# supyuxiang/Inference-Time-Scaling-for-Diffusion-Models-beyond-Scaling-Denoising-Steps

Hardware: AMD Instinct MI355X
Metric: candidate-images/sec at T=1000, CIFAR-10 32x32 UNet, N=256, 1/2/4/8 MI355X (higher is better)
Workload: dtype bf16; 1 GPU; random-search round: N=256/GPU candidates x T=1000 DDPM steps, Arch A UNet 32x32 (ch128 [1,2,3,4] attn[2] nrb2), Oracle verifier; model=DDPM UNet (Diffusion/Model.py) Arch A, global_batch=256, seq_len=1000, parallelism=candidate-dp1, T=1000, graph=True, n_local=256

## Files before the change

include/itsd.h:

```cpp
#ifndef ITSD_H
#define ITSD_H

#include <stdint.h>

#ifdef __cplusplus
extern "C" {
#endif

#define ITSD_OK 0
#define ITSD_ERR_INVALID 1
#define ITSD_ERR_HIP 2
#define ITSD_ERR_WEIGHTS 3
#define ITSD_ERR_NAN 4
#define ITSD_ERR_OOM 5
#define ITSD_ERR_HANDOFF 6

enum { ITSD_ARCH_DDPM = 0, ITSD_ARCH_CFG = 1 };
enum { ITSD_PREC_FP32 = 0, ITSD_PREC_BF16 = 1 };
enum { ITSD_VERIFY_ORACLE = 0, ITSD_VERIFY_SELFSUP = 1, ITSD_VERIFY_AESTHETIC = 2, ITSD_VERIFY_MEAN = 3 };

#define ITSD_RUN_GRAPH 1u
#define ITSD_RUN_CLIP 2u
#define ITSD_RUN_SYNC 4u

typedef struct itsd_unet itsd_unet;

typedef struct {
  int32_t arch;
  int32_t T;
  int32_t ch;
  int32_t n_mult;
  int32_t ch_mult[8];
  int32_t n_attn;
  int32_t attn[8];
  int32_t num_res_blocks;
  int32_t img_size;
  int32_t num_labels;
  int32_t max_batch;
  int32_t precision;
} itsd_unet_desc;

typedef struct {
  const char* name;
  const float* data;
  int64_t numel;
} itsd_tensor_view;

int itsd_unet_create(const itsd_unet_desc* desc, const itsd_tensor_view* weights, int n_weights,
                     int device, itsd_unet** out);
int itsd_unet_destroy(itsd_unet* u);

int itsd_unet_forward(itsd_unet* u, const float* x, const int32_t* t, const int32_t* labels,
                      float* eps, int n, void* stream);

int itsd_unet_representation(itsd_unet* u, float* repr, int n, void* stream);

int itsd_set_schedule(itsd_unet* u, int T, const float* coeff1, const float* coeff2,
                      const float* sqrt_var, float w);

typedef struct {
  int32_t K;
  const int32_t* tau;
  const float* a0;
  const float* b0;
  const float* c0;
  const float* cx;
  const float* sg;
  int32_t clip_x0;
  float w;
} itsd_x0_schedule;

int itsd_set_schedule_x0(itsd_unet* u, const itsd_x0_schedule* schedule);

int itsd_sampler_run(itsd_unet* u, float* x, const int32_t* labels, int n, int t_begin, int t_end,
                     uint64_t seed, int64_t noise_offset, const float* noise, uint32_t flags, void* stream);

int itsd_sampler_predict_x0(itsd_unet* u, const float* x, const int32_t* labels, int n, int t,
                            float a0, float b0, float* x0, void* stream);

int itsd_branch(float* dst, const float* src, const int32_t* parents, int n_src, int n_dst, int64_t per_cand,
                float a, float b, uint64_t seed, uint32_t stream_id, int64_t cand_offset, void* stream);

int itsd_noise(float* out, const float* pivot, int n_cand, int64_t per_cand, float scale, uint64_t seed,
               uint32_t stream_id, int64_t cand_offset, void* stream);

int itsd_verify(int kind, const float* images, int n_cand, int b, int c, int h, int w,
                double* scores, void* stream);

int itsd_verify_paired(const float* images, const float* ref_features, int n_cand, int c, int h, int w,
                       double* scores, void* stream);

int itsd_attention(const void* qkv, const void* vt, void* out, int n, int S, int C, int precision, void* stream);

int itsd_profile_forward(itsd_unet* u, const float* x, const int32_t* t, int n, double* conv_ms,
                         double* conv_flops, int* conv_launches, double* total_ms, void* stream);

int itsd_profile_ops(itsd_unet* u, const float* x, const int32_t* t, int n, int max_ops, int* kinds,
                     double* ms, double* flops, int* shapes, int* n_ops, void* stream);

int itsd_profile_op(itsd_unet* u, const float* x, const int32_t* t, int n, int op_index, int reps, double* ms,
                    void* stream);

int itsd_set_option(const char* key, int value);

int itsd_unet_query(const itsd_unet* u, const char* key, int64_t* value);

enum { ITSD_OP_GN = 0, ITSD_OP_CONV = 1, ITSD_OP_ATTN = 2, ITSD_OP_GNCOEF = 3, ITSD_OP_ATTNBLOCK = 4,
       ITSD_OP_HEAD = 5, ITSD_OP_TAIL = 6 };
enum { ITSD_TAG_NONE = 0,
       ITSD_TAG_QKV = 1,
       ITSD_TAG_DOWN_MERGE = 2,
       ITSD_TAG_ATTN_S1 = 3,
       ITSD_TAG_CONVT = 4,
       ITSD_TAG_ATTNBLOCK = 5 };
#define ITSD_ACT_PROJ (-2)
typedef struct {
  int32_t kind;
  int32_t launched;
  int32_t folded_into;
  int32_t src1, src2, dst, resid, vt;
  int32_t ksize, stride, pad, upsample, zins, subpix, Cout, K, temb_col, vt_from;
  int32_t silu;
  int32_t S, C;
  int32_t kernel;
  int32_t ksplit, sc_split, kS;
  int32_t epilogue;
  int32_t gn_fold;
  int32_t gn_out_op;
  int32_t sc_op;
  int32_t has_coef;
  int32_t tag;
  char name[96];
} itsd_op_info;
typedef struct {
  int32_t H, W, C;
  int32_t elem_size;
  int32_t has_stats;
  int32_t spi;
  int32_t capacity;
} itsd_act_info;
enum { ITSD_PASS_FORWARD = 0, ITSD_PASS_STEP = 1 };
int itsd_unet_op_info(itsd_unet* u, int pass, int n, int op_index, itsd_op_info* info);
int itsd_unet_act_info(const itsd_unet* u, int act, itsd_act_info* info);
enum { ITSD_READ_ACT = 0, ITSD_READ_STATS = 1, ITSD_READ_COEF = 2, ITSD_READ_PROJ = 3 };
int itsd_unet_read(itsd_unet* u, int what, int id, int n, void* dst, int64_t bytes, void* stream);
int itsd_unet_poison(itsd_unet* u, void* stream);

const char* itsd_kernel_name(int id);

enum { ITSD_CALIB_MFMA_BF16 = 0, ITSD_CALIB_HBM_COPY = 1, ITSD_CALIB_MFMA_BF16_16X16 = 2 };
int itsd_calibrate(int what, double* value, void* stream);

const char* itsd_last_error(void);
int itsd_version(void);

#ifdef __cplusplus
}
#endif
#endif
```

inference-time-scaling-for-diffusion-models-beyond-scaling-denoising-steps_amd/csrc/api.hip:

```cpp
#include <hip/hip_runtime.h>

#include <cmath>
#include <cstdio>
#include <cstring>
#include <functional>
#include <map>
#include <memory>
#include <mutex>
#include <string>
#include <tuple>
#include <unordered_map>
#include <vector>

#include "common.h"
#include "itsd.h"

namespace itsd {
template <typename T> hipError_t launch_conv(const ConvArgs&, const ConvPlan&, hipStream_t);
template <typename T> hipError_t launch_groupnorm(const GNArgs&, int, hipStream_t);
template <typename T> hipError_t launch_attn(const AttnArgs&, int, hipStream_t);
bool attn_flash_ok(int S, int C);
bool attn_cs_ok(int S, int C);
bool attn_block_ok(int S, int C);
hipError_t launch_attn_block(const AttnBlockArgs&, int, hipStream_t);
int g_attn_fuse = 1;
int g_tap_prune = 1;
int g_down_merge = 1;
int g_attn_s1 = 1;
template <typename T> hipError_t launch_head(const HeadArgs&, hipStream_t);
template <typename T> hipError_t launch_tail(const TailArgs&, hipStream_t);
hipError_t launch_emb_input(const int*, int, const float*, const float*, int, float*, int, hipStream_t);
hipError_t launch_linear(const float*, int, int, const float*, const float*, int, int, float*, hipStream_t);
hipError_t launch_verify(int, const float*, int, int, int, int, int, double*, const float*, hipStream_t);
hipError_t launch_set_int(int*, int, hipStream_t);
hipError_t launch_add_int(int*, int, hipStream_t);
int calibrate_run(int what, double* value, hipStream_t s);
hipError_t launch_run_begin(int*, int, int*, RunParams*, const RunParams&, hipStream_t);
int g_option_gen = 0;
bool conv_gn_eligible(int H, int W);
bool p5_eligible(int H, int W);
hipError_t launch_gn_coef(const GNArgs&, int, float*, hipStream_t);
hipError_t launch_head_mfma(const HeadArgs&, hipStream_t);
hipError_t launch_tail_mfma(const TailArgs&, hipStream_t);
bool tail_mfma_ok(int H, int W, int C);
int g_io_mfma = 1;
int g_small_gn = 1;
hipError_t launch_noise(float*, const float*, int, long long, float, unsigned long long, unsigned, long long,
                        hipStream_t);
hipError_t launch_branch(float*, const float*, const int*, int, long long, float, float, unsigned long long, unsigned,
                         long long, hipStream_t);
template <typename T> hipError_t launch_nhwc_to_nchw(const void*, float*, int, int, int, hipStream_t);
}

using namespace itsd;

namespace {

thread_local std::string g_err;

int fail(int code, const std::string& msg) {
  g_err = msg;
  return code;
}

#define HIPCHK(x)                                                                           \
  do {                                                                                      \
    hipError_t e_ = (x);                                                                    \
    if (e_ != hipSuccess) return fail(ITSD_ERR_HIP, std::string(#x) + ": " + hipGetErrorString(e_)); \
  } while (0)

#define CHK(x)                  \
  do {                          \
    int r_ = (x);               \
    if (r_ != ITSD_OK) return r_; \
  } while (0)

std::string handoff_msg(int bits) {
  std::string m = "in-kernel hand-off wait exhausted its poll bound (grid not co-resident?):";
  if (bits & 1) m += " attn_block_split_kernel";
  if (bits & 2) m += " conv3x3_gn_p5_kernel (split-K combine)";
  return m;
}

uint16_t host_f2bf(float f) {
  uint32_t u;
  std::memcpy(&u, &f, 4);
  if ((u & 0x7fffffffu) > 0x7f800000u) return (uint16_t)((u >> 16) | 0x40);
  u += 0x7fffu + ((u >> 16) & 1u);
  return (uint16_t)(u >> 16);
}

struct Act {
  size_t off;
  int H, W, C;
  size_t stats = SIZE_MAX;
  int spi = 0;
};

enum OpKind { OP_GN, OP_CONV, OP_ATTN, OP_GNCOEF, OP_ATTNBLOCK };
constexpr int kCensusAttnBlock = 7;
constexpr int kCensusConvGN = 4;
constexpr int kCensusConvGNW = 5;
constexpr int kCensusConvGNW4 = 6;

struct Op {
  OpKind kind;
  int src1 = -1, src2 = -1, dst = -1;
  size_t gamma = 0, beta = 0;
  int silu = 0;
  int ksize = 3, stride = 1, pad = 1, upsample = 0, zins = 0;
  int subpix = 0;
  size_t wt = 0, bias = 0;
  size_t wfrag = SIZE_MAX;
  int Cout = 0, K = 0;
  int temb_col = -1;
  int resid = -1;
  int S = 0, C = 0;
  int vt = -1, vt_from = 0;
  size_t coef = SIZE_MAX;
  size_t bias2 = 0;
  size_t gn_gamma = SIZE_MAX, gn_beta = SIZE_MAX;
  int sc_op = -1, sc_into = -1;
  size_t sc_wfrag = SIZE_MAX, bias_sc = SIZE_MAX;
  int gn_next = -1, gn_from = -1;
  std::string name;
  int tag = ITSD_TAG_NONE;
};

struct Arena {
  std::vector<char> host;
  size_t add(const void* p, size_t bytes) {
    size_t off = (host.size() + 255) & ~(size_t)255;
    host.resize(off + bytes);
    if (p) std::memcpy(host.data() + off, p, bytes);
    return off;
  }
};

struct GraphEntry {
  std::tuple<int, bool, const float*, int, int> key;
  hipGraphExec_t exec = nullptr;
};

}

struct itsd_unet {
  itsd_unet_desc d{};
  int device = 0;
  bool bf16 = false;
  size_t esz = 4;
  bool cfg = false;
  int H = 32, ch = 128, tdim = 512, sumC = 0;
  int nb_max = 0;
  int last_forward_n = 0;

  char* wdev = nullptr;
  char* ws = nullptr;
  size_t ws_bytes = 0;
  std::vector<Act> acts;
  std::vector<Op> ops;
  int head_out = -1, tail_g = -1, tail_in = -1;
  size_t tail_gn_g = 0, tail_gn_b = 0;

  size_t head_w = 0, head_b = 0, tail_w = 0, tail_b = 0;
  size_t head_wmf = SIZE_MAX, tail_wmf = SIZE_MAX, tail_coef = SIZE_MAX;
  size_t freq = 0, ttable = 0, W0t = 0, b0 = 0, W2t = 0, b2 = 0, Wpt = 0, bp = 0;
  size_t ctable = 0, C1t = 0, cb1 = 0, C3t = 0, cb3 = 0, Wct = 0, bc = 0;

  float* emb_buf = nullptr;
  float* h1_buf = nullptr;
  float* te_buf = nullptr;
  float* proj_buf = nullptr;
  int rows_cap = 0;
  float* cemb_table = nullptr;
  int T_sched = 0;
  float* coeff1 = nullptr;
  float* coeff2 = nullptr;
  float* sqrt_var = nullptr;
  float* temb_table = nullptr;
  int sched_form = 0;
  float* xrow = nullptr;
  int clip_x0 = 0;
  float guide_w = 0.f, guide_w1 = 1.f;
  int* d_t = nullptr;
  int* d_nan = nullptr;
  RunParams* d_run = nullptr;
  float* x_state = nullptr;
  int32_t* lab_state = nullptr;
  long long graph_captures = 0;
  void* zero_page = nullptr;
  float* splitk_ws = nullptr;
  int* tickets = nullptr;
  int* attn_sync = nullptr;
  static constexpr long long kSplitkCap = 16ll << 20;

  hipStream_t stream = nullptr;
  hipEvent_t ev_in = nullptr, ev_out = nullptr;
  std::vector<GraphEntry> graphs;

  template <typename P = float>
  P* wp(size_t off) const { return (P*)(wdev + off); }
  void* ap(int id) const { return ws + acts[id].off; }
};

namespace {

struct Builder {
  itsd_unet* u;
  Arena ar;
  std::unordered_map<std::string, std::pair<const float*, int64_t>> w;
  size_t used = 0;
  size_t ws_off = 0;
  std::string err;
  std::vector<std::pair<std::string, size_t>> temb_cols;

  const float* get(const std::string& name, int64_t numel) {
    auto it = w.find(name);
    if (it == w.end()) {
      if (err.empty()) err = "missing key in state_dict: " + name;
      return nullptr;
    }
    if (it->second.second != numel) {
      if (err.empty())
        err = "size mismatch for " + name + ": got " + std::to_string(it->second.second) + " elements, expected " +
              std::to_string(numel);
      return nullptr;
    }
    ++used;
    return it->second.first;
  }
  const float* peek(const std::string& name, int64_t numel) {
    auto it = w.find(name);
    return (it == w.end() || it->second.second != numel) ? nullptr : it->second.first;
  }
  size_t f32(const std::string& name, int64_t numel) {
    const float* p = get(name, numel);
    return ar.add(p, numel * 4);
  }
  int act(int H, int W, int C) {
    Act a{ws_off, H, W, C};
    size_t bytes = (size_t)u->nb_max * H * W * C * u->esz;
    ws_off = (ws_off + bytes + 255) & ~(size_t)255;
    u->acts.push_back(a);
    return (int)u->acts.size() - 1;
  }
  size_t pack(const std::vector<const float*>& parts, int Cpart, int Cin, int ks, bool flip_t = false) {
    const int Cout = Cpart * (int)parts.size();
    const int K = ks * ks * Cin;
    std::vector<float> tmp((size_t)Cout * K, 0.f);
    for (size_t pi = 0; pi < parts.size(); ++pi) {
      const float* src = parts[pi];
      if (!src) continue;
      for (int co = 0; co < Cpart; ++co)
        for (int ci = 0; ci < Cin; ++ci)
          for (int ky = 0; ky < ks; ++ky)
            for (int kx = 0; kx < ks; ++kx) {
              float v;
              if (!flip_t) v = src[(((size_t)co * Cin + ci) * ks + ky) * ks + kx];
              else v = src[(((size_t)ci * Cpart + co) * ks + (ks - 1 - ky)) * ks + (ks - 1 - kx)];
              tmp[((size_t)pi * Cpart + co) * K + (ky * ks + kx) * Cin + ci] = v;
            }
    }
    if (u->bf16) {
      std::vector<uint16_t> b(tmp.size());
      for (size_t i = 0; i < tmp.size(); ++i) b[i] = host_f2bf(tmp[i]);
      return ar.add(b.data(), b.size() * 2);
    }
    return ar.add(tmp.data(), tmp.size() * 4);
  }
  size_t pack_frag(const float* Wsrc, int Cout, int Cin, int ks) {
    const int K = ks * ks * Cin, nks = K / 16;
    std::vector<uint16_t> b((size_t)Cout * K, 0);
    if (Wsrc)
      for (int cb = 0; cb < Cout / 32; ++cb)
        for (int st = 0; st < nks; ++st)
          for (int L = 0; L < 64; ++L)
            for (int e = 0; e < 8; ++e) {
              const int co = 32 * cb + (L & 31), k = 16 * st + 8 * (L >> 5) + e;
              const int tap = k / Cin, ci = k - tap * Cin, ky = tap / ks, kx = tap - ky * ks;
              b[(((size_t)cb * nks + st) * 64 + L) * 8 + e] =
                  host_f2bf(Wsrc[(((size_t)co * Cin + ci) * ks + ky) * ks + kx]);
            }
    return ar.add(b.data(), b.size() * 2);
  }
  size_t frag4(const std::vector<float>& tmp, int Cout, int K) {
    if (!u->bf16 || Cout % 32 || K % 16) return SIZE_MAX;
    const int nks = K / 16;
    std::vector<uint16_t> f(tmp.size());
    for (int ph = 0; ph < 4; ++ph)
      for (int cb = 0; cb < Cout / 32; ++cb)
        for (int st = 0; st < nks; ++st)
          for (int L = 0; L < 64; ++L)
            for (int e = 0; e < 8; ++e)
              f[((((size_t)ph * (Cout / 32) + cb) * nks + st) * 64 + L) * 8 + e] =
                  host_f2bf(tmp[((size_t)ph * Cout + 32 * cb + (L & 31)) * K + 16 * st + 8 * (L >> 5) + e]);
    return ar.add(f.data(), f.size() * 2);
  }
  size_t pack_subpix(const float* W, int Cout, int Cin, size_t* wfrag = nullptr) {
    static const int lo[2][2] = {{0, 1}, {0, 2}}, hi[2][2] = {{0, 2}, {1, 2}};
    const int K = 4 * Cin;
    std::vector<float> tmp((size_t)4 * Cout * K, 0.f);
    for (int ph = 0; ph < 4; ++ph) {
      const int py = ph >> 1, px = ph & 1;
      for (int co = 0; co < Cout; ++co)
        for (int dy = 0; dy < 2; ++dy)
          for (int dx = 0; dx < 2; ++dx)
            for (int ci = 0; ci < Cin; ++ci) {
              double acc = 0.0;
              for (int ky = lo[py][dy]; ky <= hi[py][dy]; ++ky)
                for (int kx = lo[px][dx]; kx <= hi[px][dx]; ++kx)
                  acc += W ? (double)W[(((size_t)co * Cin + ci) * 3 + ky) * 3 + kx] : 0.0;
              tmp[((size_t)ph * Cout + co) * K + (dy * 2 + dx) * Cin + ci] = (float)acc;
            }
    }
    if (wfrag) *wfrag = frag4(tmp, Cout, K);
    if (u->bf16) {
      std::vector<uint16_t> b(tmp.size());
      for (size_t i = 0; i < tmp.size(); ++i) b[i] = host_f2bf(tmp[i]);
      return ar.add(b.data(), b.size() * 2);
    }
    return ar.add(tmp.data(), tmp.size() * 4);
  }
  size_t pack_convt_subpix(const float* W, int Cout, int Cin, size_t* wfrag = nullptr, bool centre_only = false) {
    auto kk = [](int r, int d) { return r == 0 ? 2 - 2 * d : (d < 0 ? -1 : 3 - 2 * d); };
    const int rd = centre_only ? 0 : 1, kw = 2 * rd + 1, K = kw * kw * Cin;
    std::vector<float> tmp((size_t)4 * Cout * K, 0.f);
    for (int ph = 0; ph < 4; ++ph) {
      const int ry = ph >> 1, rx = ph & 1;
      for (int co = 0; co < Cout; ++co)
        for (int dy = -rd; dy <= rd; ++dy)
          for (int dx = -rd; dx <= rd; ++dx) {
            const int ky = kk(ry, dy), kx = kk(rx, dx);
            if (ky < 0 || kx < 0 || !W) continue;
            for (int ci = 0; ci < Cin; ++ci)
              tmp[((size_t)ph * Cout + co) * K + ((dy + rd) * kw + dx + rd) * Cin + ci] =
                  W[(((size_t)ci * Cout + co) * 5 + ky) * 5 + kx];
          }
    }
    if (wfrag) *wfrag = frag4(tmp, Cout, K);
    if (u->bf16) {
      std::vector<uint16_t> b(tmp.size());
      for (size_t i = 0; i < tmp.size(); ++i) b[i] = host_f2bf(tmp[i]);
      return ar.add(b.data(), b.size() * 2);
    }
    return ar.add(tmp.data(), tmp.size() * 4);
  }
  int upconv(int s1, const std::string& name, int Cout, int Hout) {
    const Act& A = u->acts[s1];
    const int Cin = A.C, epc = u->bf16 ? 8 : 4;
    if (((A.H * A.W) % 128 && 128 % (A.H * A.W)) || Cin % (8 * epc))
      return conv_layer(s1, -1, name, Cout, 3, 1, 1, 1, Hout, Hout);
    const float* W = get(name + ".weight", (int64_t)Cout * Cin * 9);
    size_t wf = SIZE_MAX;
    const bool p4sub = Cout % 128 == 0 && Cin % 64 == 0 && Cin >= 128 && A.H == A.W && (A.W == 8 || A.W == 16 || A.W == 32);
    size_t wt = pack_subpix(W, Cout, Cin, p4sub ? &wf : nullptr);
    size_t b = f32(name + ".bias", Cout);
    int dst = act(Hout, Hout, Cout);
    if (A.H * A.W < 128) u->acts[dst].spi = 4;
    conv(s1, -1, dst, wt, b, Cout, 3, 1, 1, 1);
    Op& o = u->ops.back();
    o.name = name;
    o.subpix = 1;
    o.wfrag = wf;
    return dst;
  }
  size_t concat_f32(const std::vector<const float*>& parts, int n) {
    std::vector<float> tmp((size_t)n * parts.size(), 0.f);
    for (size_t i = 0; i < parts.size(); ++i)
      if (parts[i]) std::memcpy(tmp.data() + i * n, parts[i], n * 4);
    return ar.add(tmp.data(), tmp.size() * 4);
  }
  size_t transposed(const float* W, int out, int in) {
    std::vector<float> tmp((size_t)out * in, 0.f);
    if (W)
      for (int o = 0; o < out; ++o)
        for (int i = 0; i < in; ++i) tmp[(size_t)i * out + o] = W[(size_t)o * in + i];
    return ar.add(tmp.data(), tmp.size() * 4);
  }

  void gn(int s1, int s2, int dst, const std::string& p, int C, int silu) {
    Op o;
    o.kind = OP_GN;
    o.src1 = s1; o.src2 = s2; o.dst = dst;
    o.gamma = f32(p + ".weight", C);
    o.beta = f32(p + ".bias", C);
    o.silu = silu;
    o.name = p;
    u->ops.push_back(o);
  }
  void conv(int s1, int s2, int dst, size_t wt, size_t bias, int Cout, int ks, int stride, int pad, int ups,
            int temb_col = -1, int resid = -1, int zins = 0) {
    Op o;
    o.kind = OP_CONV;
    o.src1 = s1; o.src2 = s2; o.dst = dst;
    o.wt = wt; o.bias = bias; o.Cout = Cout;
    const int Cin = u->acts[s1].C + (s2 >= 0 ? u->acts[s2].C : 0);
    o.K = ks * ks * Cin;
    o.ksize = ks; o.stride = stride; o.pad = pad; o.upsample = ups; o.zins = zins;
    o.temb_col = temb_col; o.resid = resid;
    u->ops.push_back(o);
  }
  int conv_layer(int s1, int s2, const std::string& name, int Cout, int ks, int stride, int pad, int ups, int Hout,
                 int Wout, int temb_col = -1, int resid = -1, const std::string& gn = "", const float* Wx = nullptr,
                 const float* bx = nullptr) {
    const int Cin = u->acts[s1].C + (s2 >= 0 ? u->acts[s2].C : 0);
    size_t coef = SIZE_MAX;
    if (!gn.empty()) {
      Op g;
      g.kind = OP_GNCOEF;
      g.src1 = s1; g.src2 = s2;
      g.gamma = f32(gn + ".weight", Cin);
      g.beta = f32(gn + ".bias", Cin);
      g.coef = coef = ws_off;
      g.name = gn;
      ws_off = (ws_off + (size_t)u->nb_max * Cin * 2 * 4 + 255) & ~(size_t)255;
      u->ops.push_back(g);
    }
    const float* W = Wx ? Wx : get(name + ".weight", (int64_t)Cout * Cin * ks * ks);
    std::vector<float> wwin;
    {
      const Act& A = u->acts[s1];
      const int k0 = std::max(0, pad - (Hout - 1) * stride), k1 = std::min(ks - 1, A.H + pad - 1);
      const int x0 = std::max(0, pad - (Wout - 1) * stride), x1 = std::min(ks - 1, A.W + pad - 1);
      if (itsd::g_tap_prune && gn.empty() && !ups && W && (k0 > 0 || k1 < ks - 1) && k0 == x0 && k1 == x1 && k1 >= k0) {
        const int ks2 = k1 - k0 + 1;
        wwin.resize((size_t)Cout * Cin * ks2 * ks2);
        for (size_t oc = 0; oc < (size_t)Cout * Cin; ++oc)
          for (int ky = 0; ky < ks2; ++ky)
            for (int kx = 0; kx < ks2; ++kx)
              wwin[(oc * ks2 + ky) * ks2 + kx] = W[(oc * ks + k0 + ky) * ks + k0 + kx];
        W = wwin.data();
        ks = ks2;
        pad -= k0;
      }
    }
    size_t wt = pack({W}, Cout, Cin, ks);
    size_t b = bx ? ar.add(bx, (size_t)Cout * 4) : f32(name + ".bias", Cout);
    int dst = act(Hout, Wout, Cout);
    conv(s1, s2, dst, wt, b, Cout, ks, stride, pad, ups, temb_col, resid);
    u->ops.back().name = name;
    u->ops.back().coef = coef;
    if (coef != SIZE_MAX) {
      u->ops.back().gn_gamma = u->ops[u->ops.size() - 2].gamma;
      u->ops.back().gn_beta = u->ops[u->ops.size() - 2].beta;
    }
    const bool plain3 = coef == SIZE_MAX && ks == 3 && stride == 1 && pad == 1 && !ups && Cout % 128 == 0 &&
                        Cin % 128 == 0 && Hout == Wout && (Hout == 32 || Hout == 16 || Hout == 8);
    if ((coef != SIZE_MAX || plain3) && u->bf16 && Cout % 32 == 0 && (ks * ks * Cin) % 16 == 0)
      u->ops.back().wfrag = pack_frag(W, Cout, Cin, ks);
    return dst;
  }
  bool fusable(int s1, int s2, int Cout) const {
    const Act& A = u->acts[s1];
    return u->bf16 && itsd::g_fuse_gn && A.C % 64 == 0 && (s2 < 0 || u->acts[s2].C % 64 == 0) &&
           Cout % 128 == 0 && (conv_gn_eligible(A.H, A.W) || p5_eligible(A.H, A.W));
  }

  int resblock(int x1, int x2, const std::string& p, int in_ch, int out_ch, bool attn) {
    const int H = u->acts[x1].H, W = u->acts[x1].W;
    const int col = u->sumC;
    u->sumC += out_ch;
    temb_cols.push_back({p, (size_t)col});
    int h1, o;
    int resid = x1;
    if (fusable(x1, x2, out_ch)) {
      h1 = conv_layer(x1, x2, p + ".block1.2", out_ch, 3, 1, 1, 0, H, W, col, -1, p + ".block1.0");
    } else {
      int g1 = act(H, W, in_ch);
      gn(x1, x2, g1, p + ".block1.0", in_ch, 1);
      h1 = conv_layer(g1, -1, p + ".block1.2", out_ch, 3, 1, 1, 0, H, W, col);
    }
    const bool f2 = fusable(h1, -1, out_ch);
    int g2 = -1;
    if (!f2) {
      g2 = act(H, W, out_ch);
      gn(h1, -1, g2, p + ".block2.0", out_ch, 1);
    }
    int isc = -1;
    if (in_ch != out_ch) {
      resid = conv_layer(x1, x2, p + ".shortcut", out_ch, 1, 1, 0, 0, H, W);
      isc = (int)u->ops.size() - 1;
    }
    if (f2) o = conv_layer(h1, -1, p + ".block2.3", out_ch, 3, 1, 1, 0, H, W, -1, resid, p + ".block2.0");
    else o = conv_layer(g2, -1, p + ".block2.3", out_ch, 3, 1, 1, 0, H, W, -1, resid);
    if (f2 && isc >= 0 && u->bf16 && out_ch % 32 == 0 && u->acts[x1].C % 64 == 0 && (x2 < 0 || u->acts[x2].C % 64 == 0)) {
      const float* wsc = peek(p + ".shortcut.weight", (int64_t)out_ch * in_ch);
      const float* bsc = peek(p + ".shortcut.bias", out_ch);
      const float* bb2 = peek(p + ".block2.3.bias", out_ch);
      if (wsc && bsc && bb2) {
        std::vector<float> bs((size_t)out_ch);
        for (int c = 0; c < out_ch; ++c) bs[c] = bb2[c] + bsc[c];
        Op& c2 = u->ops.back();
        c2.sc_wfrag = pack_frag(wsc, out_ch, in_ch, 1);
        c2.bias_sc = ar.add(bs.data(), (size_t)out_ch * 4);
        c2.sc_op = isc;
        u->ops[isc].sc_into = (int)u->ops.size() - 1;
      }
    }
    if (attn && H * W == 1 && itsd::g_attn_s1) {
      const std::string a = p + ".attn";
      const int64_t cc = (int64_t)out_ch * out_ch;
      const float* wv = get(a + ".proj_v.weight", cc);
      const float* bv = get(a + ".proj_v.bias", out_ch);
      const float* wp = get(a + ".proj.weight", cc);
      const float* bp = get(a + ".proj.bias", out_ch);
      const bool qk = get(a + ".proj_q.weight", cc) && get(a + ".proj_q.bias", out_ch) && get(a + ".proj_k.weight", cc) &&
                      get(a + ".proj_k.bias", out_ch);
      if (wv && bv && wp && bp && qk) {
        std::vector<float> wf((size_t)cc), bf((size_t)out_ch);
        std::vector<double> row((size_t)out_ch);
        for (int oc = 0; oc < out_ch; ++oc) {
          std::fill(row.begin(), row.end(), 0.0);
          double bacc = (double)bp[oc];
          for (int c = 0; c < out_ch; ++c) {
            const double w = (double)wp[(size_t)oc * out_ch + c];
            const float* vr = wv + (size_t)c * out_ch;
            for (int ic = 0; ic < out_ch; ++ic) row[ic] += w * (double)vr[ic];
            bacc += w * (double)bv[c];
          }
          for (int ic = 0; ic < out_ch; ++ic) wf[(size_t)oc * out_ch + ic] = (float)row[ic];
          bf[oc] = (float)bacc;
        }
        int ga = act(H, W, out_ch);
        gn(o, -1, ga, a + ".group_norm", out_ch, 0);
        const int r = conv_layer(ga, -1, a + ".proj", out_ch, 1, 1, 0, 0, H, W, -1, o, "", wf.data(), bf.data());
        u->ops.back().name = a;
        u->ops.back().tag = ITSD_TAG_ATTN_S1;
        return r;
      }
    }
    if (attn && u->bf16 && itsd::g_attn_fuse && attn_block_ok(H * W, out_ch)) {
      const std::string a = p + ".attn";
      const int C = out_ch;
      const int64_t cc = (int64_t)C * C;
      const float* wq = get(a + ".proj_q.weight", cc);
      const float* wk = get(a + ".proj_k.weight", cc);
      const float* wv = get(a + ".proj_v.weight", cc);
      const float* wp = get(a + ".proj.weight", cc);
      const float* bq = get(a + ".proj_q.bias", C);
      const float* bv = get(a + ".proj_v.bias", C);
      get(a + ".proj_k.bias", C);
      std::vector<float> wcat((size_t)2 * cc, 0.f), bcat((size_t)2 * C, 0.f);
      if (wq && wk && wv && wp && bq && bv) {
        std::vector<double> acc((size_t)cc);
        auto fold = [&](const float* A, const float* B, bool ta, float* dst) {
          std::fill(acc.begin(), acc.end(), 0.0);
          for (int r = 0; r < C; ++r) {
            double* row = acc.data() + (size_t)r * C;
            for (int k = 0; k < C; ++k) {
              const double w = (double)(ta ? A[(size_t)k * C + r] : A[(size_t)r * C + k]);
              const float* br = B + (size_t)k * C;
              for (int i = 0; i < C; ++i) row[i] += w * (double)br[i];
            }
          }
          for (int64_t i = 0; i < cc; ++i) dst[i] = (float)acc[i];
        };
        fold(wk, wq, true, wcat.data());
        fold(wp, wv, false, wcat.data() + cc);
        for (int j = 0; j < C; ++j) {
          double su = 0.0, sb = 0.0;
          for (int k = 0; k < C; ++k) {
            su += (double)wk[(size_t)k * C + j] * (double)bq[k];
            sb += (double)wp[(size_t)j * C + k] * (double)bv[k];
          }
          bcat[j] = (float)su;
          bcat[C + j] = (float)sb;
        }
      }
      Op ab;
      ab.kind = OP_ATTNBLOCK;
      ab.src1 = o;
      ab.gamma = f32(a + ".group_norm.weight", out_ch);
      ab.beta = f32(a + ".group_norm.bias", out_ch);
      ab.wt = pack_frag(wcat.data(), 2 * out_ch, out_ch, 1);
      ab.bias = ar.add(bcat.data(), bcat.size() * 4);
      ab.bias2 = f32(a + ".proj.bias", out_ch);
      ab.S = H * W;
      ab.C = out_ch;
      ab.dst = act(H, W, out_ch);
      ab.name = a;
      ab.tag = ITSD_TAG_ATTNBLOCK;
      u->ops.push_back(ab);
      return ab.dst;
    }
    if (attn) {
      const std::string a = p + ".attn";
      int ga = act(H, W, out_ch);
      gn(o, -1, ga, a + ".group_norm", out_ch, 0);
      const int64_t cc = (int64_t)out_ch * out_ch;
      size_t wqkv = pack({get(a + ".proj_q.weight", cc), get(a + ".proj_k.weight", cc), get(a + ".proj_v.weight", cc)},
                         out_ch, out_ch, 1);
      size_t bqkv = concat_f32({get(a + ".proj_q.bias", out_ch), get(a + ".proj_k.bias", out_ch),
                                get(a + ".proj_v.bias", out_ch)}, out_ch);
      int qkv = act(H, W, 3 * out_ch);
      conv(ga, -1, qkv, wqkv, bqkv, 3 * out_ch, 1, 1, 0, 0);
      u->ops.back().name = a;
      u->ops.back().tag = ITSD_TAG_QKV;
      const int S = H * W;
      int vt = -1;
      if (u->bf16 && S % 16 == 0 && out_ch % 64 == 0 && (S <= 256 || attn_flash_ok(S, out_ch) || attn_cs_ok(S, out_ch))) {
        vt = act(out_ch, S, 1);
        u->ops.back().vt = vt;
        u->ops.back().vt_from = 2 * out_ch;
      }
      int ao = act(H, W, out_ch);
      Op at;
      at.kind = OP_ATTN;
      at.name = a;
      at.src1 = qkv; at.dst = ao; at.S = H * W; at.C = out_ch; at.vt = vt;
      u->ops.push_back(at);
      o = conv_layer(ao, -1, a + ".proj", out_ch, 1, 1, 0, 0, H, W, -1, o);
    }
    return o;
  }
};

int build(itsd_unet* u, const itsd_tensor_view* views, int nviews) {
  Builder b;
  b.u = u;
  for (int i = 0; i < nviews; ++i) b.w[views[i].name] = {views[i].data, views[i].numel};
  const itsd_unet_desc& d = u->d;
  const int ch = d.ch, tdim = 4 * ch, H = d.img_size;
  u->ch = ch; u->tdim = tdim; u->H = H;

  if (!u->cfg) {
    u->freq = b.f32("time_embedding.freq_coeffs", ch / 2);
    u->W0t = b.transposed(b.get("time_embedding.timembedding.0.weight", (int64_t)tdim * ch), tdim, ch);
    u->b0 = b.f32("time_embedding.timembedding.0.bias", tdim);
    u->W2t = b.transposed(b.get("time_embedding.timembedding.2.weight", (int64_t)tdim * tdim), tdim, tdim);
    u->b2 = b.f32("time_embedding.timembedding.2.bias", tdim);
  } else {
    u->ttable = b.f32("time_embedding.timembedding.0.weight", (int64_t)d.T * ch);
    u->W0t = b.transposed(b.get("time_embedding.timembedding.1.weight", (int64_t)tdim * ch), tdim, ch);
    u->b0 = b.f32("time_embedding.timembedding.1.bias", tdim);
    u->W2t = b.transposed(b.get("time_embedding.timembedding.3.weight", (int64_t)tdim * tdim), tdim, tdim);
    u->b2 = b.f32("time_embedding.timembedding.3.bias", tdim);
    u->ctable = b.f32("cond_embedding.condEmbedding.0.weight", (int64_t)(d.num_labels + 1) * ch);
    u->C1t = b.transposed(b.get("cond_embedding.condEmbedding.1.weight", (int64_t)tdim * ch), tdim, ch);
    u->cb1 = b.f32("cond_embedding.condEmbedding.1.bias", tdim);
    u->C3t = b.transposed(b.get("cond_embedding.condEmbedding.3.weight", (int64_t)tdim * tdim), tdim, tdim);
    u->cb3 = b.f32("cond_embedding.condEmbedding.3.bias", tdim);
  }
  u->head_w = b.f32("head.weight", (int64_t)ch * 27);
  u->head_b = b.f32("head.bias", ch);
  u->head_out = b.act(H, H, ch);
  if (u->bf16 && itsd::g_io_mfma && ch % 32 == 0 && (H * H) % 128 == 0 && 128 % H == 0) {
    const float* hw = b.peek("head.weight", (int64_t)ch * 27);
    if (hw) {
      std::vector<uint16_t> wm((size_t)ch * 32, 0);
      for (int co = 0; co < ch; ++co)
        for (int k = 0; k < 27; ++k) wm[(size_t)co * 32 + k] = host_f2bf(hw[(size_t)co * 27 + k]);
      u->head_wmf = b.ar.add(wm.data(), wm.size() * 2);
    }
  } else {
    const int G = stat_slot_px(H * H);
    if ((H * H) % G || (G % H && H % G))
      return fail(ITSD_ERR_INVALID, "img_size " + std::to_string(H) + " not supported by the head kernel (its " +
                                        std::to_string(G) + "-pixel blocks hold whole rows or lie inside one)");
  }

  std::vector<int> hs{u->head_out};
  int cur = u->head_out;
  int now = ch;
  int ndown = 0;
  auto P = [](const char* s, int i) { return std::string(s) + "." + std::to_string(i); };
  for (int i = 0; i < d.n_mult; ++i) {
    const int out = ch * d.ch_mult[i];
    bool at = false;
    for (int k = 0; k < d.n_attn; ++k) at |= (d.attn[k] == i);
    if (u->cfg) at = true;
    for (int r = 0; r < d.num_res_blocks; ++r) {
      cur = b.resblock(cur, -1, P("downblocks", ndown++), now, out, at);
      now = out;
      hs.push_back(cur);
    }
    if (i != d.n_mult - 1) {
      const std::string p = P("downblocks", ndown++);
      const int Hc = b.u->acts[cur].H;
      if (!u->cfg) {
        cur = b.conv_layer(cur, -1, p + ".main", now, 3, 2, 1, 0, Hc / 2, Hc / 2);
      } else if (!itsd::g_down_merge) {
        int t1 = b.conv_layer(cur, -1, p + ".c1", now, 3, 2, 1, 0, Hc / 2, Hc / 2);
        cur = b.conv_layer(cur, -1, p + ".c2", now, 5, 2, 2, 0, Hc / 2, Hc / 2, -1, t1);
      } else {
        const int Cin = b.u->acts[cur].C;
        const float* W1 = b.get(p + ".c1.weight", (int64_t)now * Cin * 9);
        const float* W2 = b.get(p + ".c2.weight", (int64_t)now * Cin * 25);
        const float* b1 = b.get(p + ".c1.bias", now);
        const float* b2 = b.get(p + ".c2.bias", now);
        std::vector<float> wm((size_t)now * Cin * 25, 0.f), bm(now, 0.f);
        if (W2) std::memcpy(wm.data(), W2, wm.size() * 4);
        if (W1)
          for (size_t oc = 0; oc < (size_t)now * Cin; ++oc)
            for (int ky = 0; ky < 3; ++ky)
              for (int kx = 0; kx < 3; ++kx) wm[(oc * 5 + ky + 1) * 5 + kx + 1] += W1[(oc * 3 + ky) * 3 + kx];
        for (int c = 0; c < now; ++c) bm[c] = (b1 ? b1[c] : 0.f) + (b2 ? b2[c] : 0.f);
        cur = b.conv_layer(cur, -1, p + ".c12", now, 5, 2, 2, 0, Hc / 2, Hc / 2, -1, -1, "", wm.data(), bm.data());
        u->ops.back().name = p;
        u->ops.back().tag = ITSD_TAG_DOWN_MERGE;
      }
      hs.push_back(cur);
    }
  }
  cur = b.resblock(cur, -1, "middleblocks.0", now, now, true);
  cur = b.resblock(cur, -1, "middleblocks.1", now, now, false);
  int nup = 0;
  for (int i = d.n_mult - 1; i >= 0; --i) {
    const int out = ch * d.ch_mult[i];
    bool at = false;
    for (int k = 0; k < d.n_attn; ++k) at |= (d.attn[k] == i);
    if (u->cfg) at = false;
    for (int r = 0; r < d.num_res_blocks + 1; ++r) {
      int skip = hs.back();
      hs.pop_back();
      cur = b.resblock(cur, skip, P("upblocks", nup++), now + u->acts[skip].C, out, at);
      now = out;
    }
    if (i != 0) {
      const std::string p = P("upblocks", nup++);
      const int Hc = b.u->acts[cur].H;
      if (!u->cfg) {
        cur = b.upconv(cur, p + ".main", now, 2 * Hc);
      } else {
        const float* Wt = b.get(p + ".t.weight", (int64_t)now * now * 25);
        size_t bt = b.f32(p + ".t.bias", now);
        int tmp = b.act(2 * Hc, 2 * Hc, now);
        const int epc = u->bf16 ? 8 : 4;
        if (((Hc * Hc) % 128 == 0 || 128 % (Hc * Hc) == 0) && now % (8 * epc) == 0) {
          size_t wf = SIZE_MAX;
          const bool p4sub = now % 128 == 0 && now >= 128 && (Hc == 8 || Hc == 16 || Hc == 32);
          const bool c1 = Hc == 1 && itsd::g_tap_prune;
          size_t wt = b.pack_convt_subpix(Wt, now, now, p4sub ? &wf : nullptr, c1);
          if (Hc * Hc < 128) u->acts[tmp].spi = 4;
          b.conv(cur, -1, tmp, wt, bt, now, c1 ? 1 : 3, 1, c1 ? 0 : 1, 0);
          u->ops.back().subpix = 2;
          u->ops.back().wfrag = wf;
          u->ops.back().name = p + ".t";
          u->ops.back().tag = ITSD_TAG_CONVT;
        } else {
          size_t wt = b.pack({Wt}, now, now, 5, true);
          b.conv(cur, -1, tmp, wt, bt, now, 5, 1, 2, 0, -1, -1, 1);
          u->ops.back().name = p + ".t";
          u->ops.back().tag = ITSD_TAG_CONVT;
        }
        cur = b.conv_layer(tmp, -1, p + ".c", now, 3, 1, 1, 0, 2 * Hc, 2 * Hc);
      }
    }
  }
  if (!hs.empty()) return fail(ITSD_ERR_INVALID, "internal: skip stack not empty");
  u->tail_in = cur;
  u->tail_gn_g = b.f32("tail.0.weight", now);
  u->tail_gn_b = b.f32("tail.0.bias", now);
  u->tail_w = b.f32("tail.2.weight", (int64_t)3 * now * 9);
  u->tail_b = b.f32("tail.2.bias", 3);
  if (u->bf16 && itsd::g_io_mfma && tail_mfma_ok(H, H, now)) {
    const float* tw = b.peek("tail.2.weight", (int64_t)3 * now * 9);
    if (tw) {
      const int nks = 9 * now / 32;
      std::vector<uint16_t> wm((size_t)nks * 4 * 3 * 8);
      for (int ks = 0; ks < nks; ++ks)
        for (int kg = 0; kg < 4; ++kg)
          for (int co = 0; co < 3; ++co)
            for (int j = 0; j < 8; ++j) {
              const int k = 32 * ks + 8 * kg + j, tap = k / now, ci = k - tap * now;
              wm[(((size_t)ks * 4 + kg) * 3 + co) * 8 + j] = host_f2bf(tw[((size_t)co * now + ci) * 9 + tap]);
            }
      u->tail_wmf = b.ar.add(wm.data(), wm.size() * 2);
    }
    u->tail_coef = b.ws_off;
    b.ws_off = (b.ws_off + (size_t)u->nb_max * now * 2 * 4 + 255) & ~(size_t)255;
  } else {
    u->tail_g = b.act(H, H, now);
  }

  {
    std::vector<float> Wp((size_t)u->sumC * tdim), bpv(u->sumC), Wc, bcv;
    if (u->cfg) { Wc.resize(Wp.size()); bcv.resize(u->sumC); }
    for (size_t k = 0; k < b.temb_cols.size(); ++k) {
      const std::string& p = b.temb_cols[k].first;
      const size_t col = b.temb_cols[k].second;
      const size_t next = (k + 1 < b.temb_cols.size()) ? b.temb_cols[k + 1].second : (size_t)u->sumC;
      const int oc = (int)(next - col);
      auto fill = [&](const std::string& nm, std::vector<float>& Wd, std::vector<float>& bd) {
        const float* W = b.get(nm + ".weight", (int64_t)oc * tdim);
        const float* bb = b.get(nm + ".bias", oc);
        if (!W || !bb) return;
        for (int o = 0; o < oc; ++o) {
          for (int i = 0; i < tdim; ++i) Wd[(size_t)i * u->sumC + col + o] = W[(size_t)o * tdim + i];
          bd[col + o] = bb[o];
        }
      };
      fill(p + ".temb_proj.1", Wp, bpv);
      if (u->cfg) fill(p + ".cond_proj.1", Wc, bcv);
    }
    u->Wpt = b.ar.add(Wp.data(), Wp.size() * 4);
    u->bp = b.ar.add(bpv.data(), bpv.size() * 4);
    if (u->cfg) {
      u->Wct = b.ar.add(Wc.data(), Wc.size() * 4);
      u->bc = b.ar.add(bcv.data(), bcv.size() * 4);
    }
  }
  if (!b.err.empty()) return fail(ITSD_ERR_WEIGHTS, b.err);
  if ((int)b.used != nviews) {
    return fail(ITSD_ERR_WEIGHTS, "state_dict has " + std::to_string(nviews) + " entries, model uses " +
                                      std::to_string(b.used) + " (unexpected keys present)");
  }
  for (size_t i = 1; i < u->ops.size(); ++i) {
    Op& g = u->ops[i];
    Op& p = u->ops[i - 1];
    if (g.kind == OP_GN && g.src2 < 0 && p.kind == OP_CONV && p.dst == g.src1 && p.sc_into < 0 && p.vt < 0) {
      p.gn_next = (int)i;
      g.gn_from = (int)i - 1;
    }
  }
  {
    std::vector<int> need;
    for (const Op& o : u->ops)
      if (o.kind == OP_GN || o.kind == OP_GNCOEF || o.kind == OP_ATTNBLOCK) {
        need.push_back(o.src1);
        if (o.src2 >= 0) need.push_back(o.src2);
      }
    need.push_back(u->tail_in);
    for (int id : need) {
      Act& A = u->acts[id];
      if (A.stats != SIZE_MAX) continue;
      const int HW = A.H * A.W;
      if (!(128 % HW == 0 || HW % 128 == 0))
        return fail(ITSD_ERR_INVALID, "spatial size " + std::to_string(HW) + " not supported by the GN statistics slots");
      const size_t slots = (size_t)u->nb_max * stat_spi(HW, A.spi);
      A.stats = b.ws_off;
      b.ws_off = (b.ws_off + slots * 2 * A.C * 4 + 255) & ~(size_t)255;
      bool produced = (id == u->head_out);
      for (const Op& o : u->ops) produced |= ((o.kind == OP_CONV || o.kind == OP_ATTNBLOCK) && o.dst == id);
      if (!produced) return fail(ITSD_ERR_INVALID, "internal: GroupNorm input without a statistics producer");
    }
  }
  HIPCHK(hipMalloc(&u->wdev, b.ar.host.size()));
  HIPCHK(hipMemcpy(u->wdev, b.ar.host.data(), b.ar.host.size(), hipMemcpyHostToDevice));
  u->ws_bytes = b.ws_off;
  HIPCHK(hipMalloc(&u->ws, u->ws_bytes));
  return ITSD_OK;
}

struct RunCtx {
  int nb;
  const float* x;
  int x_mod;
  const float* temb;
  const int* tsel;
  long long temb_img_stride;
  const int32_t* labels;
  int label_mod;
  int uncond_from;
  TailArgs tail;
  bool census = false;
  std::vector<std::pair<hipEvent_t, hipEvent_t>>* evs = nullptr;
  std::vector<int>* ev_kind = nullptr;
  std::vector<double>* ev_flops = nullptr;
  std::vector<int>* ev_kid = nullptr;
  std::vector<int>* ev_op = nullptr;
};

int conv_args(itsd_unet* u, const Op& o, const RunCtx& c, ConvArgs& a, ConvPlan& p) {
    const Act& in = u->acts[o.src1];
    const Act& out = u->acts[o.dst];
    a.src1 = u->ap(o.src1);
    a.src2 = o.src2 >= 0 ? u->ap(o.src2) : nullptr;
    a.C1 = in.C;
    a.C2 = o.src2 >= 0 ? u->acts[o.src2].C : 0;
    a.Hin = in.H; a.Win = in.W; a.Hout = out.H; a.Wout = out.W;
    a.ksize = o.ksize; a.stride = o.stride; a.pad = o.pad; a.upsample = o.upsample;
    a.wt = u->wdev + o.wt;
    a.wfrag = o.wfrag != SIZE_MAX ? u->wdev + o.wfrag : nullptr;
    a.Cout = o.Cout; a.K = o.K;
    a.bias = u->wp(o.bias);
    if (o.temb_col >= 0) {
      a.temb = c.temb + o.temb_col;
      a.temb_tsel = c.tsel;
      a.temb_row_stride = u->sumC;
      a.temb_img_stride = c.temb_img_stride;
      if (u->cfg) {
        a.cemb = u->cemb_table + o.temb_col;
        a.cemb_labels = (const int*)c.labels;
        a.cemb_row_stride = u->sumC;
        a.cemb_label_mod = c.label_mod;
        a.cemb_uncond_from = c.uncond_from;
      }
    }
    a.resid = o.resid >= 0 ? u->ap(o.resid) : nullptr;
    a.out = u->ap(o.dst);
    a.M = c.nb * out.H * out.W;
    a.stats = out.stats != SIZE_MAX ? (float*)(u->ws + out.stats) : nullptr;
    a.zero = u->zero_page;
    a.splitk_ws = u->splitk_ws;
    a.splitk_cap = itsd_unet::kSplitkCap;
    a.tickets = u->tickets;
    a.err = u->d_nan + 1;
    a.spin_bound = itsd::g_spin_bound;
    if (o.vt >= 0) {
      if (o.vt_from % 128 || (out.H * out.W) % 8) return fail(ITSD_ERR_INVALID, "internal: bad channel-major V split");
      a.vt_out = u->ap(o.vt);
      a.vt_from = o.vt_from;
    }
    a.zins = o.zins;
    a.dbg = itsd::g_conv_dbg;
    a.xcd = itsd::g_p4_xcd == 1 || (itsd::g_p4_xcd == 2 && a.Wout == 8);
    if (o.subpix) {
      a.subpix = o.subpix;
      a.Hout = in.H; a.Wout = in.W;
      a.M = c.nb * in.H * in.W;
      a.ksize = o.subpix == 2 ? o.ksize : 2; a.pad = o.subpix == 2 ? o.pad : 0; a.upsample = 0; a.zins = 0;
      a.K = a.ksize * a.ksize * (a.C1 + a.C2);
      a.tap_live = o.subpix == 2 && a.ksize == 3 && itsd::g_convt_prune;
    }
    if (o.coef != SIZE_MAX) {
      if (!u->bf16 || o.ksize != 3 || o.stride != 1 || o.pad != 1 || o.upsample || o.zins ||
          !(conv_gn_eligible(in.H, in.W) || p5_eligible(in.H, in.W)) || a.C1 % 64 || a.C2 % 64 || a.Cout % 128)
        return fail(ITSD_ERR_INVALID, "internal: fused GroupNorm conv on an unsupported shape");
      a.gn_coef = (const float*)(u->ws + o.coef);
    }
    {
      const int epc = u->bf16 ? 8 : 4;
      if (a.C1 % epc || a.C2 % epc || a.Cout % 4 || a.K % epc)
        return fail(ITSD_ERR_INVALID, "conv channels must be multiples of " + std::to_string(epc));
    }
  if (o.sc_op >= 0 && itsd::g_p5_sc) {
    const Op& sc = u->ops[o.sc_op];
    a.sc_src1 = u->ap(sc.src1);
    a.sc_src2 = sc.src2 >= 0 ? u->ap(sc.src2) : nullptr;
    a.sc_C1 = u->acts[sc.src1].C;
    a.sc_C2 = sc.src2 >= 0 ? u->acts[sc.src2].C : 0;
    a.sc_wfrag = u->wdev + o.sc_wfrag;
  }
  p = plan_conv(a, u->bf16);
  const bool p5 = p.kernel == ConvKernel::P5 || p.kernel == ConvKernel::P5_SHARED;
  const bool p4 = p.kernel == ConvKernel::P4_GN || p.kernel == ConvKernel::P4_C96;
  if (p.sc_split) {
    a.bias = u->wp(o.bias_sc);
    a.resid = nullptr;
  } else {
    a.sc_src1 = a.sc_src2 = a.sc_wfrag = nullptr;
    a.sc_C1 = a.sc_C2 = 0;
  }
  if (a.gn_coef && o.gn_gamma != SIZE_MAX && itsd::g_gn_fold && (a.C1 + a.C2) % 128 == 0 && in.H * in.W <= 1024 &&
      (p5 || p4)) {
    a.gn_fold = 1;
    a.gn_st1 = (const float*)(u->ws + u->acts[o.src1].stats);
    a.gn_st2 = o.src2 >= 0 ? (const float*)(u->ws + u->acts[o.src2].stats) : nullptr;
    a.gn_spi1 = u->acts[o.src1].spi;
    a.gn_spi2 = o.src2 >= 0 ? u->acts[o.src2].spi : 0;
    a.gn_gamma = u->wp(o.gn_gamma);
    a.gn_beta = u->wp(o.gn_beta);
  }
  if (o.gn_next >= 0 && itsd::g_small_gn && u->bf16 && a.stats && !a.gn_coef && !o.subpix && !a.vt_out &&
      u->acts[o.dst].spi == 0) {
    const int HWo = a.Hout * a.Wout, gs = a.Cout / kGnGroups;
    if (HWo <= 16 && 64 % HWo == 0 && a.Cout % 64 == 0 && gs >= 2 && 64 % gs == 0 && p.kernel == ConvKernel::SMALL) {
      const Op& g = u->ops[o.gn_next];
      a.gn_out = u->ap(g.dst);
      a.go_gamma = u->wp(g.gamma);
      a.go_beta = u->wp(g.beta);
      a.go_silu = g.silu;
    }
  }
  return ITSD_OK;
}

struct ConvLaunch {
  ConvArgs a{};
  ConvPlan p;
  int rc = ITSD_OK;
  std::string err;
};

std::vector<ConvLaunch> resolve_program(itsd_unet* u, const RunCtx& c) {
  std::vector<ConvLaunch> r(u->ops.size());
  for (size_t oi = 0; oi < u->ops.size(); ++oi) {
    if (u->ops[oi].kind != OP_CONV) continue;
    r[oi].rc = conv_args(u, u->ops[oi], c, r[oi].a, r[oi].p);
    if (r[oi].rc != ITSD_OK) r[oi].err = g_err;
  }
  return r;
}

int folded_into(const itsd_unet* u, const std::vector<ConvLaunch>& rp, size_t oi) {
  const Op& o = u->ops[oi];
  if (o.kind == OP_GNCOEF && oi + 1 < u->ops.size() && rp[oi + 1].a.gn_fold) return (int)oi + 1;
  if (o.kind == OP_GN && o.gn_from >= 0 && rp[o.gn_from].a.gn_out) return o.gn_from;
  if (o.kind == OP_CONV && o.sc_into >= 0 && rp[o.sc_into].p.sc_split) return o.sc_into;
  return -1;
}

GNArgs gn_args(const itsd_unet* u, const Op& o) {
  GNArgs g{};
  g.C1 = u->acts[o.src1].C;
  g.C2 = o.src2 >= 0 ? u->acts[o.src2].C : 0;
  g.HW = u->acts[o.src1].H * u->acts[o.src1].W;
  g.gamma = u->wp(o.gamma);
  g.beta = u->wp(o.beta);
  g.eps = kGnEps;
  g.st1 = (const float*)(u->ws + u->acts[o.src1].stats);
  g.st2 = o.src2 >= 0 ? (const float*)(u->ws + u->acts[o.src2].stats) : nullptr;
  g.spi1 = u->acts[o.src1].spi;
  g.spi2 = o.src2 >= 0 ? u->acts[o.src2].spi : 0;
  return g;
}

int launch_op(itsd_unet* u, const Op& o, const RunCtx& c, const ConvLaunch* cl, hipStream_t s) {
  hipError_t e = hipSuccess;
  if (o.kind == OP_GNCOEF) {
    e = launch_gn_coef(gn_args(u, o), c.nb, (float*)(u->ws + o.coef), s);
  } else if (o.kind == OP_GN) {
    GNArgs a = gn_args(u, o);
    a.src1 = u->ap(o.src1);
    a.src2 = o.src2 >= 0 ? u->ap(o.src2) : nullptr;
    a.silu = o.silu;
    a.dst = u->ap(o.dst);
    e = u->bf16 ? launch_groupnorm<bf16_t>(a, c.nb, s) : launch_groupnorm<float>(a, c.nb, s);
  } else if (o.kind == OP_CONV) {
    if (cl->rc != ITSD_OK) return fail(cl->rc, cl->err);
    e = u->bf16 ? launch_conv<bf16_t>(cl->a, cl->p, s) : launch_conv<float>(cl->a, cl->p, s);
  } else if (o.kind == OP_ATTNBLOCK) {
    AttnBlockArgs a{};
    const Act& in = u->acts[o.src1];
    const Act& out = u->acts[o.dst];
    a.x = (const bf16_t*)u->ap(o.src1);
    a.st = (const float*)(u->ws + in.stats);
    a.spi = stat_spi(in.H * in.W, in.spi);
    a.gamma = u->wp(o.gamma);
    a.beta = u->wp(o.beta);
    a.wmv = (const bf16_t*)(u->wdev + o.wt);
    a.buv = u->wp(o.bias);
    a.bp = u->wp(o.bias2);
    a.out = (bf16_t*)u->ap(o.dst);
    a.out_stats = out.stats != SIZE_MAX ? (float*)(u->ws + out.stats) : nullptr;
    a.scale = (float)std::pow((double)o.C, -0.5);
    a.n = c.nb;
    a.S = o.S;
    static_assert((4ll << 20) / 4 <= itsd_unet::kSplitkCap, "the partial-score slab fits the split-K workspace");
    a.spart = u->splitk_ws;
    a.sync = u->attn_sync;
    a.err = u->d_nan + 1;
    a.spin_bound = itsd::g_spin_bound;
    e = launch_attn_block(a, o.C, s);
  } else {
    AttnArgs a{};
    a.qkv = u->ap(o.src1);
    a.vt = o.vt >= 0 ? u->ap(o.vt) : nullptr;
    a.out = u->ap(o.dst);
    a.S = o.S; a.C = o.C;
    a.scale = (float)std::pow((double)o.C, -0.5);
    e = u->bf16 ? launch_attn<bf16_t>(a, c.nb, s) : launch_attn<float>(a, c.nb, s);
  }
  if (e != hipSuccess) return fail(ITSD_ERR_HIP, std::string("kernel launch: ") + hipGetErrorString(e));
  return ITSD_OK;
}

double op_flops(const itsd_unet* u, const Op& o, int nb) {
  if (o.kind == OP_CONV) {
    const Act& out = u->acts[o.dst];
    return 2.0 * nb * out.H * out.W * (double)o.Cout * (o.subpix == 1 ? o.K * 4 / 9 : o.K);
  }
  if (o.kind == OP_ATTN) return 2.0 * 2.0 * nb * (double)o.S * o.S * o.C;
  if (o.kind == OP_ATTNBLOCK)
    return 2.0 * nb * (double)o.S * (4.0 * o.C * o.C) + 2.0 * 2.0 * nb * (double)o.S * o.S * o.C;
  return 0.0;
}

int run_program(itsd_unet* u, const RunCtx& c, const std::vector<ConvLaunch>& rp, hipStream_t s) {
  int cur_op = 0;
  auto mark = [&](int kind, double fl, const std::function<int()>& fn) -> int {
    if (!c.census) return fn();
    if (c.ev_op) c.ev_op->push_back(cur_op);
    hipEvent_t a, b;
    HIPCHK(hipEventCreate(&a));
    if (hipError_t e = hipEventCreate(&b); e != hipSuccess) {
      hipEventDestroy(a);
      return fail(ITSD_ERR_HIP, std::string("hipEventCreate(&b): ") + hipGetErrorString(e));
    }
    HIPCHK(hipEventRecord(a, s));
    itsd::g_last_kernel = nullptr;
    int r = fn();
    HIPCHK(hipEventRecord(b, s));
    c.evs->push_back({a, b});
    c.ev_kind->push_back(kind);
    c.ev_flops->push_back(fl);
    if (c.ev_kid) c.ev_kid->push_back(itsd::kernel_id(itsd::g_last_kernel));
    return r;
  };
  CHK(mark(-1, 2.0 * c.nb * u->H * u->H * 27.0 * u->ch, [&]() -> int {
    HeadArgs h{};
    h.x = c.x;
    h.w = u->wp(u->head_w);
    h.b = u->wp(u->head_b);
    h.out = u->ap(u->head_out);
    h.H = u->H; h.W = u->H; h.Cout = u->ch; h.n = c.nb; h.x_img_mod = c.x_mod;
    const Act& ho = u->acts[u->head_out];
    h.stats = ho.stats != SIZE_MAX ? (float*)(u->ws + ho.stats) : nullptr;
    hipError_t e;
    if (u->head_wmf != SIZE_MAX) {
      h.wmf = (const bf16_t*)(u->wdev + u->head_wmf);
      e = launch_head_mfma(h, s);
    } else {
      e = u->bf16 ? launch_head<bf16_t>(h, s) : launch_head<float>(h, s);
    }
    return e == hipSuccess ? ITSD_OK : fail(ITSD_ERR_HIP, hipGetErrorString(e));
  }));
  for (size_t oi = 0; oi < u->ops.size(); ++oi) {
    const Op& o = u->ops[oi];
    if (folded_into(u, rp, oi) >= 0) continue;
    const ConvLaunch& cl = rp[oi];
    int kind = o.kind == OP_ATTNBLOCK ? kCensusAttnBlock : (int)o.kind;
    cur_op = (int)oi + 1;
    if (o.kind == OP_CONV && o.coef != SIZE_MAX)
      kind = cl.p.wide_segs == 1 ? kCensusConvGNW : cl.p.wide_segs == 4 ? kCensusConvGNW4 : kCensusConvGN;
    double fl = op_flops(u, o, c.nb);
    if (cl.p.sc_split) fl += 2.0 * cl.a.M * (double)o.Cout * (cl.a.sc_C1 + cl.a.sc_C2);
    CHK(mark(kind, fl, [&]() { return launch_op(u, o, c, &cl, s); }));
  }
  cur_op = 0;
  Op g;
  g.src1 = u->tail_in; g.gamma = u->tail_gn_g; g.beta = u->tail_gn_b; g.silu = 1;
  if (u->tail_wmf != SIZE_MAX) {
    g.kind = OP_GNCOEF;
    g.coef = u->tail_coef;
  } else {
    g.kind = OP_GN;
    g.dst = u->tail_g;
  }
  CHK(mark((int)g.kind, 0.0, [&]() { return launch_op(u, g, c, nullptr, s); }));
  CHK(mark(-2, 2.0 * c.tail.n * (c.tail.cfg ? 2 : 1) * u->H * u->H * 27.0 * u->acts[u->tail_in].C, [&]() -> int {
    TailArgs t = c.tail;
    t.w = u->wp(u->tail_w);
    t.b = u->wp(u->tail_b);
    t.H = u->H; t.W = u->H; t.C = u->acts[u->tail_in].C;
    hipError_t e;
    if (u->tail_wmf != SIZE_MAX) {
      t.g = u->ap(u->tail_in);
      t.coef = (const float*)(u->ws + u->tail_coef);
      t.wmf = (const bf16_t*)(u->wdev + u->tail_wmf);
      e = launch_tail_mfma(t, s);
    } else {
      t.g = u->ap(u->tail_g);
      e = u->bf16 ? launch_tail<bf16_t>(t, s) : launch_tail<float>(t, s);
    }
    return e == hipSuccess ? ITSD_OK : fail(ITSD_ERR_HIP, hipGetErrorString(e));
  }));
  return ITSD_OK;
}

int temb_rows(itsd_unet* u, const int* idx, int M, int offset, bool cond, float* out, hipStream_t s) {
  if (M > u->rows_cap) return fail(ITSD_ERR_INVALID, "temb rows exceed capacity");
  const int ch = u->ch, td = u->tdim;
  hipError_t e;
  if (!cond) {
    e = launch_emb_input(idx, M, u->cfg ? nullptr : u->wp(u->freq), u->cfg ? u->wp(u->ttable) : nullptr, ch,
                         u->emb_buf, offset, s);
  } else {
    e = launch_emb_input(idx, M, nullptr, u->wp(u->ctable), ch, u->emb_buf, offset, s);
  }
  if (e != hipSuccess) return fail(ITSD_ERR_HIP, hipGetErrorString(e));
  const float* W0 = u->wp(cond ? u->C1t : u->W0t);
  const float* b0 = u->wp(cond ? u->cb1 : u->b0);
  const float* W2 = u->wp(cond ? u->C3t : u->W2t);
  const float* b2 = u->wp(cond ? u->cb3 : u->b2);
  HIPCHK(launch_linear(u->emb_buf, M, ch, W0, b0, td, 0, u->h1_buf, s));
  HIPCHK(launch_linear(u->h1_buf, M, td, W2, b2, td, 1, u->te_buf, s));
  HIPCHK(launch_linear(u->te_buf, M, td, u->wp(cond ? u->Wct : u->Wpt), u->wp(cond ? u->bc : u->bp), u->sumC, 1,
                       out, s));
  return ITSD_OK;
}

int alloc_rows(itsd_unet* u, int rows) {
  if (rows <= u->rows_cap) return ITSD_OK;
  hipFree(u->emb_buf); hipFree(u->h1_buf); hipFree(u->te_buf);
  HIPCHK(hipMalloc(&u->emb_buf, (size_t)rows * u->ch * 4));
  HIPCHK(hipMalloc(&u->h1_buf, (size_t)rows * u->tdim * 4));
  HIPCHK(hipMalloc(&u->te_buf, (size_t)rows * u->tdim * 4));
  u->rows_cap = rows;
  return ITSD_OK;
}

void clear_graphs(itsd_unet* u) {
  for (auto& g : u->graphs)
    if (g.exec) hipGraphExecDestroy(g.exec);
  u->graphs.clear();
}

void drop_schedule(itsd_unet* u) {
  clear_graphs(u);
  hipFree(u->coeff1); hipFree(u->coeff2); hipFree(u->sqrt_var); hipFree(u->xrow); hipFree(u->temb_table);
  u->coeff1 = u->coeff2 = u->sqrt_var = u->xrow = u->temb_table = nullptr;
  u->T_sched = 0;
  u->sched_form = 0;
  u->clip_x0 = 0;
}

int check_batch(itsd_unet* u, int n) {
  if (n <= 0 || n > u->d.max_batch)
    return fail(ITSD_ERR_INVALID, "batch " + std::to_string(n) + " outside [1, max_batch=" +
                                      std::to_string(u->d.max_batch) + "]");
  return ITSD_OK;
}

RunCtx forward_ctx(const itsd_unet* u, int n, const float* x, const int32_t* labels, float* eps_out) {
  RunCtx c{};
  c.nb = n; c.x = x; c.x_mod = n;
  c.temb = u->proj_buf; c.tsel = nullptr; c.temb_img_stride = u->sumC;
  c.labels = labels; c.label_mod = n; c.uncond_from = -1;
  c.tail.n = n; c.tail.cfg = 0; c.tail.step_mode = 0; c.tail.eps_out = eps_out;
  return c;
}

RunCtx step_ctx(const itsd_unet* u, int n, float* x, const int32_t* labels) {
  RunCtx c{};
  c.nb = u->cfg ? 2 * n : n;
  c.x = x; c.x_mod = n;
  c.temb = u->temb_table; c.tsel = u->d_t; c.temb_img_stride = 0;
  c.labels = labels; c.label_mod = n; c.uncond_from = u->cfg ? n : -1;
  c.tail.n = n; c.tail.cfg = u->cfg ? 1 : 0; c.tail.guide_w = u->guide_w; c.tail.guide_w1 = u->guide_w1;
  c.tail.x = x;
  return c;
}

int enter_stream(itsd_unet* u, hipStream_t cs) {
  HIPCHK(hipSetDevice(u->device));
  HIPCHK(hipEventRecord(u->ev_in, cs));
  HIPCHK(hipStreamWaitEvent(u->stream, u->ev_in, 0));
  return ITSD_OK;
}
int leave_stream(itsd_unet* u, hipStream_t cs) {
  HIPCHK(hipEventRecord(u->ev_out, u->stream));
  HIPCHK(hipStreamWaitEvent(cs, u->ev_out, 0));
  return ITSD_OK;
}

int step_graph(itsd_unet* u, const RunCtx& c, int n, bool labels, const float* noise, hipGraphExec_t* exec) {
  const auto key = std::make_tuple(n, labels, noise, itsd::g_option_gen, u->sched_form);
  for (auto& g : u->graphs)
    if (g.key == key) { *exec = g.exec; return ITSD_OK; }
  hipStream_t s = u->stream;
  HIPCHK(hipStreamBeginCapture(s, hipStreamCaptureModeThreadLocal));
  int r = run_program(u, c, resolve_program(u, c), s);
  if (r == ITSD_OK && launch_add_int(u->d_t, -1, s) != hipSuccess) r = fail(ITSD_ERR_HIP, "add_int");
  hipGraph_t graph = nullptr;
  hipError_t e = hipStreamEndCapture(s, &graph);
  if (r != ITSD_OK) { if (graph) hipGraphDestroy(graph); return r; }
  if (e != hipSuccess) return fail(ITSD_ERR_HIP, std::string("capture: ") + hipGetErrorString(e));
  e = hipGraphInstantiate(exec, graph, nullptr, nullptr, 0);
  hipGraphDestroy(graph);
  if (e != hipSuccess) return fail(ITSD_ERR_HIP, std::string("instantiate: ") + hipGetErrorString(e));
  if (u->graphs.size() >= 4) { hipGraphExecDestroy(u->graphs.front().exec); u->graphs.erase(u->graphs.begin()); }
  u->graphs.push_back({key, *exec});
  ++u->graph_captures;
  return ITSD_OK;
}

struct ProfileScratch {
  float* eps = nullptr;
  int32_t* lab0 = nullptr;
  std::vector<std::pair<hipEvent_t, hipEvent_t>> evs;
  std::vector<int> kinds, kid, eop;
  std::vector<double> fl;
  ~ProfileScratch() {
    for (auto& p : evs) {
      if (p.first) hipEventDestroy(p.first);
      if (p.second) hipEventDestroy(p.second);
    }
    hipFree(eps);
    hipFree(lab0);
  }
  int begin(itsd_unet* u, const int32_t* t, int n, hipStream_t cs) {
    CHK(check_batch(u, n));
    HIPCHK(hipSetDevice(u->device));
    u->last_forward_n = 0;
    HIPCHK(hipStreamSynchronize(cs));
    HIPCHK(hipMalloc(&eps, (size_t)n * 3 * u->H * u->H * 4));
    if (u->cfg) {
      HIPCHK(hipMalloc(&lab0, (size_t)n * 4));
      HIPCHK(hipMemsetAsync(lab0, 0, (size_t)n * 4, u->stream));
    }
    return temb_rows(u, t, n, 0, false, u->proj_buf, u->stream);
  }
  void census(RunCtx& c, bool ids) {
    c.census = true; c.evs = &evs; c.ev_kind = &kinds; c.ev_flops = &fl;
    if (ids) { c.ev_kid = &kid; c.ev_op = &eop; }
  }
};

}

namespace itsd {
thread_local const char* g_last_kernel = nullptr;
std::mutex& kernel_names_mu() {
  static std::mutex m;
  return m;
}
std::vector<const char*>& kernel_names() {
  static std::vector<const char*> v;
  return v;
}
int kernel_id(const char* name) {
  if (!name) return 0;
  std::lock_guard<std::mutex> lk(kernel_names_mu());
  auto& v = kernel_names();
  for (size_t i = 0; i < v.size(); ++i)
    if (v[i] == name || !std::strcmp(v[i], name)) return (int)i + 1;
  v.push_back(name);
  return (int)v.size();
}
}

namespace {
enum : unsigned {
  kDiag = 1,
  kShip1 = 2,
  kBool = 4,
  kSet = 8,
  kMask = 16,
};
struct Option {
  const char* key;
  int* var;
  int lo, hi;
  unsigned flags;
  const char* what;
  int set[6] = {-1, -1, -1, -1, -1, -1};
};
constexpr int kConvDbgMask = 1 | 2 | 8 | 16 | 32 | 64 | 128 | 256 | 512 | 1024 | 2048 | 4096 | (127 << 13) | (3 << 20);
const Option kOptions[] = {
    {"conv_variant", &g_conv_variant, 1, 2, 0, "2 conv_pipe (shipped), 1 conv_igemm (register-staged, parity checks)"},
    {"splitk", &g_splitk, 0, 64, kShip1, "split-K for under-filled grids: 0 off, 1 auto, >= 2 forced slice count"},
    {"splitk_inl", &g_splitk_inl, 0, 1, 0, "conv_pipe split-K: 1 in-launch ticket combine, 0 splitk_epilogue_kernel"},
    {"subpix_split", &g_subpix_split, 0, 1, 0, "under-filled sub-pixel conv_pipe launches split K in-launch"},
    {"conv1x1", &g_conv1x1, 0, 2, kShip1, "streaming 1x1 kernel for statistics-free 1x1 convs of large pixel counts: 0 off, 1 on, 2 the 7-stage ring"},
    {"small_conv", &g_small_conv, 0, 2, 0, "conv_small's 64x64 tiles at the small levels: 0 off, 1 auto, 2 whenever eligible"},
    {"small_8x8", &g_small_8x8, 0, 1, 0, "conv_small (split K) for under-filled 8x8-level convs"},
    {"small_wide", &g_small_wide, 0, 2, 0, "conv_small for under-filled statistics-free convs of larger images: 0 off, 1 under 256 tiles, 2 under 512"},
    {"small_minks", &g_small_minks, 1, 64, kDiag, "conv_small split K: at least this many 64-channel K-chunks a slice"},
    {"small_gn", &g_small_gn, 0, 1, 0, "conv_small writes its consumer GroupNorm's output (the GN launch skipped): 0 off, 1 on"},
    {"conv_dbg", &g_conv_dbg, 0, kConvDbgMask, kDiag | kMask, "measurement-only conv ablations (a bit mask; results are wrong when set)"},
    {"fuse_gn", &g_fuse_gn, 0, 1, kBool, "fused GroupNorm+SiLU+conv3x3 in ResBlocks (UNets created afterwards)"},
    {"gn_wide", &g_gn_wide, 0, 2, 0, "the persistent 256-pixel fused conv: 0 off, 1 auto, 2 whenever eligible"},
    {"gn_fold", &g_gn_fold, 0, 1, kBool, "GroupNorm finalize inside conv3x3_gn_p4 / p5_kernel: 0 off, 1 on"},
    {"p4_w", &g_p4_w, 0, 7, 0, "levels conv3x3_gn_p4_kernel takes (bit 0 W = 8, 1 W = 16, 2 W = 32); the others run p5 / 128-pixel tiles"},
    {"p4_xcd", &g_p4_xcd, 0, 2, kDiag, "conv3x3_gn_p4_kernel deals each XCD a contiguous range of tiles: 0 off, 1 on, 2 the 8x8 level only"},
    {"p4_c96", &g_p4_c96, 0, 2, 0, "8x8 conv3x3_gn_p4_kernel on 96-cout tiles: 0 off, 1 auto, 2 always (Cout % 96 == 0)"},
    {"p4_sub", &g_p4_sub, 0, 1, 0, "nearest-x2 upsample convs on conv3x3_gn_p4_kernel's sub-pixel form: 0 off, 1 on"},
    {"p4_plain", &g_p4_plain, 0, 2, 0, "plain 3x3 stride-1 convs on conv3x3_gn_p4_kernel (halo copies the input): 0 off, 1 from 128 tiles, 2 any tile count"},
    {"p5", &g_p5, 0, 2, 0, "conv3x3_gn_p5_kernel at 8x8: 0 off, 1 auto, 2 always (4x4: always)"},
    {"p5_split", &g_p5_split, 0, 16, 0, "p5's K slices: 0 auto (cost model), 1..16 forced"},
    {"p5_sc", &g_p5_sc, 0, 2, 0, "ResBlock 1x1 shortcuts as K slices of their block2 p5 conv: 0 off, 1 auto, 2 always"},
    {"p5_pub", &g_p5_pub, 0, 1, 0, "p5's two-slice last-arriver combine: 1 only the first arriver stores its partial, 0 both (round 5; bit-identity checks)"},
    {"p5_xl", &g_p5_xl, 0, 3, 0, "p5's split-K partials through one XCD's L2: 0 off, 1 the shared combine at 8x8 / 16x16, 2 every eligible form (A/B), 3 (shipped) 1 + the two-slice form at 8x8 / 16x16 where K <= 3456"},
    {"p5_dist", &g_p5_dist, 0, 2, 0, "p5's split-K combine shared by every slice (co-resident grids): 0 off (last arriver), 1 on, 2 the plans of 1 combined by the last arriver (bit-identity checks)"},
    {"p5_c64", &g_p5_c64, 0, 2, kDiag, "64-cout conv3x3_gn_p5_kernel items at 8x8 / 4x4: 0 off, 1 auto, 2 always"},
    {"convt_prune", &g_convt_prune, 0, 1, 0, "ConvTranspose2d sub-pixel phases skip their all-zero taps (p4 / conv_pipe)"},
    {"tap_prune", &g_tap_prune, 0, 1, kBool, "drop all-padding conv taps at build time (UNets created afterwards)"},
    {"down_merge", &g_down_merge, 0, 1, kBool, "CFG DownSample c1 + c2 as one 5x5 conv (UNets created afterwards)"},
    {"io_mfma", &g_io_mfma, 0, 1, kBool, "bf16 head / tail on MFMA (UNets created afterwards)"},
    {"attn_fuse", &g_attn_fuse, 0, 1, 0, "fused AttnBlock kernel (S = 64): 0 off, 1 on (UNets created afterwards; the 16-token form was removed)"},
    {"attn_s1", &g_attn_s1, 0, 1, 0, "one-token AttnBlock folded to GroupNorm + one 1x1 conv (UNets created afterwards)"},
    {"attn_split", &g_attn_split, 0, 6, kSet, "attn_block_split_kernel (an image over G blocks): 0 off, 1 auto, 2 / 4 / 6 forced", {0, 1, 2, 4, 6, -1}},
    {"attn_wide", &g_attn_wide, 0, 2, 0, "channel-split attention (attn_cs_kernel): 0 off, 1 auto (C >= 384 at S >= 256; C = 1024), 2 wherever it applies"},
    {"attn_wide_nq", &g_attn_wide_nq, 0, 2, 0, "channel-split attention: query groups a block (0 auto, 1, 2)"},
    {"attn_cs", &g_attn_cs, 0, 8, kDiag, "attn_mfma_kernel output-channel slices: 0 auto, 1..8 forced"},
    {"attn_aq", &g_attn_aq, 0, 64, kDiag | kSet, "attn_mfma_kernel queries per block: 0 auto, 32, 64", {0, 32, 64, -1}},
    {"spin_bound", &g_spin_bound, 0, 0x7fffffff, 0, "diagnostic: polls before an in-kernel hand-off wait fails (shipped 1 << 22)"},
};
}

extern "C" {

int itsd_version(void) { return 1; }

const char* itsd_kernel_name(int id) {
  std::lock_guard<std::mutex> lk(itsd::kernel_names_mu());
  return id > 0 && id <= (int)itsd::kernel_names().size() ? itsd::kernel_names()[id - 1] : "";
}

int itsd_set_option(const char* key, int value) {
  if (!key) return fail(ITSD_ERR_INVALID, "null key");
#ifdef ITSD_DIAG
  const bool shipped = false;
#else
  const bool shipped = true;
#endif
  const Option* o = nullptr;
  for (const Option& r : kOptions)
    if (!std::strcmp(key, r.key)) o = &r;
  if (o && shipped && (o->flags & kDiag))
    return fail(ITSD_ERR_INVALID, std::string(key) + ": diagnostic builds only (tools/build_diag.sh)");
  if (o && shipped && (o->flags & kShip1) && value > 1)
    return fail(ITSD_ERR_INVALID, std::string(key) + " in [" + std::to_string(o->lo) + ",1] (above: diagnostic builds only, tools/build_diag.sh)");
  ++itsd::g_option_gen;
  if (!o) return fail(ITSD_ERR_INVALID, std::string("unknown option ") + key);
  int v = value;
  if (o->flags & kBool) {
    v = value ? 1 : 0;
  } else if (o->flags & kMask) {
    v = value & o->hi;
  } else if (o->flags & kSet) {
    bool ok = false;
    std::string vals;
    for (const int* q = o->set; *q >= 0; ++q) {
      ok |= *q == value;
      vals += (vals.empty() ? "" : ",") + std::to_string(*q);
    }
    if (!ok) return fail(ITSD_ERR_INVALID, std::string(key) + " in {" + vals + "}: " + o->what);
  } else if (value < o->lo || value > o->hi) {
    return fail(ITSD_ERR_INVALID, std::string(key) + " in [" + std::to_string(o->lo) + "," + std::to_string(o->hi) + "]: " + o->what);
  }
  *o->var = v;
  return ITSD_OK;
}

const char* itsd_last_error(void) { return g_err.c_str(); }

int itsd_calibrate(int what, double* value, void* stream) {
  if (!value) return fail(ITSD_ERR_INVALID, "null argument");
  if (what != ITSD_CALIB_MFMA_BF16 && what != ITSD_CALIB_HBM_COPY && what != ITSD_CALIB_MFMA_BF16_16X16) return fail(ITSD_ERR_INVALID, "unknown calibration");
  const int rc = calibrate_run(what, value, (hipStream_t)stream);
  if (rc == ITSD_ERR_OOM) return fail(rc, "calibration buffers (2 x 1 GiB)");
  if (rc != ITSD_OK) return fail(rc, "calibration kernel");
  return ITSD_OK;
}

int itsd_unet_query(const itsd_unet* u, const char* key, int64_t* value) {
  if (!u || !key || !value) return fail(ITSD_ERR_INVALID, "null argument");
  if (!std::strcmp(key, "graph_captures")) *value = u->graph_captures;
  else if (!std::strcmp(key, "max_batch")) *value = u->d.max_batch;
  else if (!std::strcmp(key, "T_sched")) *value = u->T_sched;
  else if (!std::strcmp(key, "sched_form")) *value = u->sched_form;
  else if (!std::strcmp(key, "ws_bytes")) *value = (int64_t)u->ws_bytes;
  else if (!std::strcmp(key, "ops")) *value = (int64_t)u->ops.size();
  else if (!std::strcmp(key, "status")) {
    if (hipStreamSynchronize(u->stream) != hipSuccess) return fail(ITSD_ERR_HIP, "status: stream synchronize");
    int flag = 0;
    if (hipMemcpy(&flag, u->d_nan + 1, 4, hipMemcpyDeviceToHost) != hipSuccess) return fail(ITSD_ERR_HIP, "status: copy");
    *value = flag;
  }
  else return fail(ITSD_ERR_INVALID, std::string("unknown query key ") + key);
  return ITSD_OK;
}

int itsd_unet_create(const itsd_unet_desc* desc, const itsd_tensor_view* weights, int n_weights, int device,
                     itsd_unet** out) {
  if (!desc || !out || (!weights && n_weights)) return fail(ITSD_ERR_INVALID, "null argument");
  const itsd_unet_desc& d = *desc;
  if (d.arch != ITSD_ARCH_DDPM && d.arch != ITSD_ARCH_CFG) return fail(ITSD_ERR_INVALID, "unknown arch");
  if (d.ch <= 0 || d.ch % 32 || d.n_mult < 1 || d.n_mult > 8 || d.n_attn < 0 || d.n_attn > 8 ||
      d.num_res_blocks < 1 || d.max_batch < 1 || d.img_size < 8)
    return fail(ITSD_ERR_INVALID, "invalid UNet descriptor");
  if (d.img_size % (1 << (d.n_mult - 1))) return fail(ITSD_ERR_INVALID, "img_size not divisible by the down path");
  for (int k = 0; k < d.n_attn; ++k)
    if (d.attn[k] < 0 || d.attn[k] >= d.n_mult) return fail(ITSD_ERR_INVALID, "attn index out of bound");
  if (d.precision != ITSD_PREC_FP32 && d.precision != ITSD_PREC_BF16) return fail(ITSD_ERR_INVALID, "precision");
  HIPCHK(hipSetDevice(device));
  {
    int cus = 0;
    if (hipDeviceGetAttribute(&cus, hipDeviceAttributeMultiprocessorCount, device) == hipSuccess && cus > 0)
      itsd::g_num_cus = cus;
  }
  std::unique_ptr<itsd_unet> u(new itsd_unet());
  u->d = d;
  u->device = device;
  u->bf16 = d.precision == ITSD_PREC_BF16;
  u->esz = u->bf16 ? 2 : 4;
  u->cfg = d.arch == ITSD_ARCH_CFG;
  u->nb_max = d.max_batch * (u->cfg ? 2 : 1);
  CHK(build(u.get(), weights, n_weights));
  HIPCHK(hipStreamCreateWithFlags(&u->stream, hipStreamNonBlocking));
  HIPCHK(hipEventCreateWithFlags(&u->ev_in, hipEventDisableTiming));
  HIPCHK(hipEventCreateWithFlags(&u->ev_out, hipEventDisableTiming));
  HIPCHK(hipMalloc(&u->d_t, 64));
  HIPCHK(hipMalloc(&u->d_nan, 64));
  HIPCHK(hipMalloc(&u->d_run, sizeof(RunParams)));
  HIPCHK(hipMemset(u->d_run, 0, sizeof(RunParams)));
  HIPCHK(hipMalloc(&u->x_state, (size_t)d.max_batch * 3 * d.img_size * d.img_size * 4));
  HIPCHK(hipMalloc(&u->lab_state, (size_t)d.max_batch * 4));
  HIPCHK(hipMalloc(&u->zero_page, 64 * 4096 + 1024));
  HIPCHK(hipMemset(u->zero_page, 0, 64 * 4096 + 1024));
  HIPCHK(hipMalloc(&u->splitk_ws, itsd_unet::kSplitkCap * 4));
  HIPCHK(hipMalloc(&u->tickets, itsd::kTicketCap * 4));
  HIPCHK(hipMemset(u->tickets, 0, itsd::kTicketCap * 4));
  HIPCHK(hipMalloc(&u->attn_sync, (size_t)u->nb_max * 4));
  HIPCHK(hipMemset(u->attn_sync, 0, (size_t)u->nb_max * 4));
  HIPCHK(hipMalloc(&u->proj_buf, (size_t)d.max_batch * u->sumC * 4));
  CHK(alloc_rows(u.get(), std::max(d.max_batch, d.num_labels + 1)));
  if (u->cfg) {
    HIPCHK(hipMalloc(&u->cemb_table, (size_t)(d.num_labels + 1) * u->sumC * 4));
    CHK(temb_rows(u.get(), nullptr, d.num_labels + 1, 0, true, u->cemb_table, u->stream));
    HIPCHK(hipStreamSynchronize(u->stream));
  }
  *out = u.release();
  return ITSD_OK;
}

int itsd_unet_destroy(itsd_unet* u) {
  if (!u) return ITSD_OK;
  hipSetDevice(u->device);
  clear_graphs(u);
  hipFree(u->wdev); hipFree(u->ws); hipFree(u->emb_buf); hipFree(u->h1_buf); hipFree(u->te_buf);
  hipFree(u->proj_buf); hipFree(u->cemb_table); hipFree(u->coeff1); hipFree(u->coeff2); hipFree(u->sqrt_var);
  hipFree(u->xrow); hipFree(u->temb_table); hipFree(u->d_t); hipFree(u->d_nan); hipFree(u->d_run); hipFree(u->x_state); hipFree(u->lab_state); hipFree(u->zero_page);
  hipFree(u->splitk_ws);
  hipFree(u->tickets);
  hipFree(u->attn_sync);
  if (u->stream) hipStreamDestroy(u->stream);
  if (u->ev_in) hipEventDestroy(u->ev_in);
  if (u->ev_out) hipEventDestroy(u->ev_out);
  delete u;
  return ITSD_OK;
}

int itsd_unet_forward(itsd_unet* u, const float* x, const int32_t* t, const int32_t* labels, float* eps, int n,
                      void* stream) {
  if (!u || !x || !t || !eps) return fail(ITSD_ERR_INVALID, "null argument");
  if (u->cfg && !labels) return fail(ITSD_ERR_INVALID, "CFG UNet needs labels");
  CHK(check_batch(u, n));
  hipStream_t cs = (hipStream_t)stream;
  hipStream_t s = u->stream;
  CHK(enter_stream(u, cs));
  CHK(temb_rows(u, t, n, 0, false, u->proj_buf, s));
  const RunCtx c = forward_ctx(u, n, x, labels, eps);
  HIPCHK(hipMemsetAsync(u->d_nan + 1, 0, 4, s));
  CHK(run_program(u, c, resolve_program(u, c), s));
  u->last_forward_n = n;
  return leave_stream(u, cs);
}

int itsd_unet_representation(itsd_unet* u, float* repr, int n, void* stream) {
  if (!u || !repr) return fail(ITSD_ERR_INVALID, "null argument");
  if (u->last_forward_n == 0) return fail(ITSD_ERR_INVALID, "itsd_unet_representation: no itsd_unet_forward on this handle yet");
  if (n < 1 || n > u->last_forward_n)
    return fail(ITSD_ERR_INVALID, "itsd_unet_representation: n outside [1, last forward's batch]");
  const Act& A = u->acts[u->tail_in];
  hipStream_t cs = (hipStream_t)stream;
  hipStream_t s = u->stream;
  CHK(enter_stream(u, cs));
  HIPCHK(u->bf16 ? launch_nhwc_to_nchw<bf16_t>(u->ap(u->tail_in), repr, n, A.H * A.W, A.C, s)
                 : launch_nhwc_to_nchw<float>(u->ap(u->tail_in), repr, n, A.H * A.W, A.C, s));
  return leave_stream(u, cs);
}

int itsd_set_schedule(itsd_unet* u, int T, const float* coeff1, const float* coeff2, const float* sqrt_var, float w) {
  if (!u || T < 1 || !coeff1 || !coeff2 || !sqrt_var) return fail(ITSD_ERR_INVALID, "bad schedule");
  if (u->cfg && T > u->d.T)
    return fail(ITSD_ERR_INVALID, "CFG time-embedding table has " + std::to_string(u->d.T) + " rows < sampler T");
  HIPCHK(hipSetDevice(u->device));
  drop_schedule(u);
  HIPCHK(hipMalloc(&u->coeff1, T * 4));
  HIPCHK(hipMalloc(&u->coeff2, T * 4));
  HIPCHK(hipMalloc(&u->sqrt_var, T * 4));
  HIPCHK(hipMemcpy(u->coeff1, coeff1, T * 4, hipMemcpyHostToDevice));
  HIPCHK(hipMemcpy(u->coeff2, coeff2, T * 4, hipMemcpyHostToDevice));
  HIPCHK(hipMemcpy(u->sqrt_var, sqrt_var, T * 4, hipMemcpyHostToDevice));
  HIPCHK(hipMalloc(&u->temb_table, (size_t)T * u->sumC * 4));
  CHK(alloc_rows(u, T));
  CHK(temb_rows(u, nullptr, T, 0, false, u->temb_table, u->stream));
  HIPCHK(hipStreamSynchronize(u->stream));
  u->T_sched = T;
  u->guide_w = w;
  u->guide_w1 = (float)(1.0 + (double)w);
  return ITSD_OK;
}

int itsd_set_schedule_x0(itsd_unet* u, const itsd_x0_schedule* sc) {
  if (!sc) return fail(ITSD_ERR_INVALID, "itsd_set_schedule_x0: null schedule");
  if (!sc->tau || !sc->a0 || !sc->b0 || !sc->c0 || !sc->cx || !sc->sg)
    return fail(ITSD_ERR_INVALID, "itsd_set_schedule_x0: null table");
  const int K = sc->K;
  if (K < 1) return fail(ITSD_ERR_INVALID, "itsd_set_schedule_x0: K = " + std::to_string(K) + " < 1");
  for (int k = 0; k < K; ++k)
    if (sc->tau[k] < 0 || (k && sc->tau[k] <= sc->tau[k - 1]))
      return fail(ITSD_ERR_INVALID, "itsd_set_schedule_x0: tau[" + std::to_string(k) + "] = " +
                                        std::to_string(sc->tau[k]) + ": timesteps must be >= 0 and strictly increasing");
  if (sc->clip_x0 != 0 && sc->clip_x0 != 1)
    return fail(ITSD_ERR_INVALID, "itsd_set_schedule_x0: clip_x0 = " + std::to_string(sc->clip_x0) + " is neither 0 nor 1");
  if (!u) return fail(ITSD_ERR_INVALID, "itsd_set_schedule_x0: null handle");
  if (u->cfg && sc->tau[K - 1] >= u->d.T)
    return fail(ITSD_ERR_INVALID, "CFG time-embedding table has " + std::to_string(u->d.T) + " rows <= timestep " +
                                      std::to_string(sc->tau[K - 1]));
  HIPCHK(hipSetDevice(u->device));
  drop_schedule(u);
  HIPCHK(hipMalloc(&u->xrow, (size_t)5 * K * 4));
  const float* rows[5] = {sc->a0, sc->b0, sc->c0, sc->cx, sc->sg};
  for (int i = 0; i < 5; ++i) HIPCHK(hipMemcpy(u->xrow + (size_t)i * K, rows[i], (size_t)K * 4, hipMemcpyHostToDevice));
  HIPCHK(hipMalloc(&u->temb_table, (size_t)K * u->sumC * 4));
  CHK(alloc_rows(u, K));
  int* d_tau = nullptr;
  HIPCHK(hipMalloc(&d_tau, (size_t)K * 4));
  int rc = ITSD_OK;
  if (hipMemcpy(d_tau, sc->tau, (size_t)K * 4, hipMemcpyHostToDevice) != hipSuccess) rc = fail(ITSD_ERR_HIP, "tau upload");
  if (rc == ITSD_OK) rc = temb_rows(u, d_tau, K, 0, false, u->temb_table, u->stream);
// ... 5 lines not shown
  u->clip_x0 = sc->clip_x0;
  u->guide_w = sc->w;
  u->guide_w1 = (float)(1.0 + (double)sc->w);
  return ITSD_OK;
}

int itsd_sampler_run(itsd_unet* u, float* x, const int32_t* labels, int n, int t_begin, int t_end, uint64_t seed,
                     int64_t noise_offset, const float* noise, uint32_t flags, void* stream) {
  if (!u || !x) return fail(ITSD_ERR_INVALID, "null argument");
  if (!u->T_sched) return fail(ITSD_ERR_INVALID, "itsd_set_schedule not called");
  if (u->cfg && !labels) return fail(ITSD_ERR_INVALID, "CFG sampler needs labels");
  CHK(check_batch(u, n));
  if (t_begin >= u->T_sched || t_end < 0 || t_end > t_begin) return fail(ITSD_ERR_INVALID, "bad step range");
  hipStream_t cs = (hipStream_t)stream;
  hipStream_t s = u->stream;
  CHK(enter_stream(u, cs));
  u->last_forward_n = 0;
  const int clip_at = (flags & ITSD_RUN_CLIP) ? t_end : -1;
  const size_t xbytes = (size_t)n * 3 * u->H * u->H * 4;
  HIPCHK(hipMemcpyAsync(u->x_state, x, xbytes, hipMemcpyDeviceToDevice, s));
  if (labels) HIPCHK(hipMemcpyAsync(u->lab_state, labels, (size_t)n * 4, hipMemcpyDeviceToDevice, s));

  RunCtx c = step_ctx(u, n, u->x_state, labels ? u->lab_state : nullptr);
  TailArgs& t = c.tail;
  t.step_mode = u->sched_form ? 3 : 1; t.tsel = u->d_t;
  t.coeff1 = u->coeff1; t.coeff2 = u->coeff2; t.sqrt_var = u->sqrt_var;
  if (u->sched_form) {
    for (int i = 0; i < 5; ++i) t.xrow[i] = u->xrow + (size_t)i * u->T_sched;
    t.clip_x0 = u->clip_x0;
  }
  t.noise = noise; t.run = u->d_run; t.nan_flag = u->d_nan;

  RunParams rp{};
  rp.seed = seed; rp.noise_offset = noise_offset; rp.clip_at = clip_at;
  HIPCHK(launch_run_begin(u->d_t, t_begin, u->d_nan, u->d_run, rp, s));
  const int steps = t_begin - t_end + 1;
  if (flags & ITSD_RUN_GRAPH) {
    hipGraphExec_t exec = nullptr;
    CHK(step_graph(u, c, n, labels != nullptr, noise, &exec));
    for (int i = 0; i < steps; ++i) HIPCHK(hipGraphLaunch(exec, s));
  } else {
    const std::vector<ConvLaunch> convs = resolve_program(u, c);
    for (int i = 0; i < steps; ++i) {
      CHK(run_program(u, c, convs, s));
      HIPCHK(launch_add_int(u->d_t, -1, s));
    }
  }
  HIPCHK(hipMemcpyAsync(x, u->x_state, xbytes, hipMemcpyDeviceToDevice, s));
  CHK(leave_stream(u, cs));
  if (flags & ITSD_RUN_SYNC) {
    HIPCHK(hipStreamSynchronize(s));
    int flag[2] = {0, 0};
    HIPCHK(hipMemcpy(flag, u->d_nan, 8, hipMemcpyDeviceToHost));
    if (flag[1]) return fail(ITSD_ERR_HANDOFF, handoff_msg(flag[1]));
    if (flag[0]) return fail(ITSD_ERR_NAN, "nan in tensor.");
  }
  return ITSD_OK;
}

int itsd_sampler_predict_x0(itsd_unet* u, const float* x, const int32_t* labels, int n, int t, float a0, float b0,
                            float* x0, void* stream) {
  if (!u || !x || !x0) return fail(ITSD_ERR_INVALID, "null argument");
  if (!u->T_sched) return fail(ITSD_ERR_INVALID, "itsd_set_schedule not called");
  if (u->cfg && !labels) return fail(ITSD_ERR_INVALID, "CFG sampler needs labels");
  CHK(check_batch(u, n));
  if (t < 0 || t >= u->T_sched)
    return fail(ITSD_ERR_INVALID, "step " + std::to_string(t) + " outside [0, T_sched=" + std::to_string(u->T_sched) + ")");
  hipStream_t cs = (hipStream_t)stream;
  hipStream_t s = u->stream;
  CHK(enter_stream(u, cs));
  u->last_forward_n = 0;
  RunCtx c = step_ctx(u, n, const_cast<float*>(x), labels);
  c.tail.step_mode = 2; c.tail.a0 = a0; c.tail.b0 = b0; c.tail.x0_out = x0;
  HIPCHK(launch_set_int(u->d_t, t, s));
  HIPCHK(hipMemsetAsync(u->d_nan + 1, 0, 4, s));
  CHK(run_program(u, c, resolve_program(u, c), s));
  return leave_stream(u, cs);
}

int itsd_branch(float* dst, const float* src, const int32_t* parents, int n_src, int n_dst, int64_t per_cand, float a,
                float b, uint64_t seed, uint32_t stream_id, int64_t cand_offset, void* stream) {
  if (!dst || !src || !parents) return fail(ITSD_ERR_INVALID, "itsd_branch: null argument");
  if (n_src < 1 || n_dst < 0 || per_cand < 1)
    return fail(ITSD_ERR_INVALID, "itsd_branch: needs n_src >= 1, n_dst >= 0, per_cand >= 1");
  if (n_dst == 0) return ITSD_OK;
  for (int j = 0; j < n_dst; ++j)
    if (parents[j] < 0 || parents[j] >= n_src)
      return fail(ITSD_ERR_INVALID, "itsd_branch: parents[" + std::to_string(j) + "] = " + std::to_string(parents[j]) +
                                        " outside [0, n_src=" + std::to_string(n_src) + ")");
  {
    const uintptr_t d0 = (uintptr_t)dst, s0 = (uintptr_t)src;
    const uintptr_t db = (uintptr_t)n_dst * (uintptr_t)per_cand * 4, sb = (uintptr_t)n_src * (uintptr_t)per_cand * 4;
    if (d0 < s0 + sb && s0 < d0 + db) return fail(ITSD_ERR_INVALID, "itsd_branch: dst and src overlap");
  }
  HIPCHK(launch_branch(dst, src, parents, n_dst, per_cand, a, b, seed, stream_id, cand_offset, (hipStream_t)stream));
  return ITSD_OK;
}

int itsd_verify(int kind, const float* images, int n_cand, int b, int c, int h, int w, double* scores, void* stream) {
  if (!images || !scores || n_cand < 1 || b < 1) return fail(ITSD_ERR_INVALID, "bad verify arguments");
  if (kind < 0 || kind > 3) return fail(ITSD_ERR_INVALID, "unknown verifier kind");
  if (kind == ITSD_VERIFY_SELFSUP && (c * 64 > 192 || h % 8 || w % 8 || b > 64))
    return fail(ITSD_ERR_INVALID, "selfsup verifier needs c<=3, h,w divisible by 8, b<=64");
  HIPCHK(launch_verify(kind, images, n_cand, b, c, h, w, scores, nullptr, (hipStream_t)stream));
  return ITSD_OK;
}

int itsd_verify_paired(const float* images, const float* ref_features, int n_cand, int c, int h, int w,
                       double* scores, void* stream) {
  if (!images || !ref_features || !scores || n_cand < 1) return fail(ITSD_ERR_INVALID, "bad verify arguments");
  if (c * 64 > 192 || h % 8 || w % 8) return fail(ITSD_ERR_INVALID, "paired selfsup needs c<=3, h,w divisible by 8");
  HIPCHK(launch_verify(4, images, n_cand, 1, c, h, w, scores, ref_features, (hipStream_t)stream));
  return ITSD_OK;
}

int itsd_attention(const void* qkv, const void* vt, void* out, int n, int S, int C, int precision, void* stream) {
  if (!qkv || !out || n < 1 || S < 1 || C < 1) return fail(ITSD_ERR_INVALID, "bad attention arguments");
  if (precision != ITSD_PREC_FP32 && precision != ITSD_PREC_BF16) return fail(ITSD_ERR_INVALID, "precision");
  AttnArgs a{};
  a.qkv = qkv; a.out = out; a.S = S; a.C = C;
  a.scale = (float)std::pow((double)C, -0.5);
  if (precision == ITSD_PREC_BF16) {
    if (C % 8) return fail(ITSD_ERR_INVALID, "C must be a multiple of 8");
    if (vt) {
      if (S % 16 || C % 64 || (S > 256 && !attn_flash_ok(S, C) && !attn_cs_ok(S, C)))
        return fail(ITSD_ERR_INVALID, "MFMA attention needs S % 16 == 0, C % 64 == 0 (S > 256: S % 32 == 0 with C in "
                                      "{64,128,256}, or S % 64 == 0 with C in {256,384,512,1024})");
      a.vt = vt;
    }
    HIPCHK(launch_attn<bf16_t>(a, n, (hipStream_t)stream));
  } else {
    if (C % 4) return fail(ITSD_ERR_INVALID, "C must be a multiple of 4");
    HIPCHK(launch_attn<float>(a, n, (hipStream_t)stream));
  }
  return ITSD_OK;
}

int itsd_noise(float* out, const float* pivot, int n_cand, int64_t per_cand, float scale, uint64_t seed,
               uint32_t stream_id, int64_t cand_offset, void* stream) {
  if (!out || n_cand < 0 || per_cand < 1) return fail(ITSD_ERR_INVALID, "bad noise arguments");
  if (n_cand == 0) return ITSD_OK;
  HIPCHK(launch_noise(out, pivot, n_cand, per_cand, scale, seed, stream_id, cand_offset, (hipStream_t)stream));
  return ITSD_OK;
}

int itsd_profile_forward(itsd_unet* u, const float* x, const int32_t* t, int n, double* conv_ms, double* conv_flops,
                         int* conv_launches, double* total_ms, void* stream) {
  if (!u || !x || !t) return fail(ITSD_ERR_INVALID, "null argument");
  if (u->cfg) return fail(ITSD_ERR_INVALID, "profile_forward: DDPM only");
  hipStream_t s = u->stream;
  ProfileScratch p;
  CHK(p.begin(u, t, n, (hipStream_t)stream));
  RunCtx c = forward_ctx(u, n, x, nullptr, p.eps);
  p.census(c, false);
  int r = run_program(u, c, resolve_program(u, c), s);
  hipError_t e = hipStreamSynchronize(s);
  CHK(r);
  HIPCHK(e);
  double cm = 0, cf = 0, tm = 0;
  int cl = 0;
  for (size_t i = 0; i < p.evs.size(); ++i) {
    float ms = 0.f;
    hipEventElapsedTime(&ms, p.evs[i].first, p.evs[i].second);
    tm += ms;
    if (p.kinds[i] == OP_CONV || p.kinds[i] == kCensusConvGN || p.kinds[i] == kCensusConvGNW ||
        p.kinds[i] == kCensusConvGNW4) {
      cm += ms; cf += p.fl[i]; ++cl;
    }
  }
  if (conv_ms) *conv_ms = cm;
  if (conv_flops) *conv_flops = cf;
  if (conv_launches) *conv_launches = cl;
  if (total_ms) *total_ms = tm;
  return ITSD_OK;
}

int itsd_profile_op(itsd_unet* u, const float* x, const int32_t* t, int n, int op_index, int reps, double* ms,
                    void* stream) {
  if (!u || !x || !t || !ms || reps < 1) return fail(ITSD_ERR_INVALID, "null argument or reps < 1");
  if (op_index < 1 || op_index > (int)u->ops.size()) return fail(ITSD_ERR_INVALID, "profile_op: op_index out of range");
  hipStream_t s = u->stream;
  ProfileScratch p;
  CHK(p.begin(u, t, n, (hipStream_t)stream));
  const RunCtx c = forward_ctx(u, n, x, p.lab0, p.eps);
  const std::vector<ConvLaunch> convs = resolve_program(u, c);
  CHK(run_program(u, c, convs, s));
  p.evs.push_back({nullptr, nullptr});
  hipEvent_t &e0 = p.evs[0].first, &e1 = p.evs[0].second;
  HIPCHK(hipEventCreate(&e0));
  HIPCHK(hipEventCreate(&e1));
  const Op& o = u->ops[op_index - 1];
  const ConvLaunch* cl = &convs[op_index - 1];
  CHK(launch_op(u, o, c, cl, s));
  HIPCHK(hipEventRecord(e0, s));
  for (int i = 0; i < reps; ++i) CHK(launch_op(u, o, c, cl, s));
  HIPCHK(hipEventRecord(e1, s));
  HIPCHK(hipStreamSynchronize(s));
  float m = 0.f;
  HIPCHK(hipEventElapsedTime(&m, e0, e1));
  *ms = (double)m / reps;
  return ITSD_OK;
}

int itsd_profile_ops(itsd_unet* u, const float* x, const int32_t* t, int n, int max_ops, int* kinds, double* ms,
                     double* flops, int* shapes, int* n_ops, void* stream) {
  if (!u || !x || !t || !n_ops) return fail(ITSD_ERR_INVALID, "null argument");
  hipStream_t s = u->stream;
  ProfileScratch p;
  CHK(p.begin(u, t, n, (hipStream_t)stream));
  RunCtx c = forward_ctx(u, n, x, p.lab0, p.eps);
  p.census(c, true);
  const std::vector<ConvLaunch> convs = resolve_program(u, c);
  int r = run_program(u, c, convs, s);
  hipError_t e = hipStreamSynchronize(s);
  CHK(r);
  HIPCHK(e);
  int k = 0;
  for (size_t i = 0; i < p.evs.size() && k < max_ops; ++i, ++k) {
    const int op = p.eop[i];
    float m = 0.f;
    hipEventElapsedTime(&m, p.evs[i].first, p.evs[i].second);
    if (kinds) kinds[k] = (p.kid[i] << 8) | (p.kinds[i] & 0xff);
    if (ms) ms[k] = m;
    if (flops) flops[k] = p.fl[i];
    if (shapes) {
      int* sh = shapes + 8 * k;
      for (int q = 0; q < 8; ++q) sh[q] = 0;
      sh[6] = op;
      if (op >= 1) {
        const Op& o = u->ops[op - 1];
        const Act& out = u->acts[o.dst >= 0 ? o.dst : o.src1];
        const Act& in = u->acts[o.src1];
        sh[0] = n * out.H * out.W;
        sh[1] = o.kind == OP_CONV ? o.Cout : out.C;
        sh[2] = o.kind == OP_CONV ? o.K : in.C + (o.src2 >= 0 ? u->acts[o.src2].C : 0);
        sh[3] = out.H;
        sh[4] = o.ksize;
        sh[5] = o.stride * 10 + o.upsample;
        sh[7] = (o.resid >= 0 ? 1 : 0) | (out.stats != SIZE_MAX ? 2 : 0) | (o.coef != SIZE_MAX ? 4 : 0);
        const ConvLaunch& cl = convs[op - 1];
        if (cl.p.sc_split) sh[7] = (sh[7] & ~1) | ((cl.a.sc_C1 + cl.a.sc_C2) << 8);
      }
    }
  }
  *n_ops = k;
  return ITSD_OK;
}

int itsd_unet_op_info(itsd_unet* u, int pass, int n, int op_index, itsd_op_info* info) {
  if (!u || !info) return fail(ITSD_ERR_INVALID, "null argument");
  if (pass != ITSD_PASS_FORWARD && pass != ITSD_PASS_STEP) return fail(ITSD_ERR_INVALID, "op_info: unknown pass");
  const int nops = (int)u->ops.size();
  if (op_index < 0 || op_index > nops + 1)
    return fail(ITSD_ERR_INVALID, "op_info: op_index outside [0, ops + 1 = " + std::to_string(nops + 1) + "]");
  CHK(check_batch(u, n));
  itsd_op_info r;
  std::memset(&r, 0, sizeof(r));
  r.launched = 1;
  r.src1 = r.src2 = r.dst = r.resid = r.vt = r.temb_col = r.kernel = -1;
  auto name = [&r](const std::string& s) { std::snprintf(r.name, sizeof(r.name), "%s", s.c_str()); };
  if (op_index == 0) {
    r.kind = ITSD_OP_HEAD;
    r.dst = u->head_out;
    r.ksize = 3; r.stride = 1; r.pad = 1; r.Cout = u->ch; r.K = 27;
    name("head");
  } else if (op_index == nops + 1) {
    r.kind = ITSD_OP_TAIL;
    r.src1 = u->tail_in;
    r.dst = u->tail_g;
    r.has_coef = u->tail_wmf != SIZE_MAX;
    r.silu = 1;
    r.ksize = 3; r.stride = 1; r.pad = 1; r.Cout = 3; r.K = 9 * u->acts[u->tail_in].C;
    name("tail");
  } else {
    const RunCtx c = pass == ITSD_PASS_STEP ? step_ctx(u, n, nullptr, nullptr) : forward_ctx(u, n, nullptr, nullptr, nullptr);
    const std::vector<ConvLaunch> rp = resolve_program(u, c);
    const int oi = op_index - 1;
    const Op& o = u->ops[oi];
    r.kind = o.kind == OP_GN ? ITSD_OP_GN : o.kind == OP_CONV ? ITSD_OP_CONV : o.kind == OP_ATTN ? ITSD_OP_ATTN
             : o.kind == OP_GNCOEF ? ITSD_OP_GNCOEF : ITSD_OP_ATTNBLOCK;
    r.src1 = o.src1; r.src2 = o.src2; r.dst = o.dst; r.resid = o.resid; r.vt = o.vt;
    r.silu = o.silu;
    r.S = o.S; r.C = o.C;
    r.tag = o.tag;
    name(o.name);
    if (const int into = folded_into(u, rp, (size_t)oi); into >= 0) { r.launched = 0; r.folded_into = into + 1; }
    if (o.kind == OP_GNCOEF) r.has_coef = 1;
    if (o.kind == OP_CONV) {
      const ConvLaunch& cl = rp[oi];
      if (cl.rc != ITSD_OK) return fail(cl.rc, cl.err);
      r.ksize = o.ksize; r.stride = o.stride; r.pad = o.pad; r.upsample = o.upsample; r.zins = o.zins;
      r.subpix = o.subpix; r.Cout = o.Cout; r.K = o.K; r.temb_col = o.temb_col; r.vt_from = o.vt_from;
      r.kernel = (int)cl.p.kernel;
      r.ksplit = cl.p.ksplit; r.sc_split = cl.p.sc_split; r.kS = cl.p.S;
      r.epilogue = cl.p.epilogue ? 1 : 0;
      r.gn_fold = cl.a.gn_fold;
      r.gn_out_op = cl.a.gn_out ? o.gn_next + 1 : 0;
      r.sc_op = cl.p.sc_split ? o.sc_op + 1 : 0;
      r.has_coef = o.coef != SIZE_MAX;
    }
  }
  *info = r;
  return ITSD_OK;
}

int itsd_unet_act_info(const itsd_unet* u, int act, itsd_act_info* info) {
  if (!u || !info) return fail(ITSD_ERR_INVALID, "null argument");
  itsd_act_info r;
  std::memset(&r, 0, sizeof(r));
  if (act == ITSD_ACT_PROJ) {
    r.H = r.W = 1; r.C = u->sumC; r.elem_size = 4; r.capacity = u->d.max_batch;
  } else {
    if (act < 0 || act >= (int)u->acts.size())
      return fail(ITSD_ERR_INVALID, "act_info: act outside [0, " + std::to_string(u->acts.size()) + ")");
    const Act& A = u->acts[act];
    r.H = A.H; r.W = A.W; r.C = A.C; r.elem_size = (int)u->esz; r.capacity = u->nb_max;
    r.has_stats = A.stats != SIZE_MAX;
    r.spi = stat_spi(A.H * A.W, A.spi);
  }
  *info = r;
  return ITSD_OK;
}

int itsd_unet_read(itsd_unet* u, int what, int id, int n, void* dst, int64_t bytes, void* stream) {
  if (!u || !dst) return fail(ITSD_ERR_INVALID, "null argument");
  const char* src = nullptr;
  int64_t want = 0;
  int cap = u->nb_max;
  if (what == ITSD_READ_ACT || what == ITSD_READ_STATS) {
    if (id < 0 || id >= (int)u->acts.size())
      return fail(ITSD_ERR_INVALID, "read: act outside [0, " + std::to_string(u->acts.size()) + ")");
    const Act& A = u->acts[id];
    if (what == ITSD_READ_ACT) {
      src = u->ws + A.off;
      want = (int64_t)A.H * A.W * A.C * (int64_t)u->esz;
    } else {
      if (A.stats == SIZE_MAX) return fail(ITSD_ERR_INVALID, "read: activation " + std::to_string(id) + " has no statistics slab");
      src = u->ws + A.stats;
      want = (int64_t)stat_spi(A.H * A.W, A.spi) * 2 * A.C * 4;
    }
  } else if (what == ITSD_READ_COEF) {
    const int nops = (int)u->ops.size();
    if (id == nops + 1 && u->tail_coef != SIZE_MAX) {
      src = u->ws + u->tail_coef;
      want = (int64_t)u->acts[u->tail_in].C * 2 * 4;
    } else if (id >= 1 && id <= nops && u->ops[id - 1].kind == OP_GNCOEF) {
      const Op& o = u->ops[id - 1];
      src = u->ws + o.coef;
      want = (int64_t)(u->acts[o.src1].C + (o.src2 >= 0 ? u->acts[o.src2].C : 0)) * 2 * 4;
    } else {
      return fail(ITSD_ERR_INVALID, "read: op " + std::to_string(id) + " has no coef buffer");
    }
  } else if (what == ITSD_READ_PROJ) {
    src = (const char*)u->proj_buf;
    want = (int64_t)u->sumC * 4;
    cap = u->d.max_batch;
  } else {
    return fail(ITSD_ERR_INVALID, "read: unknown buffer class " + std::to_string(what));
  }
  if (n < 1 || n > cap) return fail(ITSD_ERR_INVALID, "read: n outside [1, " + std::to_string(cap) + "]");
  want *= n;
  if (bytes != want)
    return fail(ITSD_ERR_INVALID, "read: bytes = " + std::to_string(bytes) + ", the buffer holds " + std::to_string(want));
// ... 18 lines not shown
```

inference-time-scaling-for-diffusion-models-beyond-scaling-denoising-steps_amd/csrc/common.h:

```cpp
#pragma once

#include <hip/hip_runtime.h>
#include <stdint.h>

namespace itsd {

extern int g_conv_variant;
extern int g_small_conv;
extern int g_splitk;
extern int g_conv_dbg;
extern int g_gn_wide;
extern int g_attn_cs;
extern int g_attn_aq;
extern int g_p4_w;
extern int g_num_cus;
extern int g_splitk_inl;
extern int g_p4_plain;
extern int g_conv1x1;
extern int g_small_8x8;
extern int g_small_wide;
extern int g_attn_wide_nq;
extern int g_attn_wide;
extern int g_small_minks;
extern int g_convt_prune;
// ... 10 lines not shown
extern int g_p5_c64;
extern int g_spin_bound;
extern int g_attn_split;
extern int g_gn_fold;
extern int g_fuse_gn;
extern thread_local const char* g_last_kernel;
int kernel_id(const char* name);
#define ITSD_LAUNCH(K, ...)                                    \
  do {                                                         \
    if (!::itsd::g_last_kernel) ::itsd::g_last_kernel = #K;    \
    hipLaunchKernelGGL(K, __VA_ARGS__);                        \
  } while (0)

typedef uint16_t bf16_t;

constexpr long long kTicketCap = 16384;

constexpr int kGnGroups = 32;
constexpr float kGnEps = 1e-5f;

typedef __attribute__((ext_vector_type(8))) short bf16x8;
typedef __attribute__((ext_vector_type(4))) float f32x4;
typedef __attribute__((ext_vector_type(16))) float f32x16;
typedef __attribute__((ext_vector_type(4))) uint32_t u32x4;

__device__ __forceinline__ float bf2f(bf16_t u) { return __uint_as_float(((uint32_t)u) << 16); }
__device__ __forceinline__ bf16_t f2bf(float f) {
  __bf16 b = (__bf16)f;
  return __builtin_bit_cast(bf16_t, b);
}

__device__ __forceinline__ uint32_t pk_bf16(float lo, float hi) {
  typedef float f2v __attribute__((ext_vector_type(2)));
  typedef __bf16 b2v __attribute__((ext_vector_type(2)));
  const b2v r = __builtin_convertvector((f2v){lo, hi}, b2v);
  return __builtin_bit_cast(uint32_t, r);
}

template <typename T> struct Elem;
template <> struct Elem<float> {
  static __device__ __forceinline__ float load(const float* p) { return *p; }
  static __device__ __forceinline__ float to(float v) { return v; }
  static __device__ __forceinline__ float tof(float v) { return v; }
};
template <> struct Elem<bf16_t> {
  static __device__ __forceinline__ float load(const bf16_t* p) { return bf2f(*p); }
  static __device__ __forceinline__ bf16_t to(float v) { return f2bf(v); }
  static __device__ __forceinline__ float tof(bf16_t v) { return bf2f(v); }
};

__device__ __forceinline__ float silu(float x) { return x / (1.0f + __expf(-x)); }

__device__ __forceinline__ float wave_sum(float v) {
#pragma unroll
  for (int o = 32; o > 0; o >>= 1) v += __shfl_xor(v, o, 64);
  return v;
}
__device__ __forceinline__ double wave_sum_d(double v) {
#pragma unroll
  for (int o = 32; o > 0; o >>= 1) v += __shfl_xor(v, o, 64);
  return v;
}
__device__ __forceinline__ float wave_max(float v) {
#pragma unroll
  for (int o = 32; o > 0; o >>= 1) v = fmaxf(v, __shfl_xor(v, o, 64));
  return v;
}

struct ConvArgs {
  const void* src1;
  const void* src2;
  int C1, C2;
  int Hin, Win, Hout, Wout;
  int ksize, stride, pad, upsample;
  int zins;
  const void* wt;
  const void* wfrag;
  int Cout, K;
  const float* bias;
  const float* temb;
  const int* temb_tsel;
  long long temb_row_stride, temb_img_stride;
  const float* cemb;
  const int* cemb_labels;
  long long cemb_row_stride;
  int cemb_label_mod;
  int cemb_uncond_from;
  const void* resid;
  void* out;
  int M;
  float* stats;
  const void* zero;
  void* vt_out;
  int vt_from;
  float* splitk_ws;
  long long splitk_cap;
  const float* gn_coef;
  int subpix;
  int dbg;
  int xcd;
  int tap_live;
  int ksplit;
  int* tickets;
  int gn_fold;
  const float* gn_st1;
  const float* gn_st2;
  int gn_spi1, gn_spi2;
  const float* gn_gamma;
  const float* gn_beta;
  const void* sc_src1;
  const void* sc_src2;
  int sc_C1, sc_C2, sc_split;
  const void* sc_wfrag;
  int kdist;
  int kpub;
  int kxl;
  int* err;
  int spin_bound;
  void* gn_out;
  const float* go_gamma;
  const float* go_beta;
  int go_silu;
};

enum class ConvKernel {
  P5,
  P5_SHARED,
  P4_GN,
  P4_C96,
  P4_PLAIN,
  P4_SUB,
  P4_CONVT,
  GN128,
  STREAM1X1,
  SMALL,
  PIPE_LIN,
  PIPE,
  PIPE_SUBPIX,
  IGEMM,
};
struct ConvPlan {
  bool valid = true;
  ConvKernel kernel = ConvKernel::IGEMM;
  dim3 grid;
  int block = 256;
  int ksplit = 1, sc_split = 0, cb = 128, kdist = 0, kpub = 0, kxl = 0;
  int S = 1;
  bool inl = true, epilogue = false;
  int gn_segs = 0;
  int wide_segs = 0;
};
ConvPlan plan_conv(const ConvArgs& a, bool bf16);

__host__ __device__ inline int stat_slot_px(int HW) { return HW < 128 ? HW : 128; }
__host__ __device__ inline int stat_spi(int HW, int spi) { return spi > 0 ? spi : HW / stat_slot_px(HW); }

struct GNArgs {
  const void* src1; const void* src2;
  const float* st1; const float* st2;
  int C1, C2, HW;
  int spi1, spi2;
  const float* gamma; const float* beta;
  float eps;
  int silu;
  void* dst;
  int chunks_per_block;
};

struct AttnArgs {
  const void* qkv;
  const void* vt;
  void* out;
  int S, C;
  float scale;
};

struct AttnBlockArgs {
  const bf16_t* x;
  const float* st;
  int spi;
  const float* gamma; const float* beta;
  const bf16_t* wmv;
  const float* buv;
  const float* bp;
  bf16_t* out;
  float* out_stats;
  float scale;
  int n;
  int S;
  float* spart;
  int* sync;
  int* err;
  int spin_bound;
};

struct HeadArgs {
  const float* x;
  const float* w;
  const float* b;
  void* out;
  int H, W, Cout, n;
  int x_img_mod;
  float* stats;
  const bf16_t* wmf;
};

struct RunParams {
  unsigned long long seed;
  long long noise_offset;
  int clip_at;
  int pad_;
};

struct TailArgs {
  const void* g;
  const float* w;
  const float* b;
  int H, W, C, n;
  int cfg;
  float guide_w;
  float guide_w1;
  int step_mode;
  float* eps_out;
  float* x;
  const int* tsel;
  const float* coeff1; const float* coeff2; const float* sqrt_var;
  const float* noise;
  const RunParams* run;
  int* nan_flag;
  const float* coef;
  const bf16_t* wmf;
  float a0, b0;
  float* x0_out;
  const float* xrow[5];
  int clip_x0;
};

constexpr int kBranchChunk = 256;

}
```

inference-time-scaling-for-diffusion-models-beyond-scaling-denoising-steps_amd/csrc/conv.hip:

```cpp
#include <algorithm>
#include <type_traits>

#include "common.h"

namespace itsd {

constexpr int CONV_BM = 128;
constexpr int CONV_BN = 128;
constexpr int ROWB = 128;
constexpr int TILEB = 128 * ROWB;
constexpr int EROW = 132;
constexpr int EPI_BYTES = 128 * EROW * 4 + 8 * 2 * 128 * 4;
constexpr int SMEM_BYTES = (2 * 2 * TILEB > EPI_BYTES) ? 2 * 2 * TILEB : EPI_BYTES;
int g_fuse_gn = 1;
int g_conv_dbg = 0;
int g_conv_variant = 2;
int g_small_conv = 1;
int g_conv1x1 = 1;
int g_small_8x8 = 1;
int g_small_wide = 1;
int g_splitk = 1;
int g_gn_wide = 1;
int g_p4_w = 7;
int g_num_cus = 256;
// ... 1132 lines not shown
        bfg[j] = *(const bf16x8*)(halo + h * ROWB + (((2 * kk + hh) ^ ((h >> 1) & 7)) << 4));
      }
#pragma unroll
      for (int i = 0; i < 2; ++i)
#pragma unroll
        for (int j = 0; j < 2; ++j)
          acc[i][j] = __builtin_amdgcn_mfma_f32_32x32x16_bf16(af[i], bfg[j], acc[i][j], 0, 0, 0);
    }
  };

  zero_acc(acc);
  load_chunk(0);
  issue_w(0);
  issue_w(1);
  wait_vmcnt<8>();
  write_halo();
  asm volatile("s_waitcnt lgkmcnt(0)" ::: "memory");
  auto run_chunk = [&](int cc, auto stage) {
    constexpr bool ST = decltype(stage)::value;
    const int s0 = cc * 9;
    wait_vmcnt<4>();
    __builtin_amdgcn_s_barrier();
    issue_w(s0 + 2);
    if constexpr (ST) {
      asm volatile("" ::: "memory");
      load_chunk(cc + 1);
      asm volatile("" ::: "memory");
    }
    mma_tap(s0, 0);
#pragma unroll 1
    for (int tap = 1; tap < 8; ++tap) {
      if (ST && tap <= 2) wait_vmcnt<4 + LPC>();
      else wait_vmcnt<4>();
      __builtin_amdgcn_s_barrier();
      issue_w(s0 + tap + 2);
      mma_tap(s0 + tap, tap);
    }
    wait_vmcnt<4>();
    __builtin_amdgcn_s_barrier();
    issue_w(s0 + 10);
    mma_tap(s0 + 8, 8);
    if constexpr (ST) {
      asm volatile("s_waitcnt lgkmcnt(0)" ::: "memory");
      __builtin_amdgcn_s_barrier();
      write_halo();
      asm volatile("s_waitcnt lgkmcnt(0)" ::: "memory");
    }
  };
  for (int cc = 0; cc + 1 < ncc; ++cc) run_chunk(cc, std::true_type{});
  run_chunk(ncc - 1, std::false_type{});
  wait_vmcnt<0>();
  __syncthreads();
  if (a.dbg & 16) return;
  conv_epilogue<T>(a, acc, smem, tileP, tileC);
}

#ifdef ITSD_STAMPS
__device__ unsigned long long g_stamps[1024 * 16 * 8];
__device__ __forceinline__ unsigned long long stamp() {
  __builtin_amdgcn_sched_barrier(0);
  const unsigned long long t = __builtin_amdgcn_s_memtime();
  __builtin_amdgcn_sched_barrier(0);
  return t;
}
#define STAMP(var) const unsigned long long var = stamp()
#define STAMP_ADD(slot, d) st[slot] += (d)
__device__ __forceinline__ void tl_stamp(int slot) {
  __builtin_amdgcn_sched_barrier(0);
  const unsigned long long t = (threadIdx.x >> 6) == 1 ? __builtin_amdgcn_s_memtime() : __builtin_amdgcn_s_memrealtime();
  if ((threadIdx.x & 63) == 0) g_stamps[((blockIdx.x & 1023) * 16 + (threadIdx.x >> 6)) * 8 + slot] = t;
  __builtin_amdgcn_sched_barrier(0);
}
#define TL(slot) tl_stamp(slot)
#else
#define TL(slot)
#define STAMP(var)
#define STAMP_ADD(slot, d)
#endif
constexpr int GNW_BN = 256;
constexpr int GNW_EPI = GNW_BN * EROW * 4 + (GNW_BN / 16) * 2 * CONV_BM * 4;
constexpr int GNW_SMEM = 160 * 1024;
static_assert(GNW_EPI <= GNW_SMEM, "epilogue tile");

constexpr float GN_L2E = -1.44269504f;
__device__ __forceinline__ float gn_silu_l2(float x, float a2, float b2) {
  const float t = __builtin_fmaf(x, a2, b2);
  return t * __builtin_amdgcn_rcpf(__builtin_fmaf(__builtin_amdgcn_exp2f(t), GN_L2E, GN_L2E));
}
__device__ __forceinline__ void gn_silu_x4(uint32_t xa, uint32_t xb, float a0, float a1, float a2, float a3,
                                           float b0, float b1, float b2, float b3, uint32_t zm, uint32_t& ya,
                                           uint32_t& yb) {
  float t0, t1, t2, t3, e0, e1, e2, e3;
  asm volatile(
      "v_lshlrev_b32 %2, 16, %10\n\t"
      "v_and_b32 %3, 0xffff0000, %10\n\t"
      "v_lshlrev_b32 %4, 16, %11\n\t"
      "v_and_b32 %5, 0xffff0000, %11\n\t"
      "v_fma_f32 %2, %2, %12, %16\n\t"
      "v_fma_f32 %3, %3, %13, %17\n\t"
      "v_fma_f32 %4, %4, %14, %18\n\t"
      "v_fma_f32 %5, %5, %15, %19\n\t"
      "v_exp_f32 %6, %2\n\t"
      "v_exp_f32 %7, %3\n\t"
      "v_exp_f32 %8, %4\n\t"
      "v_exp_f32 %9, %5\n\t"
      "v_fma_f32 %6, %6, %21, %21\n\t"
      "v_fma_f32 %7, %7, %21, %21\n\t"
      "v_fma_f32 %8, %8, %21, %21\n\t"
      "v_fma_f32 %9, %9, %21, %21\n\t"
      "v_rcp_f32 %6, %6\n\t"
      "v_rcp_f32 %7, %7\n\t"
      "v_rcp_f32 %8, %8\n\t"
      "v_rcp_f32 %9, %9\n\t"
      "v_mul_f32 %2, %2, %6\n\t"
      "v_mul_f32 %3, %3, %7\n\t"
      "v_mul_f32 %4, %4, %8\n\t"
      "v_mul_f32 %5, %5, %9\n\t"
      "v_cvt_pk_bf16_f32 %0, %2, %3\n\t"
      "v_cvt_pk_bf16_f32 %1, %4, %5\n\t"
      "v_and_b32 %0, %0, %20\n\t"
      "v_and_b32 %1, %1, %20"
      : "=&v"(ya), "=&v"(yb), "=&v"(t0), "=&v"(t1), "=&v"(t2), "=&v"(t3), "=&v"(e0), "=&v"(e1), "=&v"(e2),
        "=&v"(e3)
      : "v"(xa), "v"(xb), "v"(a0), "v"(a1), "v"(a2), "v"(a3), "v"(b0), "v"(b1), "v"(b2), "v"(b3), "v"(zm),
        "s"(GN_L2E));
}

template <int W> struct GnpCfg;
template <> struct GnpCfg<32> { static constexpr int NSEG = 1, ITEMS = 11, RES = 1; };
template <> struct GnpCfg<16> { static constexpr int NSEG = 1, ITEMS = 11, RES = 1; };
template <> struct GnpCfg<8> { static constexpr int NSEG = 4, ITEMS = 13, RES = 0; };


#ifndef ITSD_P4_M16
#define ITSD_P4_M16 2
#endif
#ifndef ITSD_P4_ZR8
#define ITSD_P4_ZR8 1
#endif
#ifndef ITSD_P5_SC_LAUNCH
#define ITSD_P5_SC_LAUNCH 7.5
#endif
#ifndef ITSD_P5_SWZ
#define ITSD_P5_SWZ 1
#endif
#ifndef ITSD_P4_SUBSWZ
#define ITSD_P4_SUBSWZ 1
#endif
#ifndef ITSD_P4_HSWZ
#define ITSD_P4_HSWZ 1
#endif
constexpr int P4_RING = 6;
constexpr int P4_BD = 2;
template <int W, int AB = 0>
__global__ __launch_bounds__(512, 1) void conv3x3_gn_p4_kernel(ConvArgs a) {
  typedef bf16_t T;
  constexpr bool SUB = (AB & 128) != 0, PLAIN = SUB || (AB & 2) != 0;
  constexpr bool SUB4 = SUB && (AB & 256) == 0;
  constexpr int NTAP = SUB4 ? 4 : 9, KST = 4 * NTAP;
  constexpr bool COMPACT = !SUB && (W == 8 || W == 16);
  constexpr int NSEG = GnpCfg<W>::NSEG, ITEMS = COMPACT ? 8 : GnpCfg<W>::ITEMS, RES = COMPACT ? 1 : GnpCfg<W>::RES;
  constexpr int W2 = W + 2;
  constexpr int THs = NSEG == 1 ? GNW_BN / W : W;
  constexpr int HS = (THs + 2) * W2;
  constexpr int HWs = THs * W;
  constexpr int TPS = 256 / NSEG, RPP = TPS / 8;
  constexpr int ZROW = GNW_BN;
  constexpr bool M16 = ITSD_P4_M16 >= 1 && RES && !SUB && (AB & 1) == 0 && (W == 32 || ITSD_P4_M16 >= 2);
  constexpr int ZROWS = COMPACT ? (M16 ? (ITSD_P4_ZR8 ? 72 : 65) : 1) : 0;
  auto hswz = [](int h) { return M16 && ITSD_P4_HSWZ ? (h & 6) : ((h >> 1) & 7); };
  constexpr bool CSWZ = ITSD_P4_SUBSWZ && !COMPACT && !M16 && W <= 16;
  constexpr int SC1 = 1, SC2 = W <= 8 ? 2 : 1;
  constexpr bool C96 = (AB & 512) != 0;
  constexpr int BM = C96 ? 96 : CONV_BM, HB = BM / 2, NCI = HB / 16;
  static_assert(!C96 || (M16 && COMPACT), "96-cout tiles: the 16x16x32 compact forms");
  constexpr int HALO = COMPACT ? (((GNW_BN + ZROWS) * ROWB + 1023) & ~1023) : NSEG * ITEMS * RPP * ROWB;
  constexpr int RESB = RES ? GNW_BN * CONV_BM * 2 : 0;
  static_assert(COMPACT ? ITEMS * RPP == HWs : ITEMS * RPP >= HS, "halo items cover the segment");
  constexpr int RING = ((AB & 64) || SUB) ? 4 : P4_RING, BD = (AB & 32) ? P4_BD + 1 : P4_BD;
  static_assert(KST % RING == 0, "ring slots repeat per chunk");
  __shared__ __attribute__((aligned(16))) char smem[2 * HALO + RESB + 2 * NSEG * CONV_BM * 4 + 4 * 64 * 4];
  char* const rlds = smem + 2 * HALO;
  float* const addv = (float*)(smem + 2 * HALO + RESB);
#ifdef ITSD_STAMPS
  {
    const unsigned hw = __builtin_amdgcn_s_getreg(4 | (4 << 6) | (1 << 11));
    if ((threadIdx.x & 63) == 0) g_stamps[((blockIdx.x & 1023) * 16 + 8 + (threadIdx.x >> 6)) * 8 + 1] = hw;
  }
#endif
  const int tid = threadIdx.x, lane = tid & 63;
  const int wid = __builtin_amdgcn_readfirstlane(tid >> 6);
  const int H = a.Hout;
  const int Cin = a.C1 + a.C2, ncc = Cin / 64, kpt = Cin >> 4;
  const int nTC = a.Cout / BM, nPT = a.M / GNW_BN, NT = (SUB ? 4 : 1) * nPT * nTC;
  const int G = gridDim.x;
  const int b = (a.xcd && (G & 7) == 0) ? (int)(blockIdx.x & 7) * (G >> 3) + (int)(blockIdx.x >> 3) : (int)blockIdx.x;
  const int tb0 = (int)(((long long)b * NT) / G);
  const int ntiles = (int)(((long long)(b + 1) * NT) / G) - tb0;
  const int nstages = ntiles * ncc;
  constexpr bool CT = SUB && !SUB4;
  const int Q = nPT * nTC;
  auto tile_r = [&](int k) -> int {
    const int t = tb0 + k;
    if constexpr (!SUB) return t;
    if (CT && a.tap_live) return (t - (t >= 2 * Q ? 2 * Q : 0)) >> 1;
    return t % Q;
  };
  auto tile_p = [&](int k) { return (tile_r(k) / nTC) * GNW_BN; };
  auto tile_c = [&](int k) { return (tile_r(k) % nTC) * BM; };
  auto tile_ph = [&](int k) -> int {
    const int t = tb0 + k;
    if constexpr (!SUB) return 0;
    if (CT && a.tap_live) return t >= 2 * Q ? 1 + ((t - 2 * Q) & 1) : 3 * (t & 1);
    return t / Q;
  };
  auto orow = [&](int p, int ph) -> size_t {
    if constexpr (!SUB) return (size_t)p;
    const int HWi = H * W, img = p / HWi, rem = p - img * HWi, i = rem / W, j = rem - i * W;
    return ((size_t)img * 2 * H + 2 * i + (ph >> 1)) * (2 * W) + 2 * j + (ph & 1);
  };
#ifdef ITSD_STAMPS
  unsigned long long st[8] = {0, 0, 0, 0, 0, 0, 0, 0};
  const unsigned long long t_begin = stamp();
  auto stamps_out = [&]() {
    st[7] = stamp() - t_begin;
    if (lane == 0) {
      const int bb = blockIdx.x & 1023;
#pragma unroll
      for (int qq = 0; qq < 8; ++qq) g_stamps[(bb * 16 + wid) * 8 + qq] = st[qq];
    }
  };
#define P4_STAMP_OUT() stamps_out()
#else
#define P4_STAMP_OUT()
#endif
  auto block_sync = [&]() {
    STAMP(b0);
    asm volatile("s_waitcnt lgkmcnt(0)" ::: "memory");
    __builtin_amdgcn_s_barrier();
    asm volatile("" ::: "memory");
    STAMP(b1);
    STAMP_ADD(1, b1 - b0);
  };
  if (ntiles == 0) return;
  auto stage_addv = [&](int k, int t0) {
    const int tileP = tile_p(k), tileC = tile_c(k), img0 = tileP / (H * W);
    const long long trow = a.temb ? (a.temb_tsel ? (long long)(*a.temb_tsel) * a.temb_row_stride : 0) : 0;
    for (int it = t0; it < NSEG * BM; it += 256) {
      const int il = it / BM, cl = it - il * BM, co = tileC + cl, img = img0 + il;
      float v = a.bias[co];
      if (a.temb) v += a.temb[trow + (long long)img * a.temb_img_stride + co];
      if (a.cemb) {
        int lab = 0;
        if (a.cemb_uncond_from < 0 || img < a.cemb_uncond_from) lab = a.cemb_labels[img % a.cemb_label_mod];
        v += a.cemb[(long long)lab * a.cemb_row_stride + co];
      }
      addv[(k & 1) * NSEG * BM + it] = v;
    }
  };

  if (wid < 4) {
    if constexpr (M16) {
    const int wm = wid & 1, wn = wid >> 1, m = lane & 15, kg = lane >> 4;
    static_assert(COMPACT || (W == 32 && NSEG == 1), "halo rows of the 16-pixel blocks from one base");
    const int hb0 = COMPACT ? wn * 128 + m : wn * 4 * W2 + m;
    const uint32_t ablk = (uint32_t)(NTAP * kpt) * 1024;
    const __amdgpu_buffer_rsrc_t wrs = __builtin_amdgcn_make_buffer_rsrc((void*)a.wfrag, (short)0, 0x7fffffff, 0x00020000);
    const uint32_t avo0 = (uint32_t)((kg >> 1) * 1024 + (m + 32 * (kg & 1)) * 16) + 2 * wm * ablk, avo1 = avo0 + ablk;
    auto abase_of = [&](int k) -> uint32_t { return (uint32_t)(tile_c(k) >> 5) * ablk; };
    constexpr int KS2 = 2 * NTAP, RING2 = 3;
    static_assert(KS2 % RING2 == 0, "ring slots repeat per chunk");
    f32x4 acc[NCI][8];
#pragma unroll
    for (int i = 0; i < NCI; ++i)
#pragma unroll
      for (int j = 0; j < 8; ++j) acc[i][j] = f32x4{0.f, 0.f, 0.f, 0.f};
    u32x4 ra[RING2][NCI];
    const uint32_t avl = (uint32_t)((kg >> 1) * 1024 + (m + 32 * (kg & 1)) * 16);
    auto fo96 = [&](int b) -> uint32_t { return (uint32_t)((3 * wm + b) >> 1) * ablk + (uint32_t)((3 * wm + b) & 1) * 256; };
    auto load_a = [&](uint32_t base, int st, u32x4 (&dst)[NCI], int hf) __attribute__((always_inline)) {
      const uint32_t off = base + (uint32_t)((st >> 1) * kpt + 2 * (st & 1)) * 1024;
      if constexpr ((AB & 8) != 0) {
#pragma unroll
        for (int b = 2 * hf; b < 2 * hf + 2; ++b)
          if (b < NCI) dst[b] = u32x4{(uint32_t)st, (uint32_t)b, 0u, 0u};
      } else if constexpr (C96) {
#pragma unroll
        for (int b = 2 * hf; b < 2 * hf + 2; ++b)
          if (b < NCI) dst[b] = __builtin_amdgcn_raw_buffer_load_b128(wrs, avl, off + fo96(b), 0);
      } else {
        const uint32_t vo = hf ? avo1 : avo0;
        dst[2 * hf] = __builtin_amdgcn_raw_buffer_load_b128(wrs, vo, off, 0);
        dst[2 * hf + 1] = __builtin_amdgcn_raw_buffer_load_b128(wrs, vo + 256, off, 0);
      }
    };
    {
      const uint32_t ab0 = abase_of(0);
#pragma unroll
      for (int s0 = 0; s0 < RING2 - 1; ++s0) {
        load_a(ab0, s0, ra[s0], 0);
        load_a(ab0, s0, ra[s0], 1);
      }
    }
    auto init_acc = [&](int kk) __attribute__((always_inline)) {
#pragma unroll
      for (int j = 0; j < 8; ++j) {
        const int seg = NSEG == 1 ? 0 : (wn * 128 + j * 16) / HWs;
#pragma unroll
        for (int i = 0; i < NCI; ++i)
          acc[i][j] = *(const f32x4*)(addv + ((kk & 1) * NSEG + seg) * BM + wm * HB + 16 * i + 4 * kg);
      }
    };
    stage_addv(0, tid);
    block_sync();
    init_acc(0);
    int q = 0;
    for (int k = 0; k < ntiles; ++k) {
      const uint32_t ab = abase_of(k);
      const uint32_t abn = k + 1 < ntiles ? abase_of(k + 1) : ab;
      for (int cc = 0; cc < ncc; ++cc, ++q) {
        const char* hcur = smem + (q & 1) * HALO;
        const uint32_t nb = cc + 1 < ncc ? ab + (uint32_t)(cc + 1) * 4 * 1024 : abn;
        const uint32_t cb = ab + (uint32_t)cc * 4 * 1024;
        STAMP(c0);
        auto half_sched = [&]() __attribute__((always_inline)) {
#pragma unroll
          for (int g = 0; g < 2; ++g) {
            __builtin_amdgcn_sched_group_barrier(0x008, 1, 0);
            __builtin_amdgcn_sched_group_barrier(0x020, 1, 0);
            __builtin_amdgcn_sched_group_barrier(0x002, 2, 0);
          }
#pragma unroll
          for (int g = 0; g < 4; ++g) {
            __builtin_amdgcn_sched_group_barrier(0x008, 1, 0);
            __builtin_amdgcn_sched_group_barrier(0x100, 1, 0);
            __builtin_amdgcn_sched_group_barrier(0x002, 2, 0);
          }
#pragma unroll
          for (int g = 0; g < 10; ++g) {
            __builtin_amdgcn_sched_group_barrier(0x008, 1, 0);
            __builtin_amdgcn_sched_group_barrier(0x002, 2, 0);
          }
          __builtin_amdgcn_sched_barrier(0);
// ... 349 lines not shown
          if (!has_res) rr = uint2{0u, 0u};
          float v[4];
          v[0] = acc[i][j][4 * g + 0] + ad[0] + __uint_as_float(rr.x << 16);
          v[1] = acc[i][j][4 * g + 1] + ad[1] + __uint_as_float(rr.x & 0xffff0000u);
          v[2] = acc[i][j][4 * g + 2] + ad[2] + __uint_as_float(rr.y << 16);
          v[3] = acc[i][j][4 * g + 3] + ad[3] + __uint_as_float(rr.y & 0xffff0000u);
          const T b0 = f2bf(v[0]), b1 = f2bf(v[1]), b2 = f2bf(v[2]), b3 = f2bf(v[3]);
          wv[g][0] = (uint32_t)b0 | ((uint32_t)b1 << 16);
          wv[g][1] = (uint32_t)b2 | ((uint32_t)b3 << 16);
          const float r0 = bf2f(b0), r1 = bf2f(b1), r2 = bf2f(b2), r3 = bf2f(b3);
          s16[4 * g + 0] += r0; q16[4 * g + 0] = fmaf(r0, r0, q16[4 * g + 0]);
          s16[4 * g + 1] += r1; q16[4 * g + 1] = fmaf(r1, r1, q16[4 * g + 1]);
          s16[4 * g + 2] += r2; q16[4 * g + 2] = fmaf(r2, r2, q16[4 * g + 2]);
          s16[4 * g + 3] += r3; q16[4 * g + 3] = fmaf(r3, r3, q16[4 * g + 3]);
        }
#pragma unroll
        for (int gp = 0; gp < 4; gp += 2) {
          u32x4 o;
#pragma unroll
          for (int d = 0; d < 2; ++d) {
            const auto sw = __builtin_amdgcn_permlane32_swap(wv[gp][d], wv[gp + 1][d], false, false);
            o[d] = sw[0];
            o[2 + d] = sw[1];
          }
          const int c8 = wmi * 32 + 8 * (gp + hh);
          *(u32x4*)((T*)a.out + orow(tileP + p, tph) * a.Cout + tileC + c8) = o;
        }
        if (a.stats && ((NSEG == 1 && j == 3) || (NSEG != 1 && (j & 1)))) {
          float v[32];
#pragma unroll
          for (int e = 0; e < 16; ++e) {
            v[e] = s16[e];
            v[16 + e] = q16[e];
          }
          auto xchg = [](float x, auto wc) {
            constexpr int w = decltype(wc)::value;
            const int xi = __builtin_bit_cast(int, x);
            int r;
            if constexpr (w == 1) r = __builtin_amdgcn_update_dpp(0, xi, 0xB1, 0xF, 0xF, false);
            else if constexpr (w == 2) r = __builtin_amdgcn_update_dpp(0, xi, 0x4E, 0xF, 0xF, false);
            else if constexpr (w == 8) r = __builtin_amdgcn_update_dpp(0, xi, 0x128, 0xF, 0xF, false);
            else r = __builtin_amdgcn_ds_swizzle(xi, 0x1F | (w << 10));
            return __builtin_bit_cast(float, r);
          };
          auto halve = [&](auto wc) {
            constexpr int w = decltype(wc)::value;
            const bool up = (rl & w) != 0;
#pragma unroll
            for (int ii = 0; ii < w; ++ii) {
              const float lo = v[ii], hi = v[ii + w];
              v[ii] = (up ? hi : lo) + xchg(up ? lo : hi, wc);
            }
          };
          halve(std::integral_constant<int, 16>{});
          halve(std::integral_constant<int, 8>{});
          halve(std::integral_constant<int, 4>{});
          halve(std::integral_constant<int, 2>{});
          halve(std::integral_constant<int, 1>{});
          {
            constexpr int SLOT = NSEG == 1 ? 128 : 64;
            long long slot = (long long)(tileP + wn * 128 + (NSEG == 1 ? 0 : (j >> 1) * 64)) / SLOT;
            if constexpr (SUB) slot = slot * 4 + tph;
            const int e = rl & 15, co = wmi * 32 + 8 * (e >> 2) + 4 * hh + (e & 3);
            a.stats[(slot * 2 + (rl >> 4)) * a.Cout + tileC + co] = v[0];
          }
#pragma unroll
          for (int e = 0; e < 16; ++e) s16[e] = q16[e] = 0.f;
        }
      }
      }
      } else {
        float sm = 0.f;
#pragma unroll
        for (int i = 0; i < 2; ++i)
#pragma unroll
          for (int j = 0; j < 4; ++j)
#pragma unroll
            for (int r = 0; r < 16; ++r) sm += acc[i][j][r];
        if (sm == 1.2345f) ((float*)a.out)[0] = sm;
      }
      if constexpr (RES) {
        if (k + 1 < ntiles) init_acc(k + 1);
      } else {
#pragma unroll
        for (int i = 0; i < 2; ++i)
#pragma unroll
          for (int j = 0; j < 4; ++j)
#pragma unroll
            for (int r = 0; r < 16; ++r) acc[i][j][r] = 0.0f;
      }
      STAMP(e1);
      STAMP_ADD(6, e1 - e0);
    }
    if constexpr (RES) block_sync();
    P4_STAMP_OUT();
    return;
    }
  }

  const int tt = tid - 256, lch = tt & 7, sg = tt / TPS, lt = tt - sg * TPS;
  static_assert(COMPACT || NSEG * ITEMS * RPP > NSEG * HS, "a scratch row exists");
  if (a.dbg & (1 << 20)) __builtin_amdgcn_s_setprio(1);
  if (a.dbg & (1 << 21)) __builtin_amdgcn_s_setprio(2);
  const int dump = NSEG * HS * ROWB + (lch << 4);
  const int hrow0 = (COMPACT ? sg * HWs : sg * HS) + (lt >> 3), hrow1 = hrow0 + RPP;
  const int lds0 = hrow0 * ROWB + ((lch ^ hswz(hrow0)) << 4);
  const int lds1 = hrow1 * ROWB + ((lch ^ hswz(hrow1)) << 4);
  auto item_lds = [&](int j) {
    if constexpr (CSWZ) {
      const int r = (lt >> 3) + RPP * j, hy = r / W2, hx = r - hy * W2;
      return (sg * HS + r) * ROWB + ((lch ^ ((SC1 * hy + SC2 * hx) & 7)) << 4);
    }
    return ((j & 1) ? lds1 : lds0) + (j >> 1) * (2 * RPP * ROWB);
  };
  auto tile_y0img = [&](int k, int& img0, int& y0) {
    const int tileP = tile_p(k);
    img0 = tileP / (H * W);
    y0 = (tileP - img0 * H * W) / W;
  };
  int ipix[ITEMS];
  const float* cbase;
  int simg = 0;
  int gimg = -1;
  float* const gsw = (float*)(smem + 2 * HALO + RESB + 2 * NSEG * CONV_BM * 4) + (wid - 4) * 64;
  auto group_stats = [&](int img) __attribute__((always_inline)) {
    const int g = lane & 31, hf = Cin / 64, c0 = g * 2 * hf + (lane >> 5) * hf;
    const int HWi = H * W;
    const int sp1 = stat_spi(HWi, a.gn_spi1), sp2 = a.C2 ? stat_spi(HWi, a.gn_spi2) : 0;
    const int spm = sp1 > sp2 ? sp1 : sp2, np = hf >> 1, m = np * spm;
    double sm = 0.0, sq = 0.0;
    for (int b0 = 0; b0 < m; b0 += 8) {
      float2 vs[8], vq[8];
#pragma unroll
      for (int i = 0; i < 8; ++i) {
        const int it = b0 + i, q = it / np, cr = c0 + 2 * (it - q * np);
        const bool s1 = cr < a.C1;
        const bool ok = it < m && q < (s1 ? sp1 : sp2);
        const int c = ok ? cr : c0, qq = ok ? q : 0;
        const bool t1 = c < a.C1;
        const float* st = t1 ? a.gn_st1 : a.gn_st2;
        const int Cs = t1 ? a.C1 : a.C2, cs = t1 ? c : c - a.C1, sp = t1 ? sp1 : sp2;
        const long long slot = (long long)img * sp + qq;
        const float2 u0 = *(const float2*)(st + (slot * 2) * Cs + cs);
        const float2 u1 = *(const float2*)(st + (slot * 2 + 1) * Cs + cs);
        vs[i] = ok ? u0 : float2{0.f, 0.f};
        vq[i] = ok ? u1 : float2{0.f, 0.f};
      }
#pragma unroll
      for (int i = 0; i < 8; ++i) {
        sm += (double)vs[i].x + (double)vs[i].y;
        sq += (double)vq[i].x + (double)vq[i].y;
      }
    }
    sm += __shfl_xor(sm, 32, 64);
    sq += __shfl_xor(sq, 32, 64);
    const double E = (double)(Cin / 32) * HWi, mean = sm / E;
    double var = sq / E - mean * mean;
    var = var > 0.0 ? var : 0.0;
    if (lane < 32) {
      gsw[2 * g] = (float)mean;
      gsw[2 * g + 1] = (float)(1.0 / sqrt(var + 1e-5));
    }
  };
  auto geometry_pix = [&](int k) __attribute__((always_inline)) {
    int img0, y0;
    tile_y0img(k, img0, y0);
    int ltv = lt;
    asm volatile("" : "+v"(ltv));
#pragma unroll
    for (int j = 0; j < ITEMS; ++j) {
      const int r = (ltv >> 3) + RPP * j;
      if constexpr (COMPACT) {
        ipix[j] = (img0 + sg) * HWs + r;
      } else {
        const int hy = r / W2, hx = r - hy * W2, iy = y0 + hy - 1, ix = hx - 1;
        const bool ok = r < HS && iy >= 0 && iy < H && ix >= 0 && ix < W;
        ipix[j] = ok ? ((img0 + sg) * H + iy) * W + ix : 0;
      }
    }
    if constexpr (!PLAIN) cbase = a.gn_coef + ((size_t)(img0 + sg) * (Cin / 8) + lch) * 16;
    simg = img0 + sg;
  };
  static_assert(COMPACT || ITEMS * RPP - HS < RPP, "scratch rows only in the last item");
  const int waddr_last = (COMPACT || ((lt >> 3) + RPP * (ITEMS - 1)) < HS) ? item_lds(ITEMS - 1) : dump;
  auto waddr = [&](int j) { return j == ITEMS - 1 ? waddr_last : item_lds(j); };
  int inm = 0;
  auto geometry_emit = [&](int k) __attribute__((always_inline)) {
    int img0, y0;
    tile_y0img(k, img0, y0);
    int ltv = lt;
    asm volatile("" : "+v"(ltv));
    inm = 0;
    if constexpr (COMPACT) {
      inm = (1 << ITEMS) - 1;
      return;
    }
#pragma unroll
    for (int j = 0; j < ITEMS; ++j) {
      const int r = (ltv >> 3) + RPP * j;
      const int hy = r / W2, hx = r - hy * W2, iy = y0 + hy - 1, ix = hx - 1;
      const bool in = r >= HS || (iy >= 0 && iy < H && ix >= 0 && ix < W);
      inm |= (int)in << j;
    }
  };
  const int nrec1 = (int)std::min<long long>((long long)a.M * a.C1 * 2, 0x7fffffffLL);
  const int nrec2 = (int)std::min<long long>((long long)a.M * a.C2 * 2, 0x7fffffffLL);
  struct Src {
    __amdgpu_buffer_rsrc_t rs;
    uint32_t rowb, so;
  };
  auto src_of = [&](int cc, bool live) __attribute__((always_inline)) {
    const int ci0 = cc * 64;
    const bool s1 = ci0 < a.C1;
    Src c;
    c.rs = __builtin_amdgcn_make_buffer_rsrc(s1 ? (void*)a.src1 : (void*)a.src2, (short)0,
                                             live ? (s1 ? nrec1 : nrec2) : 0, 0x00020000);
    c.rowb = (uint32_t)(s1 ? a.C1 : a.C2) * 2;
    c.so = (uint32_t)(s1 ? ci0 : ci0 - a.C1) * 2;
    return c;
  };
  const int dh = (wid - 4) & 1, ds = (wid - 4) >> 1;
  auto res_dma = [&](int k) __attribute__((always_inline)) {
    if constexpr (RES) {
      const int tileP = tile_p(k), tileC = tile_c(k);
#pragma unroll
      for (int i = 0; i < 16; ++i) {
        const int row = 128 * ds + 8 * i + (lane >> 3), u = (lane & 7) ^ ((row >> 1) & 7);
        const int us = (C96 && u >= HB / 8) ? 0 : u;
        const T* src = (const T*)a.resid + (size_t)(tileP + row) * a.Cout + tileC + dh * HB + us * 8;
        __builtin_amdgcn_global_load_lds((const void*)src, (lds_ptr_t)(rlds + dh * 32768 + (128 * ds + 8 * i) * 128), 16, 0, 0);
      }
    }
  };
  auto drain = [&](int kd) __attribute__((always_inline)) {
    if constexpr (RES) {
      int lane = tid & 63;
      asm volatile("" : "+v"(lane));
      const int tileP = tile_p(kd), tileC = tile_c(kd), u = lane & 7, dph = tile_ph(kd);
      constexpr int NH = NSEG == 4 ? 2 : 1;
#pragma unroll
      for (int hf = 0; hf < NH; ++hf) {
        float v[16];
#pragma unroll
        for (int e = 0; e < 16; ++e) v[e] = 0.f;
#pragma unroll
        for (int i = hf * 16 / NH; i < (hf + 1) * 16 / NH; ++i) {
          const int row = 128 * ds + 8 * i + (lane >> 3);
          u32x4 d = *(const u32x4*)(rlds + dh * 32768 + row * 128 + ((u ^ ((row >> 1) & 7)) << 4));
          if (!C96 || u < HB / 8) *(u32x4*)((T*)a.out + orow(tileP + row, dph) * a.Cout + tileC + dh * HB + u * 8) = d;
          else d = u32x4{0u, 0u, 0u, 0u};
#pragma unroll
          for (int w = 0; w < 4; ++w) {
            const float lo = __uint_as_float(d[w] << 16), hi = __uint_as_float(d[w] & 0xffff0000u);
            v[2 * w] += lo;
            v[2 * w + 1] += hi;
            v[8 + 2 * w] = fmaf(lo, lo, v[8 + 2 * w]);
            v[8 + 2 * w + 1] = fmaf(hi, hi, v[8 + 2 * w + 1]);
          }
        }
        if (a.stats) {
          auto xchg = [&](float x, auto wc) {
            constexpr int w = decltype(wc)::value;
            const int xi = __builtin_bit_cast(int, x);
            int r;
            if constexpr (w == 8) r = __builtin_amdgcn_update_dpp(0, xi, 0x128, 0xF, 0xF, false);
            else if constexpr (w == 16) r = __builtin_amdgcn_ds_swizzle(xi, 0x1F | (16 << 10));
            else r = __builtin_amdgcn_ds_bpermute((lane ^ 32) << 2, xi);
            return __builtin_bit_cast(float, r);
          };
          auto halve = [&](auto wc, int n) {
            const bool up = (lane & decltype(wc)::value) != 0;
#pragma unroll
            for (int ii = 0; ii < 8; ++ii) {
              if (ii < n) {
                const float lo = v[ii], hi = v[ii + n];
                v[ii] = (up ? hi : lo) + xchg(up ? lo : hi, wc);
              }
            }
          };
          halve(std::integral_constant<int, 8>{}, 8);
          halve(std::integral_constant<int, 16>{}, 4);
          halve(std::integral_constant<int, 32>{}, 2);
          long long slot = NH == 1 ? (long long)tileP / 128 + ds : ((long long)tileP + 128 * ds + 64 * hf) / 64;
          if constexpr (SUB) {
            const int HWi = H * W, spp = HWi / 128, img = tileP / HWi;
            slot = (long long)img * 4 * spp + dph * spp + (tileP - img * HWi) / 128 + ds;
          }
          const int co = dh * HB + 8 * u + 4 * ((lane >> 4) & 1) + 2 * (lane >> 5);
          if (!C96 || u < HB / 8) *(float2*)(a.stats + (slot * 2 + ((lane >> 3) & 1)) * a.Cout + tileC + co) = float2{v[0], v[1]};
        }
      }
    }
  };
  int kL = 0, ccL = 0;
  u32x4 h[ITEMS];
  f32x4 c[4], cn[4];
  auto prescale = [&]() __attribute__((always_inline)) {
    if constexpr (PLAIN) return;
    if (a.gn_fold) {
      const int c0 = ccL * 64 + 8 * lch;
      const float rg = 32.0f / (float)Cin;
#pragma unroll
      for (int e = 0; e < 8; ++e) {
        const int g = (int)(((float)(c0 + e) + 0.5f) * rg);
        const float mean = gsw[2 * g], rstd = gsw[2 * g + 1];
        const float sc = rstd * cn[e >> 2][e & 3];
        c[e >> 2][e & 3] = sc * GN_L2E;
        c[2 + (e >> 2)][e & 3] = (cn[2 + (e >> 2)][e & 3] - mean * sc) * GN_L2E;
      }
    } else {
#pragma unroll
      for (int q = 0; q < 4; ++q)
#pragma unroll
        for (int e = 0; e < 4; ++e) c[q][e] = cn[q][e] * GN_L2E;
    }
  };
  auto load_cn = [&](int ccx) __attribute__((always_inline)) {
    if constexpr (PLAIN) return;
    if (a.gn_fold) {
      const int c0 = ccx * 64 + 8 * lch;
      cn[0] = *(const f32x4*)(a.gn_gamma + c0);
      cn[1] = *(const f32x4*)(a.gn_gamma + c0 + 4);
      cn[2] = *(const f32x4*)(a.gn_beta + c0);
      cn[3] = *(const f32x4*)(a.gn_beta + c0 + 4);
    } else {
      const f32x4* cp = (const f32x4*)(cbase + ccx * 128);
#pragma unroll
      for (int q = 0; q < 4; ++q) cn[q] = cp[q];
    }
  };
  auto emit = [&](char* hbuf) __attribute__((always_inline)) {
    if (ccL == 0) geometry_emit(kL);
    bool opened = false;
    if (++ccL == ncc) {
      ccL = 0;
      if (++kL < ntiles) {
        geometry_pix(kL);
        opened = true;
      }
    }
    const bool live = kL < ntiles;
    load_cn(live ? ccL : 0);
    const Src nx = src_of(ccL, live);
    typedef __attribute__((ext_vector_type(2))) float f32x2;
    typedef __attribute__((ext_vector_type(2))) __bf16 bf16x2_t;
#pragma unroll
    for (int j = 0; j < ITEMS; ++j) {
      const uint32_t zm = (uint32_t)__builtin_amdgcn_sbfe(inm, j, 1);
      uint32_t yw[4];
      if constexpr (PLAIN) {
#pragma unroll
        for (int w = 0; w < 4; ++w) yw[w] = h[j][w] & zm;
      } else
#pragma unroll
      for (int hf = 0; hf < 2; ++hf)
        gn_silu_x4(h[j][2 * hf], h[j][2 * hf + 1], c[hf][0], c[hf][1], c[hf][2], c[hf][3], c[2 + hf][0],
                   c[2 + hf][1], c[2 + hf][2], c[2 + hf][3], zm, yw[2 * hf], yw[2 * hf + 1]);
      const u32x4 y = {yw[0], yw[1], yw[2], yw[3]};
      *(u32x4*)(hbuf + waddr(j)) = y;
      __builtin_amdgcn_sched_barrier(0);
      h[j] = __builtin_amdgcn_raw_buffer_load_b128(nx.rs, __umul24((uint32_t)ipix[j], nx.rowb) + lch * 16, nx.so, 0);
    }
    if (a.gn_fold && opened && simg != gimg) {
      group_stats(simg);
      gimg = simg;
    }
    prescale();
  };
  geometry_pix(0);
  {
    load_cn(0);
    const Src s0 = src_of(0, true);
#pragma unroll
    for (int j = 0; j < ITEMS; ++j)
      h[j] = __builtin_amdgcn_raw_buffer_load_b128(s0.rs, __umul24((uint32_t)ipix[j], s0.rowb) + lch * 16, s0.so, 0);
    if (a.gn_fold) group_stats(simg);
    gimg = simg;
    prescale();
  }
  if constexpr (COMPACT) {
    if (tt < 16) *(u32x4*)(smem + (tt >> 3) * HALO + ZROW * ROWB + ((tt & 7) << 4)) = u32x4{0u, 0u, 0u, 0u};
    if (M16 && ITSD_P4_ZR8) {
      const int r = (tt >> 3) & 15;
      *(u32x4*)(smem + (tt >> 7) * HALO + (ZROW + (r & 7) + (r >> 3) * 64) * ROWB + ((tt & 7) << 4)) = u32x4{0u, 0u, 0u, 0u};
    } else if (M16 && tt >= 16 && tt < 32) {
      *(u32x4*)(smem + ((tt >> 3) & 1) * HALO + (ZROW + 64) * ROWB + ((tt & 7) << 4)) = u32x4{0u, 0u, 0u, 0u};
    }
  }
  emit(smem);
#ifdef ITSD_STAMPS
  st[5] = stamp() - t_begin;
#endif
  block_sync();
  for (int q = 0, k = 0, cc = 0; q < nstages; ++q) {
    STAMP(h0);
    if (RES && cc == 1 && k > 0) {
      drain(k - 1);
      asm volatile("s_waitcnt lgkmcnt(0)" ::: "memory");
    }
    const bool res = RES && a.resid && cc == ncc - 1;
    if (res) res_dma(k);
    const int addv_cc = RES ? 0 : ncc - 1;
    if (cc == addv_cc && k + 1 < ntiles) stage_addv(k + 1, tt);
    if (q + 1 < nstages) emit(smem + ((q + 1) & 1) * HALO);
    if (res) {
      if (q + 1 < nstages) asm volatile("s_waitcnt vmcnt(%0)" ::"n"(ITEMS + 4) : "memory");
      else asm volatile("s_waitcnt vmcnt(0)" ::: "memory");
    }
#ifdef ITSD_STAMPS
    asm volatile("s_waitcnt lgkmcnt(0)" ::: "memory");
#endif
    STAMP(h1);
    STAMP_ADD(3, h1 - h0);
    block_sync();
    if (++cc == ncc) {
      cc = 0;
      ++k;
    }
  }
  if constexpr (RES) {
    block_sync();
    drain(ntiles - 1);
  }
  P4_STAMP_OUT();
}

template <int W> struct Gp5Cfg {
  static constexpr int HW = W * W;
  static constexpr bool ROWS = HW > 128;
  static constexpr int TH = ROWS ? 128 / W : W, NSEG = ROWS ? 1 : 128 / HW, W2 = W + 2, HS = (TH + 2) * W2;
  static constexpr int HY0 = ROWS ? 0 : 1, NHY = ROWS ? TH + 2 : TH;
  static constexpr int TPS = 256 / NSEG, RPP = TPS / 8, ITEMS = NHY * W / RPP;
  static constexpr int HALO = ((NSEG * HS * ROWB) + 1023) & ~1023;
};
#ifndef ITSD_P5_RING
#define ITSD_P5_RING 9
#endif
#ifndef ITSD_P5_BD
#define ITSD_P5_BD 3
#endif
constexpr int P5_RING = ITSD_P5_RING;
constexpr int P5_BD = ITSD_P5_BD;

template <int W, int CB = 128, bool DIST = false>
__global__ __launch_bounds__(512, 1) void conv3x3_gn_p5_kernel(ConvArgs a) {
  typedef bf16_t T;
  using Cf = Gp5Cfg<W>;
  static_assert(CB == 128 || (CB == 64 && W <= 8), "p5 cout tile");
  static_assert(!DIST || CB == 128, "shared combine: 128-cout items");
  constexpr int CWB = CB / 32, NJW = CWB;
  constexpr int HW = Cf::HW, NSEG = Cf::NSEG, W2 = Cf::W2, HS = Cf::HS, TPS = Cf::TPS, RPP = Cf::RPP;
  constexpr int ITEMS = Cf::ITEMS, HALO = Cf::HALO, TH = Cf::TH, HY0 = Cf::HY0, NHY = Cf::NHY;
  constexpr int SPX = TH * W;
  constexpr int SC1 = 1, SC2 = W <= 8 ? 2 : 1;
  auto swz = [](int hy, int hx, int h) { return W <= 16 && ITSD_P5_SWZ ? (SC1 * hy + SC2 * hx) & 7 : (h >> 1) & 7; };
  static_assert(NSEG * SPX == 128 && ITEMS * RPP == NHY * W && ITEMS <= 31 && 36 % P5_RING == 0, "p5 geometry");
  constexpr int SEGW = 64 / TPS > 0 ? 64 / TPS : 1;
  constexpr int RTILE = 128 * CONV_BM * 2;
  __shared__ __attribute__((aligned(16))) char smem[2 * HALO + 2 * NSEG * CONV_BM * 4 + 4 * 2 * SEGW * 64 * 4 + 2 * RTILE];
  float* const addv = (float*)(smem + 2 * HALO);
  char* const rres = smem + 2 * HALO + 2 * NSEG * CONV_BM * 4 + 4 * 2 * SEGW * 64 * 4;
  float* const gsw_all = (float*)(smem + 2 * HALO + 2 * NSEG * CONV_BM * 4);
  TL(0);
#ifdef ITSD_STAMPS
  {
    const unsigned hw = __builtin_amdgcn_s_getreg(4 | (4 << 6) | (1 << 11));
    if ((threadIdx.x & 63) == 0) g_stamps[((blockIdx.x & 1023) * 16 + 8 + (threadIdx.x >> 6)) * 8] = hw;
  }
#endif
  const int tid = threadIdx.x, lane = tid & 63;
  const int wid = __builtin_amdgcn_readfirstlane(tid >> 6);
  const int Cin = a.C1 + a.C2, nch = Cin / 64, kpt = Cin >> 4;
  const int nimg = a.M / HW, nTP = Cf::ROWS ? a.M / 128 : (nimg + NSEG - 1) / NSEG;
  const int nTC = a.Cout / CB, S = a.ksplit;
  const int S2 = a.sc_split, ST = S + S2, nchx = (a.sc_C1 + a.sc_C2) / 64;
  const int NI = nTP * nTC * ST;
  const int G = gridDim.x, b = blockIdx.x;
  const int bl = (G & 7) ? b : (b & 7) * (G >> 3) + (b >> 3);
  const int nit = bl < NI ? (NI - 1 - bl) / G + 1 : 0;
  if (nit == 0) return;
  const bool xl = a.kxl != 0;
  const int d1 = xl ? ST : nTP, d2 = xl ? nTP : ST;
  auto item_of = [&](int k, int& tp, int& tc, int& z) {
    const int L = bl + k * G;
    const int i1 = L % d1, r = L / d1, i2 = r % d2;
    tp = xl ? i2 : i1;
    z = xl ? i1 : i2;
    tc = r / d2;
  };
  auto chunk_lo = [&](int z) { return z < S ? (nch * z) / S : (nchx * (z - S)) / S2; };
  auto chunk_hi = [&](int z) { return z < S ? (nch * (z + 1)) / S : (nchx * (z + 1 - S)) / S2; };
  auto block_sync = [&]() {
    asm volatile("s_waitcnt lgkmcnt(0)" ::: "memory");
    __builtin_amdgcn_s_barrier();
    asm volatile("" ::: "memory");
  };

  if (wid < 4) {
    const int rl = lane & 31, hh = lane >> 5;
    const int cw = CB == 128 ? wid : wid % CWB, jb0 = CB == 128 ? 0 : (wid / CWB) * NJW;
    int hb[NJW];
    int hq[NJW];
#pragma unroll
    for (int j = 0; j < NJW; ++j) {
      const int pl = (jb0 + j) * 32 + rl, seg = pl / SPX, rem = pl - seg * SPX, y = rem / W;
      hb[j] = seg * HS + y * W2 + (rem - y * W);
      hq[j] = SC1 * y + SC2 * (rem - y * W);
    }
    auto bunit = [&](int j, int h, int ky, int kx) {
      return W <= 16 && ITSD_P5_SWZ ? (hq[j] + SC1 * ky + SC2 * kx) & 7 : (h >> 1) & 7;
    };
    const uint32_t ablk = (uint32_t)(9 * kpt) * 1024;
    const __amdgpu_buffer_rsrc_t wrs = __builtin_amdgcn_make_buffer_rsrc((void*)a.wfrag, (short)0, 0x7fffffff, 0x00020000);
    const uint32_t avo = (uint32_t)lane * 16 + (uint32_t)cw * ablk;
    auto abase = [&](int tc, int cc) -> uint32_t { return (uint32_t)(tc * CWB) * ablk + (uint32_t)cc * 4 * 1024; };
    auto load_a = [&](uint32_t base, int st, u32x4& dst) __attribute__((always_inline)) {
#if defined(ITSD_DIAG) && defined(P5_AB)
      if constexpr ((P5_AB & 8) != 0) {
        dst = u32x4{(uint32_t)st, 0u, 0u, 0u};
        return;
      }
#endif
      dst = __builtin_amdgcn_raw_buffer_load_b128(wrs, avo, base + (uint32_t)((st >> 2) * kpt + (st & 3)) * 1024, 0);
    };
    f32x16 acc[NJW];
    u32x4 ra[P5_RING];
    const __amdgpu_buffer_rsrc_t wrx = __builtin_amdgcn_make_buffer_rsrc((void*)a.sc_wfrag, (short)0, 0x7fffffff, 0x00020000);
    const uint32_t ablkx = (uint32_t)(nchx * 4) * 1024;
    auto load_ax = [&](int tc, int cc, int st, u32x4& dst) __attribute__((always_inline)) {
      dst = __builtin_amdgcn_raw_buffer_load_b128(wrx, (uint32_t)lane * 16,
                                                  (uint32_t)(tc * CWB + cw) * ablkx + (uint32_t)(cc * 4 + st) * 1024, 0);
    };
    bool ring = false;
    {
      int tp, tc, z;
      item_of(0, tp, tc, z);
      if (z < S) {
        const uint32_t ab0 = abase(tc, chunk_lo(z));
#pragma unroll
        for (int s0 = 0; s0 < P5_RING - 1; ++s0) load_a(ab0, s0, ra[s0]);
        ring = true;
      }
    }
    block_sync();
    TL(1);
    int q = 0;
    for (int k = 0; k < nit; ++k) {
      int tp, tc, z;
      item_of(k, tp, tc, z);
      const int c0 = chunk_lo(z), c1 = chunk_hi(z);
#pragma unroll
      for (int j = 0; j < NJW; ++j)
#pragma unroll
        for (int r = 0; r < 16; ++r) acc[j][r] = 0.0f;
#if defined(ITSD_DIAG) && defined(P5_CHAINS2)
      f32x16 acc2[NJW];
#pragma unroll
      for (int j = 0; j < NJW; ++j)
#pragma unroll
        for (int r = 0; r < 16; ++r) acc2[j][r] = 0.0f;
#endif
      if (z >= S) {
#pragma unroll
        for (int st = 0; st < 4; ++st) load_ax(tc, c0, st, ra[st]);
        auto chunk1 = [&](auto pc, int cc) __attribute__((always_inline)) {
          constexpr int P = decltype(pc)::value;
          if (cc + 1 < c1) {
#pragma unroll
            for (int st = 0; st < 4; ++st) load_ax(tc, cc + 1, st, ra[4 * (1 - P) + st]);
          }
          int tx[NJW];
#pragma unroll
          for (int j = 0; j < NJW; ++j) {
            const int h = hb[j] + W2 + 1;
            tx[j] = (q & 1) * HALO + h * ROWB + ((hh ^ bunit(j, h, 1, 1)) << 4);
          }
#pragma unroll
// ... 1146 lines not shown
    while (S > 1 && (long long)blocks * S * 16384 > a.splitk_cap) --S;
    return S < 1 ? 1 : S;
  };
  if (a.subpix) {
    if (!pipe || !lin || (a.subpix == 2 ? (a.ksize != 3 && !(a.ksize == 1 && a.Hout * a.Wout == 1)) : a.ksize != 2) ||
        ((a.Hout * a.Wout) % 128 && 128 % (a.Hout * a.Wout))) {
      p.valid = false;
      return p;
    }
    if (bf16 && p4_sub_selected(a)) return persistent(a.subpix == 1 ? ConvKernel::P4_SUB : ConvKernel::P4_CONVT, 4 * tiles256);
    const int blocks = (int)(grid.x * grid.y) * 4;
    if (a.splitk_ws && a.tickets && g_splitk && g_splitk_inl && g_subpix_split && blocks < 256 && blocks <= kTicketCap)
      p.S = fit(std::min((512 + blocks - 1) / blocks, nK / 8), blocks);
    p.kernel = ConvKernel::PIPE_SUBPIX;
    p.grid = dim3(grid.x, grid.y, 4 * p.S);
    return p;
  }
  p.grid = grid;
  if (!pipe || g_conv_variant == 1) return p;
  p.kernel = lin ? ConvKernel::PIPE_LIN : ConvKernel::PIPE;
  if (a.splitk_ws && g_splitk) {
    const int blocks = (int)(grid.x * grid.y);
    p.inl = blocks <= kTicketCap && g_splitk_inl;
    int S = 1;
    if (g_splitk >= 2) S = std::min(g_splitk, nK / 4);
    else if (blocks < 256) S = std::min((512 + blocks - 1) / blocks, nK / 8);
    p.S = fit(S, blocks);
    p.grid.z = p.S;
    p.epilogue = p.S > 1 && !(p.inl && a.tickets);
  }
  return p;
}

#ifdef ITSD_DIAG
static hipError_t launch_p4_ablation(const ConvArgs& a, dim3 gp, hipStream_t s) {
  switch ((g_conv_dbg >> 13) & 127) {
    case 2: ITSD_LAUNCH((conv3x3_gn_p4_kernel<32, 2>), gp, dim3(512), 0, s, a); break;
    case 4: ITSD_LAUNCH((conv3x3_gn_p4_kernel<32, 4>), gp, dim3(512), 0, s, a); break;
    case 8: ITSD_LAUNCH((conv3x3_gn_p4_kernel<32, 8>), gp, dim3(512), 0, s, a); break;
    case 16: ITSD_LAUNCH((conv3x3_gn_p4_kernel<32, 16>), gp, dim3(512), 0, s, a); break;
    case 24: ITSD_LAUNCH((conv3x3_gn_p4_kernel<32, 24>), gp, dim3(512), 0, s, a); break;
    case 10: ITSD_LAUNCH((conv3x3_gn_p4_kernel<32, 10>), gp, dim3(512), 0, s, a); break;
    case 32: ITSD_LAUNCH((conv3x3_gn_p4_kernel<32, 32>), gp, dim3(512), 0, s, a); break;
    case 64: ITSD_LAUNCH((conv3x3_gn_p4_kernel<32, 64>), gp, dim3(512), 0, s, a); break;
    case 18: ITSD_LAUNCH((conv3x3_gn_p4_kernel<32, 18>), gp, dim3(512), 0, s, a); break;
    default: return hipErrorInvalidValue;
  }
  return hipGetLastError();
}

#endif

#define ITSD_GO(K) ITSD_LAUNCH(K, p.grid, dim3(p.block), 0, s, a)
#define ITSD_GO_W(K32, K16, K8)    \
  do {                             \
    if (a.Wout == 32) ITSD_GO(K32); \
    else if (a.Wout == 16) ITSD_GO(K16); \
    else ITSD_GO(K8);              \
  } while (0)

static void launch_p5(const ConvArgs& a, const ConvPlan& p, hipStream_t s) {
  if (p.kernel == ConvKernel::P5_SHARED) {
    if (a.Wout == 4) ITSD_GO((conv3x3_gn_p5_kernel<4, 128, true>));
    else ITSD_GO_W((conv3x3_gn_p5_kernel<32, 128, true>), (conv3x3_gn_p5_kernel<16, 128, true>), (conv3x3_gn_p5_kernel<8, 128, true>));
    return;
  }
  if (a.Wout == 64) ITSD_GO(conv3x3_gn_p5_kernel<64>);
#ifdef ITSD_DIAG
  else if (a.Wout == 8 && p.cb == 64) ITSD_GO((conv3x3_gn_p5_kernel<8, 64>));
  else if (a.Wout <= 8 && p.cb == 64) ITSD_GO((conv3x3_gn_p5_kernel<4, 64>));
#endif
  else if (a.Wout == 4) ITSD_GO(conv3x3_gn_p5_kernel<4>);
  else ITSD_GO_W(conv3x3_gn_p5_kernel<32>, conv3x3_gn_p5_kernel<16>, conv3x3_gn_p5_kernel<8>);
}

static void launch_stream1x1(const ConvArgs& a, const ConvPlan& p, hipStream_t s) {
  const int Cin = a.C1 + a.C2;
#define ITSD_S1(NS)                                                 \
  if (Cin == 128) ITSD_GO((conv1x1_stream_kernel<128, NS>));        \
  else if (Cin == 256) ITSD_GO((conv1x1_stream_kernel<256, NS>));   \
  else if (Cin == 384) ITSD_GO((conv1x1_stream_kernel<384, NS>));   \
  else if (Cin == 512) ITSD_GO((conv1x1_stream_kernel<512, NS>));   \
  else ITSD_GO((conv1x1_stream_kernel<640, NS>));
  if (g_conv1x1 == 2) {
    ITSD_S1(7)
  } else {
    ITSD_S1(4)
  }
#undef ITSD_S1
}

template <typename T>
hipError_t launch_conv(const ConvArgs& a0, const ConvPlan& p, hipStream_t s) {
  const bool generic = p.kernel == ConvKernel::PIPE_LIN || p.kernel == ConvKernel::PIPE ||
                       p.kernel == ConvKernel::PIPE_SUBPIX || p.kernel == ConvKernel::IGEMM;
  if (!p.valid || (a0.gn_out && p.kernel != ConvKernel::SMALL) || (a0.sc_C1 + a0.sc_C2 && !p.sc_split) ||
      (sizeof(T) != 2 && !generic))
    return hipErrorInvalidValue;
  ConvArgs a = a0;
  switch (p.kernel) {
    case ConvKernel::P5:
    case ConvKernel::P5_SHARED:
      a.ksplit = p.ksplit;
      a.sc_split = p.sc_split;
      a.kdist = p.kdist;
      a.kpub = p.kpub;
      a.kxl = p.kxl;
      launch_p5(a, p, s);
      break;
    case ConvKernel::P4_GN:
#ifdef ITSD_DIAG
      if ((g_conv_dbg & 4096) && a.Wout == 32) return launch_p4_ablation(a, p.grid, s);
#endif
      ITSD_GO_W(conv3x3_gn_p4_kernel<32>, conv3x3_gn_p4_kernel<16>, conv3x3_gn_p4_kernel<8>);
      break;
    case ConvKernel::P4_C96: ITSD_GO((conv3x3_gn_p4_kernel<8, 512>)); break;
    case ConvKernel::P4_PLAIN:
      ITSD_GO_W((conv3x3_gn_p4_kernel<32, 2>), (conv3x3_gn_p4_kernel<16, 2>), (conv3x3_gn_p4_kernel<8, 2>));
      break;
    case ConvKernel::P4_SUB:
      ITSD_GO_W((conv3x3_gn_p4_kernel<32, 128>), (conv3x3_gn_p4_kernel<16, 128>), (conv3x3_gn_p4_kernel<8, 128>));
      break;
    case ConvKernel::P4_CONVT:
      ITSD_GO_W((conv3x3_gn_p4_kernel<32, 384>), (conv3x3_gn_p4_kernel<16, 384>), (conv3x3_gn_p4_kernel<8, 384>));
      break;
    case ConvKernel::GN128:
      if (p.gn_segs == 1) ITSD_GO(conv3x3_gn_kernel<1>);
      else ITSD_GO(conv3x3_gn_kernel<2>);
      break;
    case ConvKernel::STREAM1X1: launch_stream1x1(a, p, s); break;
    case ConvKernel::SMALL: ITSD_GO(conv_small<false>); break;
    case ConvKernel::PIPE_SUBPIX: ITSD_GO((conv_pipe<T, 2, true>)); break;
    case ConvKernel::PIPE_LIN:
    case ConvKernel::PIPE:
      if (!p.inl) a.tickets = nullptr;
      if (p.kernel == ConvKernel::PIPE_LIN) ITSD_GO((conv_pipe<T, 2, true>));
      else ITSD_GO((conv_pipe<T, 2, false>));
      if (p.epilogue) {
        const hipError_t e = hipGetLastError();
        if (e != hipSuccess) return e;
        ITSD_LAUNCH(splitk_epilogue_kernel<T>, dim3(p.grid.x, p.grid.y), dim3(256), 0, s, a0, (int)p.grid.z);
      }
      break;
    case ConvKernel::IGEMM: ITSD_GO(conv_igemm<T>); break;
  }
  return hipGetLastError();
}
#undef ITSD_GO_W
#undef ITSD_GO

template hipError_t launch_conv<float>(const ConvArgs&, const ConvPlan&, hipStream_t);
template hipError_t launch_conv<bf16_t>(const ConvArgs&, const ConvPlan&, hipStream_t);

}

#ifdef ITSD_STAMPS
extern "C" int itsd_debug_stamps(unsigned long long* host) {
  if (hipDeviceSynchronize() != hipSuccess) return 1;
  return hipMemcpyFromSymbol(host, HIP_SYMBOL(itsd::g_stamps), sizeof(unsigned long long) * 1024 * 128) == hipSuccess ? 0 : 1;
}
#endif
```

inference-time-scaling-for-diffusion-models-beyond-scaling-denoising-steps_amd/runtime.py:

```python
from __future__ import annotations

import ctypes
import os
from typing import Dict, Optional, Sequence

import torch

from .arch import ARCH_CFG, ARCH_DDPM, UNetArch

_HERE = os.path.dirname(os.path.abspath(__file__))
LIB_PATH = os.environ.get("ITSD_LIB") or os.path.join(_HERE, "libitsd_hip.so")

ITSD_OK, ITSD_ERR_INVALID, ITSD_ERR_HIP, ITSD_ERR_WEIGHTS, ITSD_ERR_NAN, ITSD_ERR_OOM, ITSD_ERR_HANDOFF = range(7)
PREC_FP32, PREC_BF16 = 0, 1
VERIFY_ORACLE, VERIFY_SELFSUP, VERIFY_AESTHETIC, VERIFY_MEAN = 0, 1, 2, 3
RUN_GRAPH, RUN_CLIP, RUN_SYNC = 1, 2, 4


class ItsdError(RuntimeError):
    def __init__(self, code: int, msg: str):
        super().__init__(f"[itsd error {code}] {msg}")
        self.code = code


class UNetDesc(ctypes.Structure):
    _fields_ = [("arch", ctypes.c_int32), ("T", ctypes.c_int32), ("ch", ctypes.c_int32),
                ("n_mult", ctypes.c_int32), ("ch_mult", ctypes.c_int32 * 8), ("n_attn", ctypes.c_int32),
                ("attn", ctypes.c_int32 * 8), ("num_res_blocks", ctypes.c_int32), ("img_size", ctypes.c_int32),
                ("num_labels", ctypes.c_int32), ("max_batch", ctypes.c_int32), ("precision", ctypes.c_int32)]


class TensorView(ctypes.Structure):
    _fields_ = [("name", ctypes.c_char_p), ("data", ctypes.c_void_p), ("numel", ctypes.c_int64)]


class X0Schedule(ctypes.Structure):
    _fields_ = [("K", ctypes.c_int32), ("tau", ctypes.POINTER(ctypes.c_int32))] + \
               [(k, ctypes.POINTER(ctypes.c_float)) for k in ("a0", "b0", "c0", "cx", "sg")] + \
               [("clip_x0", ctypes.c_int32), ("w", ctypes.c_float)]


X0_ROW_KEYS = ("a0", "b0", "c0", "cx", "sg")


class OpInfo(ctypes.Structure):
    _fields_ = [(k, ctypes.c_int32) for k in (
        "kind", "launched", "folded_into", "src1", "src2", "dst", "resid", "vt", "ksize", "stride", "pad", "upsample",
        "zins", "subpix", "Cout", "K", "temb_col", "vt_from", "silu", "S", "C", "kernel", "ksplit", "sc_split", "kS",
        "epilogue", "gn_fold", "gn_out_op", "sc_op", "has_coef", "tag")] + [("name", ctypes.c_char * 96)]


class ActInfo(ctypes.Structure):
    _fields_ = [(k, ctypes.c_int32) for k in ("H", "W", "C", "elem_size", "has_stats", "spi", "capacity")]


OP_GN, OP_CONV, OP_ATTN, OP_GNCOEF, OP_ATTNBLOCK, OP_HEAD, OP_TAIL = range(7)
OP_KINDS = ("gn", "conv", "attn", "gncoef", "attnblock", "head", "tail")
TAG_NONE, TAG_QKV, TAG_DOWN_MERGE, TAG_ATTN_S1, TAG_CONVT, TAG_ATTNBLOCK = range(6)
CONV_KERNELS = ("P5", "P5_SHARED", "P4_GN", "P4_C96", "P4_PLAIN", "P4_SUB", "P4_CONVT", "GN128", "STREAM1X1", "SMALL",
                "PIPE_LIN", "PIPE", "PIPE_SUBPIX", "IGEMM")
ACT_PROJ = -2
READ_ACT, READ_STATS, READ_COEF, READ_PROJ = range(4)
PASS_FORWARD, PASS_STEP = 0, 1

_lib = None

_SIGS = {
    "itsd_unet_create": [ctypes.POINTER(UNetDesc), ctypes.POINTER(TensorView), ctypes.c_int, ctypes.c_int,
                         ctypes.POINTER(ctypes.c_void_p)],
    "itsd_unet_destroy": [ctypes.c_void_p],
    "itsd_unet_forward": [ctypes.c_void_p, ctypes.c_void_p, ctypes.c_void_p, ctypes.c_void_p, ctypes.c_void_p,
                          ctypes.c_int, ctypes.c_void_p],
    "itsd_unet_representation": [ctypes.c_void_p, ctypes.c_void_p, ctypes.c_int, ctypes.c_void_p],
    "itsd_set_schedule": [ctypes.c_void_p, ctypes.c_int, ctypes.c_void_p, ctypes.c_void_p, ctypes.c_void_p,
                          ctypes.c_float],
    "itsd_set_schedule_x0": [ctypes.c_void_p, ctypes.POINTER(X0Schedule)],
    "itsd_sampler_run": [ctypes.c_void_p, ctypes.c_void_p, ctypes.c_void_p, ctypes.c_int, ctypes.c_int, ctypes.c_int,
                         ctypes.c_uint64, ctypes.c_int64, ctypes.c_void_p, ctypes.c_uint32, ctypes.c_void_p],
    "itsd_sampler_predict_x0": [ctypes.c_void_p, ctypes.c_void_p, ctypes.c_void_p, ctypes.c_int, ctypes.c_int,
                                ctypes.c_float, ctypes.c_float, ctypes.c_void_p, ctypes.c_void_p],
    "itsd_branch": [ctypes.c_void_p, ctypes.c_void_p, ctypes.POINTER(ctypes.c_int32), ctypes.c_int, ctypes.c_int,
                    ctypes.c_int64, ctypes.c_float, ctypes.c_float, ctypes.c_uint64, ctypes.c_uint32, ctypes.c_int64,
                    ctypes.c_void_p],
    "itsd_noise": [ctypes.c_void_p, ctypes.c_void_p, ctypes.c_int, ctypes.c_int64, ctypes.c_float, ctypes.c_uint64,
                   ctypes.c_uint32, ctypes.c_int64, ctypes.c_void_p],
    "itsd_verify": [ctypes.c_int, ctypes.c_void_p, ctypes.c_int, ctypes.c_int, ctypes.c_int, ctypes.c_int,
                    ctypes.c_int, ctypes.c_void_p, ctypes.c_void_p],
    "itsd_verify_paired": [ctypes.c_void_p, ctypes.c_void_p, ctypes.c_int, ctypes.c_int, ctypes.c_int, ctypes.c_int,
                           ctypes.c_void_p, ctypes.c_void_p],
    "itsd_attention": [ctypes.c_void_p, ctypes.c_void_p, ctypes.c_void_p, ctypes.c_int, ctypes.c_int, ctypes.c_int,
                       ctypes.c_int, ctypes.c_void_p],
    "itsd_profile_forward": [ctypes.c_void_p, ctypes.c_void_p, ctypes.c_void_p, ctypes.c_int,
                             ctypes.POINTER(ctypes.c_double), ctypes.POINTER(ctypes.c_double),
                             ctypes.POINTER(ctypes.c_int), ctypes.POINTER(ctypes.c_double), ctypes.c_void_p],
    "itsd_profile_op": [ctypes.c_void_p, ctypes.c_void_p, ctypes.c_void_p, ctypes.c_int, ctypes.c_int,
                        ctypes.c_int, ctypes.POINTER(ctypes.c_double), ctypes.c_void_p],
    "itsd_profile_ops": [ctypes.c_void_p, ctypes.c_void_p, ctypes.c_void_p, ctypes.c_int, ctypes.c_int,
                         ctypes.c_void_p, ctypes.c_void_p, ctypes.c_void_p, ctypes.c_void_p,
                         ctypes.POINTER(ctypes.c_int), ctypes.c_void_p],
    "itsd_set_option": [ctypes.c_char_p, ctypes.c_int],
    "itsd_calibrate": [ctypes.c_int, ctypes.POINTER(ctypes.c_double), ctypes.c_void_p],
    "itsd_unet_query": [ctypes.c_void_p, ctypes.c_char_p, ctypes.POINTER(ctypes.c_int64)],
    "itsd_unet_op_info": [ctypes.c_void_p, ctypes.c_int, ctypes.c_int, ctypes.c_int, ctypes.POINTER(OpInfo)],
    "itsd_unet_act_info": [ctypes.c_void_p, ctypes.c_int, ctypes.POINTER(ActInfo)],
    "itsd_unet_read": [ctypes.c_void_p, ctypes.c_int, ctypes.c_int, ctypes.c_int, ctypes.c_void_p, ctypes.c_int64,
                       ctypes.c_void_p],
    "itsd_unet_poison": [ctypes.c_void_p, ctypes.c_void_p],
    "itsd_kernel_name": [ctypes.c_int],
    "itsd_last_error": [],
    "itsd_version": [],
}

EXPORTS = tuple(_SIGS)


def lib():
    global _lib
    if _lib is None:
        if not os.path.exists(LIB_PATH):
            raise ItsdError(ITSD_ERR_INVALID, f"{LIB_PATH} is not built; run __graft_entry__.build()")
        L = ctypes.CDLL(LIB_PATH)
        shipped = os.path.abspath(LIB_PATH) == os.path.join(_HERE, "libitsd_hip.so")
        for name, args in _SIGS.items():
            if not shipped and not hasattr(L, name):
                continue
            f = getattr(L, name)
            f.argtypes = args
            f.restype = ctypes.c_char_p if name in ("itsd_last_error", "itsd_kernel_name") else ctypes.c_int
        _lib = L
    return _lib


def check(rc: int) -> None:
    if rc != ITSD_OK:
        msg = lib().itsd_last_error().decode(errors="replace")
        if rc == ITSD_ERR_NAN:
            raise AssertionError(msg)
        raise ItsdError(rc, msg)


def stream_ptr(device=None) -> int:
    return torch.cuda.current_stream(device).cuda_stream


def _ptr(t: Optional[torch.Tensor]) -> Optional[int]:
    return None if t is None else t.data_ptr()


class NativeUNet:

    def __init__(self, arch: UNetArch, state_dict: Dict[str, torch.Tensor], max_batch: int, precision: int,
                 device: int = 0):
        L = lib()
        d = UNetDesc()
        d.arch = ARCH_CFG if arch.cfg else ARCH_DDPM
        d.T = arch.T
        d.ch = arch.ch
        d.n_mult = len(arch.ch_mult)
        for i, m in enumerate(arch.ch_mult):
            d.ch_mult[i] = m
        d.n_attn = len(arch.attn)
        for i, m in enumerate(arch.attn):
            d.attn[i] = m
        d.num_res_blocks = arch.num_res_blocks
        d.img_size = arch.img_size
        d.num_labels = arch.num_labels
        d.max_batch = int(max_batch)
        d.precision = int(precision)
        keep = []
        views = (TensorView * len(state_dict))()
        for i, (k, v) in enumerate(state_dict.items()):
            hv = v.detach().to("cpu", torch.float32).contiguous()
            keep.append(hv)
            views[i].name = k.encode()
            views[i].data = hv.data_ptr()
            views[i].numel = hv.numel()
        h = ctypes.c_void_p()
        check(L.itsd_unet_create(ctypes.byref(d), views, len(state_dict), int(device), ctypes.byref(h)))
        self.h = h
        self.arch = arch
        self.max_batch = int(max_batch)
        self.precision = int(precision)
        self.device = int(device)
        self.T_sched = 0

    def close(self):
        if getattr(self, "h", None):
            lib().itsd_unet_destroy(self.h)
            self.h = None

    def __del__(self):
        try:
            self.close()
        except Exception:
            pass

    def forward(self, x: torch.Tensor, t: torch.Tensor, labels: Optional[torch.Tensor], eps: torch.Tensor) -> None:
        check(lib().itsd_unet_forward(self.h, x.data_ptr(), t.data_ptr(), _ptr(labels), eps.data_ptr(),
                                      x.shape[0], stream_ptr(x.device)))

    def representation(self, n: int, channels: int, hw: int, device) -> torch.Tensor:
        out = torch.empty(n, channels, hw, hw, dtype=torch.float32, device=device)
        check(lib().itsd_unet_representation(self.h, out.data_ptr(), int(n), stream_ptr(out.device)))
        return out

    def set_schedule(self, coeff1: torch.Tensor, coeff2: torch.Tensor, sqrt_var: torch.Tensor, w: float = 0.0):
        c1 = coeff1.detach().cpu().float().contiguous()
        c2 = coeff2.detach().cpu().float().contiguous()
        sv = sqrt_var.detach().cpu().float().contiguous()
        check(lib().itsd_set_schedule(self.h, c1.numel(), c1.data_ptr(), c2.data_ptr(), sv.data_ptr(), float(w)))
        self.T_sched = c1.numel()

    def set_schedule_x0(self, tau: Sequence[int], rows: Dict[str, torch.Tensor], clip_x0: bool, w: float = 0.0):
        K = len(tau)
        sc = X0Schedule()
        sc.K = K
        keep = [(ctypes.c_int32 * K)(*[int(t) for t in tau])]
        sc.tau = keep[0]
        for k in X0_ROW_KEYS:
            v = rows[k].detach().cpu().float().contiguous()
            if v.numel() != K:
                raise ValueError(f"x0-form table {k} has {v.numel()} rows, tau has {K}")
            keep.append(v)
            setattr(sc, k, ctypes.cast(v.data_ptr(), ctypes.POINTER(ctypes.c_float)))
        sc.clip_x0 = int(bool(clip_x0))
        sc.w = float(w)
        check(lib().itsd_set_schedule_x0(self.h, ctypes.byref(sc)))
        self.T_sched = K

    def run(self, x: torch.Tensor, t_begin: int, t_end: int, seed: int, noise: Optional[torch.Tensor] = None,
            labels: Optional[torch.Tensor] = None, noise_offset: int = 0, graph: bool = True, clip: bool = True,
            sync: bool = True) -> None:
        flags = (RUN_GRAPH if graph else 0) | (RUN_CLIP if clip else 0) | (RUN_SYNC if sync else 0)
        check(lib().itsd_sampler_run(self.h, x.data_ptr(), _ptr(labels), x.shape[0], int(t_begin), int(t_end),
                                     int(seed) & ((1 << 64) - 1), int(noise_offset), _ptr(noise), flags,
                                     stream_ptr(x.device)))

    def predict_x0(self, x: torch.Tensor, t: int, a0: float, b0: float, out: torch.Tensor,
                   labels: Optional[torch.Tensor] = None) -> torch.Tensor:
        assert out.shape == x.shape and out.dtype == torch.float32 and out.is_contiguous() and x.is_contiguous()
        check(lib().itsd_sampler_predict_x0(self.h, x.data_ptr(), _ptr(labels), x.shape[0], int(t), float(a0),
                                            float(b0), out.data_ptr(), stream_ptr(x.device)))
        return out

    def query(self, key: str) -> int:
        v = ctypes.c_int64()
        check(lib().itsd_unet_query(self.h, key.encode(), ctypes.byref(v)))
        return int(v.value)

    def profile_forward(self, x: torch.Tensor, t: torch.Tensor):
        cm, cf, tm = ctypes.c_double(), ctypes.c_double(), ctypes.c_double()
        cl = ctypes.c_int()
        check(lib().itsd_profile_forward(self.h, x.data_ptr(), t.data_ptr(), x.shape[0], ctypes.byref(cm),
                                         ctypes.byref(cf), ctypes.byref(cl), ctypes.byref(tm), stream_ptr(x.device)))
        return {"conv_ms": cm.value, "conv_flops": cf.value, "conv_launches": cl.value, "total_ms": tm.value}

    def profile_op(self, x: torch.Tensor, t: torch.Tensor, op_index: int, reps: int = 10) -> float:
        ms = ctypes.c_double()
        check(lib().itsd_profile_op(self.h, x.data_ptr(), t.data_ptr(), x.shape[0], int(op_index), int(reps),
                                    ctypes.byref(ms), stream_ptr(x.device)))
# ... 143 lines not shown
```

Before: 64.45 candidate-images/sec.

## Chain consecutive block-local fused P4 convs into one persistent launch

```diff
diff --git a/include/itsd.h b/include/itsd.h
--- a/include/itsd.h
+++ b/include/itsd.h
@@ -146,6 +146,8 @@
 int itsd_unet_read(itsd_unet* u, int what, int id, int n, void* dst, int64_t bytes, void* stream);
 int itsd_unet_poison(itsd_unet* u, void* stream);
 
+int itsd_p4_chain_plan(const itsd_unet_desc* desc, int n, int cus, int mode, int32_t* out, int cap, int32_t* n_out);
+
 const char* itsd_kernel_name(int id);
 
 enum { ITSD_CALIB_MFMA_BF16 = 0, ITSD_CALIB_HBM_COPY = 1, ITSD_CALIB_MFMA_BF16_16X16 = 2 };
diff --git a/inference-time-scaling-for-diffusion-models-beyond-scaling-denoising-steps_amd/csrc/api.hip b/inference-time-scaling-for-diffusion-models-beyond-scaling-denoising-steps_amd/csrc/api.hip
--- a/inference-time-scaling-for-diffusion-models-beyond-scaling-denoising-steps_amd/csrc/api.hip
+++ b/inference-time-scaling-for-diffusion-models-beyond-scaling-denoising-steps_amd/csrc/api.hip
@@ -26,6 +26,7 @@
 int g_attn_fuse = 1;
 int g_tap_prune = 1;
 int g_down_merge = 1;
+int g_p4_chain = 1;
 int g_attn_s1 = 1;
 template <typename T> hipError_t launch_head(const HeadArgs&, hipStream_t);
 template <typename T> hipError_t launch_tail(const TailArgs&, hipStream_t);
@@ -129,7 +130,14 @@
 
 struct Arena {
   std::vector<char> host;
+  bool dry = false;
+  size_t top = 0;
   size_t add(const void* p, size_t bytes) {
+    if (dry) {
+      const size_t off = (top + 255) & ~(size_t)255;
+      top = off + bytes;
+      return off;
+    }
     size_t off = (host.size() + 255) & ~(size_t)255;
     host.resize(off + bytes);
     if (p) std::memcpy(host.data() + off, p, bytes);
@@ -152,6 +160,7 @@
   bool cfg = false;
   int H = 32, ch = 128, tdim = 512, sumC = 0;
   int nb_max = 0;
+  int p4_chained = 0;
   int last_forward_n = 0;
 
   char* wdev = nullptr;
@@ -215,6 +224,7 @@
   std::vector<std::pair<std::string, size_t>> temb_cols;
 
   const float* get(const std::string& name, int64_t numel) {
+    if (ar.dry) return nullptr;
     auto it = w.find(name);
     if (it == w.end()) {
       if (err.empty()) err = "missing key in state_dict: " + name;
@@ -487,9 +497,9 @@
       const float* wsc = peek(p + ".shortcut.weight", (int64_t)out_ch * in_ch);
       const float* bsc = peek(p + ".shortcut.bias", out_ch);
       const float* bb2 = peek(p + ".block2.3.bias", out_ch);
-      if (wsc && bsc && bb2) {
-        std::vector<float> bs((size_t)out_ch);
-        for (int c = 0; c < out_ch; ++c) bs[c] = bb2[c] + bsc[c];
+      if (ar.dry || (wsc && bsc && bb2)) {
+        std::vector<float> bs((size_t)out_ch, 0.f);
+        for (int c = 0; c < out_ch && !ar.dry; ++c) bs[c] = bb2[c] + bsc[c];
         Op& c2 = u->ops.back();
         c2.sc_wfrag = pack_frag(wsc, out_ch, in_ch, 1);
         c2.bias_sc = ar.add(bs.data(), (size_t)out_ch * 4);
@@ -615,9 +625,10 @@
   }
 };
 
-int build(itsd_unet* u, const itsd_tensor_view* views, int nviews) {
+int build(itsd_unet* u, const itsd_tensor_view* views, int nviews, bool dry = false) {
   Builder b;
   b.u = u;
+  b.ar.dry = dry;
   for (int i = 0; i < nviews; ++i) b.w[views[i].name] = {views[i].data, views[i].numel};
   const itsd_unet_desc& d = u->d;
   const int ch = d.ch, tdim = 4 * ch, H = d.img_size;
@@ -801,7 +812,7 @@
     }
   }
   if (!b.err.empty()) return fail(ITSD_ERR_WEIGHTS, b.err);
-  if ((int)b.used != nviews) {
+  if (!dry && (int)b.used != nviews) {
     return fail(ITSD_ERR_WEIGHTS, "state_dict has " + std::to_string(nviews) + " entries, model uses " +
                                       std::to_string(b.used) + " (unexpected keys present)");
   }
@@ -835,9 +846,10 @@
       if (!produced) return fail(ITSD_ERR_INVALID, "internal: GroupNorm input without a statistics producer");
     }
   }
+  u->ws_bytes = b.ws_off;
+  if (dry) return ITSD_OK;
   HIPCHK(hipMalloc(&u->wdev, b.ar.host.size()));
   HIPCHK(hipMemcpy(u->wdev, b.ar.host.data(), b.ar.host.size(), hipMemcpyHostToDevice));
-  u->ws_bytes = b.ws_off;
   HIPCHK(hipMalloc(&u->ws, u->ws_bytes));
   return ITSD_OK;
 }
@@ -853,6 +865,7 @@
   int label_mod;
   int uncond_from;
   TailArgs tail;
+  int chain = 0;
   bool census = false;
   std::vector<std::pair<hipEvent_t, hipEvent_t>>* evs = nullptr;
   std::vector<int>* ev_kind = nullptr;
@@ -1067,6 +1080,90 @@
   return 0.0;
 }
 
+struct PassLaunch {
+  int n = 1;
+  int ops[itsd::kP4ChainMax] = {-1, -1, -1, -1};
+  int G = 0;
+};
+static_assert(itsd::kP4ChainMax == 4, "PassLaunch::ops' initialiser");
+
+int chain_grid(const itsd_unet* u, const std::vector<ConvLaunch>& rp, size_t oi, int mode) {
+  const Op& o = u->ops[oi];
+  const ConvLaunch& cl = rp[oi];
+  const ConvArgs& a = cl.a;
+  if (o.kind != OP_CONV || cl.rc != ITSD_OK || cl.p.kernel != ConvKernel::P4_GN || !cl.p.valid) return 0;
+  if ((a.Wout != 32 && a.Wout != 16) || a.Hout != a.Wout || !a.gn_fold || a.vt_out || a.dbg || a.subpix) return 0;
+  const long long HW = (long long)a.Hout * a.Wout;
+  if (a.M % HW || a.M % 256 || a.Cout % 128) return 0;
+  const long long nct = a.Cout / 128, NT = a.M / 256 * nct, tpi = HW / 256 * nct, G = cl.p.grid.x;
+  if (G >= 1 && NT % G == 0 && (NT / G) % tpi == 0) return (int)G;
+  const long long nimg = a.M / HW;
+  if (mode == 2 && nimg <= itsd::g_num_cus) return (int)nimg;
+  return 0;
+}
+
+std::vector<PassLaunch> chain_plan(const itsd_unet* u, const std::vector<ConvLaunch>& rp, int mode) {
+  std::vector<int> L;
+  for (size_t oi = 0; oi < u->ops.size(); ++oi)
+    if (folded_into(u, rp, oi) < 0) L.push_back((int)oi);
+  std::vector<PassLaunch> out;
+  auto single = [&](int oi) {
+    PassLaunch q;
+    q.ops[0] = oi;
+    out.push_back(q);
+  };
+  for (size_t i = 0; i < L.size();) {
+    const int G = mode ? chain_grid(u, rp, L[i], mode) : 0;
+    if (!G) {
+      single(L[i++]);
+      continue;
+    }
+    PassLaunch ch;
+    ch.ops[0] = L[i];
+    ch.G = G;
+    std::vector<int> ahead;
+    const ConvArgs& a0 = rp[L[i]].a;
+    auto written = [&](int act) {
+      for (int k = 0; k < ch.n; ++k)
+        if (act >= 0 && u->ops[ch.ops[k]].dst == act) return true;
+      return false;
+    };
+    auto member = [&](int oj) {
+      const ConvArgs& a = rp[oj].a;
+      return chain_grid(u, rp, oj, mode) == G && a.Wout == a0.Wout && a.M == a0.M && a.Cout == a0.Cout && a.xcd == a0.xcd;
+    };
+    auto shortcut_at = [&](size_t j) {
+      if (j + 1 >= L.size()) return false;
+      const Op& x = u->ops[L[j]];
+      const Op& b2 = u->ops[L[j + 1]];
+      return x.kind == OP_CONV && x.ksize == 1 && x.resid < 0 && x.vt < 0 && b2.kind == OP_CONV && b2.resid == x.dst &&
+             member(L[j + 1]);
+    };
+    size_t j = i + 1;
+    while (j < L.size() && ch.n < itsd::kP4ChainMax) {
+      if (member(L[j])) {
+        if (shortcut_at(j + 1) && (written(u->ops[L[j + 1]].src1) || written(u->ops[L[j + 1]].src2))) break;
+        ch.ops[ch.n++] = L[j++];
+        continue;
+      }
+      if (shortcut_at(j) && !written(u->ops[L[j]].src1) && !written(u->ops[L[j]].src2)) {
+        ahead.push_back(L[j]);
+        ch.ops[ch.n++] = L[j + 1];
+        j += 2;
+        continue;
+      }
+      break;
+    }
+    for (int oi : ahead) single(oi);
+    if (ch.n < 2) {
+      ch.G = 0;
+    }
+    out.push_back(ch);
+    i = j;
+  }
+  return out;
+}
+
 int run_program(itsd_unet* u, const RunCtx& c, const std::vector<ConvLaunch>& rp, hipStream_t s) {
   int cur_op = 0;
   auto mark = [&](int kind, double fl, const std::function<int()>& fn) -> int {
@@ -1106,9 +1203,19 @@
     }
     return e == hipSuccess ? ITSD_OK : fail(ITSD_ERR_HIP, hipGetErrorString(e));
   }));
-  for (size_t oi = 0; oi < u->ops.size(); ++oi) {
+  const std::vector<PassLaunch> plan = chain_plan(u, rp, c.census ? 0 : c.chain);
+  int saved = 0;
+  for (const PassLaunch& pl : plan) {
+    if (pl.n > 1) {
+      ConvArgs tab[itsd::kP4ChainMax];
+      for (int k = 0; k < pl.n; ++k) tab[k] = rp[pl.ops[k]].a;
+      const hipError_t e = itsd::launch_p4_chain(tab, pl.n, pl.G, s);
+      if (e != hipSuccess) return fail(ITSD_ERR_HIP, std::string("kernel launch: ") + hipGetErrorString(e));
+      saved += pl.n - 1;
+      continue;
+    }
+    const size_t oi = (size_t)pl.ops[0];
     const Op& o = u->ops[oi];
-    if (folded_into(u, rp, oi) >= 0) continue;
     const ConvLaunch& cl = rp[oi];
     int kind = o.kind == OP_ATTNBLOCK ? kCensusAttnBlock : (int)o.kind;
     cur_op = (int)oi + 1;
@@ -1118,6 +1225,7 @@
     if (cl.p.sc_split) fl += 2.0 * cl.a.M * (double)o.Cout * (cl.a.sc_C1 + cl.a.sc_C2);
     CHK(mark(kind, fl, [&]() { return launch_op(u, o, c, &cl, s); }));
   }
+  if (!c.census) u->p4_chained = saved;
   cur_op = 0;
   Op g;
   g.src1 = u->tail_in; g.gamma = u->tail_gn_g; g.beta = u->tail_gn_b; g.silu = 1;
@@ -1209,6 +1317,7 @@
   c.temb = u->proj_buf; c.tsel = nullptr; c.temb_img_stride = u->sumC;
   c.labels = labels; c.label_mod = n; c.uncond_from = -1;
   c.tail.n = n; c.tail.cfg = 0; c.tail.step_mode = 0; c.tail.eps_out = eps_out;
+  c.chain = itsd::g_p4_chain;
   return c;
 }
 
@@ -1220,6 +1329,7 @@
   c.labels = labels; c.label_mod = n; c.uncond_from = u->cfg ? n : -1;
   c.tail.n = n; c.tail.cfg = u->cfg ? 1 : 0; c.tail.guide_w = u->guide_w; c.tail.guide_w1 = u->guide_w1;
   c.tail.x = x;
+  c.chain = itsd::g_p4_chain;
   return c;
 }
 
@@ -1346,6 +1456,7 @@
     {"p4_w", &g_p4_w, 0, 7, 0, "levels conv3x3_gn_p4_kernel takes (bit 0 W = 8, 1 W = 16, 2 W = 32); the others run p5 / 128-pixel tiles"},
     {"p4_xcd", &g_p4_xcd, 0, 2, kDiag, "conv3x3_gn_p4_kernel deals each XCD a contiguous range of tiles: 0 off, 1 on, 2 the 8x8 level only"},
     {"p4_c96", &g_p4_c96, 0, 2, 0, "8x8 conv3x3_gn_p4_kernel on 96-cout tiles: 0 off, 1 auto, 2 always (Cout % 96 == 0)"},
+    {"p4_chain", &g_p4_chain, 0, 2, 0, "consecutive block-local fused convs of the 32x32 / 16x16 levels as one launch: 0 off, 1 where each block walks whole images, 2 also on one block an image (tests at small batches)"},
     {"p4_sub", &g_p4_sub, 0, 1, 0, "nearest-x2 upsample convs on conv3x3_gn_p4_kernel's sub-pixel form: 0 off, 1 on"},
     {"p4_plain", &g_p4_plain, 0, 2, 0, "plain 3x3 stride-1 convs on conv3x3_gn_p4_kernel (halo copies the input): 0 off, 1 from 128 tiles, 2 any tile count"},
     {"p5", &g_p5, 0, 2, 0, "conv3x3_gn_p5_kernel at 8x8: 0 off, 1 auto, 2 always (4x4: always)"},
@@ -1434,6 +1545,7 @@
   else if (!std::strcmp(key, "sched_form")) *value = u->sched_form;
   else if (!std::strcmp(key, "ws_bytes")) *value = (int64_t)u->ws_bytes;
   else if (!std::strcmp(key, "ops")) *value = (int64_t)u->ops.size();
+  else if (!std::strcmp(key, "p4_chained")) *value = u->p4_chained;
   else if (!std::strcmp(key, "status")) {
     if (hipStreamSynchronize(u->stream) != hipSuccess) return fail(ITSD_ERR_HIP, "status: stream synchronize");
     int flag = 0;
@@ -1441,6 +1553,44 @@
     *value = flag;
   }
   else return fail(ITSD_ERR_INVALID, std::string("unknown query key ") + key);
+  return ITSD_OK;
+}
+
+int itsd_p4_chain_plan(const itsd_unet_desc* desc, int n, int cus, int mode, int32_t* out, int cap, int32_t* n_out) {
+  if (!desc || !out || !n_out || cap < 0) return fail(ITSD_ERR_INVALID, "null argument");
+  if (n < 1 || n > desc->max_batch || cus < 1 || mode < 0 || mode > 2) return fail(ITSD_ERR_INVALID, "p4_chain_plan: n, cus or mode out of range");
+  if (desc->arch != ITSD_ARCH_DDPM || desc->precision != ITSD_PREC_BF16 || desc->ch <= 0 || desc->ch % 32 || desc->n_mult < 1 ||
+      desc->n_mult > 8 || desc->n_attn < 0 || desc->n_attn > 8 || desc->num_res_blocks < 1 || desc->img_size < 8)
+    return fail(ITSD_ERR_INVALID, "p4_chain_plan: a bf16 DDPM descriptor");
+  std::unique_ptr<itsd_unet> u(new itsd_unet());
+  u->d = *desc;
+  u->bf16 = true;
+  u->esz = 2;
+  u->nb_max = desc->max_batch;
+  CHK(build(u.get(), nullptr, 0, true));
+  auto made_up = [](int k) { return (char*)(((uintptr_t)k + 1) << 40); };
+  u->wdev = made_up(0); u->ws = made_up(1);
+  u->proj_buf = (float*)made_up(2); u->zero_page = made_up(3); u->splitk_ws = (float*)made_up(4);
+  u->tickets = (int*)made_up(5); u->d_nan = (int*)made_up(6);
+  const int cus0 = itsd::g_num_cus;
+  itsd::g_num_cus = cus;
+  const RunCtx c = forward_ctx(u.get(), n, nullptr, nullptr, nullptr);
+  const std::vector<ConvLaunch> rp = resolve_program(u.get(), c);
+  const std::vector<PassLaunch> plan = chain_plan(u.get(), rp, mode);
+  itsd::g_num_cus = cus0;
+  std::vector<int> cidx(u->ops.size(), 0);
+  int k = 0;
+  for (size_t oi = 0; oi < u->ops.size(); ++oi)
+    if (folded_into(u.get(), rp, oi) < 0) cidx[oi] = ++k;
+  int w = 0;
+  for (const PassLaunch& pl : plan) {
+    if (w + 1 + pl.n > cap) return fail(ITSD_ERR_INVALID, "p4_chain_plan: out too small");
+    out[w++] = pl.n;
+    for (int i = 0; i < pl.n; ++i) out[w++] = cidx[pl.ops[i]];
+  }
+  *n_out = w;
+  u->wdev = u->ws = nullptr;
+  u->proj_buf = nullptr; u->zero_page = nullptr; u->splitk_ws = nullptr; u->tickets = nullptr; u->d_nan = nullptr;
   return ITSD_OK;
 }
 
@@ -1752,6 +1902,7 @@
   ProfileScratch p;
   CHK(p.begin(u, t, n, (hipStream_t)stream));
   RunCtx c = forward_ctx(u, n, x, nullptr, p.eps);
+  c.chain = 0;
   p.census(c, false);
   int r = run_program(u, c, resolve_program(u, c), s);
   hipError_t e = hipStreamSynchronize(s);
@@ -1782,7 +1933,8 @@
   hipStream_t s = u->stream;
   ProfileScratch p;
   CHK(p.begin(u, t, n, (hipStream_t)stream));
-  const RunCtx c = forward_ctx(u, n, x, p.lab0, p.eps);
+  RunCtx c = forward_ctx(u, n, x, p.lab0, p.eps);
+  c.chain = 0;
   const std::vector<ConvLaunch> convs = resolve_program(u, c);
   CHK(run_program(u, c, convs, s));
   p.evs.push_back({nullptr, nullptr});
@@ -1809,6 +1961,7 @@
   ProfileScratch p;
   CHK(p.begin(u, t, n, (hipStream_t)stream));
   RunCtx c = forward_ctx(u, n, x, p.lab0, p.eps);
+  c.chain = 0;
   p.census(c, true);
   const std::vector<ConvLaunch> convs = resolve_program(u, c);
   int r = run_program(u, c, convs, s);
diff --git a/inference-time-scaling-for-diffusion-models-beyond-scaling-denoising-steps_amd/csrc/common.h b/inference-time-scaling-for-diffusion-models-beyond-scaling-denoising-steps_amd/csrc/common.h
--- a/inference-time-scaling-for-diffusion-models-beyond-scaling-denoising-steps_amd/csrc/common.h
+++ b/inference-time-scaling-for-diffusion-models-beyond-scaling-denoising-steps_amd/csrc/common.h
@@ -186,6 +186,9 @@
 };
 ConvPlan plan_conv(const ConvArgs& a, bool bf16);
 
+constexpr int kP4ChainMax = 4;
+hipError_t launch_p4_chain(const ConvArgs* ops, int nops, int G, hipStream_t s);
+
 __host__ __device__ inline int stat_slot_px(int HW) { return HW < 128 ? HW : 128; }
 __host__ __device__ inline int stat_spi(int HW, int spi) { return spi > 0 ? spi : HW / stat_slot_px(HW); }
 
diff --git a/inference-time-scaling-for-diffusion-models-beyond-scaling-denoising-steps_amd/csrc/conv.hip b/inference-time-scaling-for-diffusion-models-beyond-scaling-denoising-steps_amd/csrc/conv.hip
--- a/inference-time-scaling-for-diffusion-models-beyond-scaling-denoising-steps_amd/csrc/conv.hip
+++ b/inference-time-scaling-for-diffusion-models-beyond-scaling-denoising-steps_amd/csrc/conv.hip
@@ -1308,8 +1308,8 @@
 #endif
 constexpr int P4_RING = 6;
 constexpr int P4_BD = 2;
-template <int W, int AB = 0>
-__global__ __launch_bounds__(512, 1) void conv3x3_gn_p4_kernel(ConvArgs a) {
+template <int W, int AB, typename CA>
+__device__ __forceinline__ void conv3x3_gn_p4_body(CA a, const int tz) {
   typedef bf16_t T;
   constexpr bool SUB = (AB & 128) != 0, PLAIN = SUB || (AB & 2) != 0;
   constexpr bool SUB4 = SUB && (AB & 256) == 0;
@@ -1344,7 +1344,7 @@
     if ((threadIdx.x & 63) == 0) g_stamps[((blockIdx.x & 1023) * 16 + 8 + (threadIdx.x >> 6)) * 8 + 1] = hw;
   }
 #endif
-  const int tid = threadIdx.x, lane = tid & 63;
+  const int tid = threadIdx.x + tz, lane = tid & 63;
   const int wid = __builtin_amdgcn_readfirstlane(tid >> 6);
   const int H = a.Hout;
   const int Cin = a.C1 + a.C2, ncc = Cin / 64, kpt = Cin >> 4;
@@ -2000,8 +2000,13 @@
         sq += (double)vq[i].x + (double)vq[i].y;
       }
     }
-    sm += __shfl_xor(sm, 32, 64);
-    sq += __shfl_xor(sq, 32, 64);
+    auto xhalf = [&](double v) {
+      const int lo = __builtin_amdgcn_ds_bpermute((lane ^ 32) << 2, __double2loint(v));
+      const int hi = __builtin_amdgcn_ds_bpermute((lane ^ 32) << 2, __double2hiint(v));
+      return __hiloint2double(hi, lo);
+    };
+    sm += xhalf(sm);
+    sq += xhalf(sq);
     const double E = (double)(Cin / 32) * HWi, mean = sm / E;
     double var = sq / E - mean * mean;
     var = var > 0.0 ? var : 0.0;
@@ -2227,12 +2232,14 @@
     prescale();
   }
   if constexpr (COMPACT) {
-    if (tt < 16) *(u32x4*)(smem + (tt >> 3) * HALO + ZROW * ROWB + ((tt & 7) << 4)) = u32x4{0u, 0u, 0u, 0u};
+    const uint32_t z0 = (uint32_t)tz;
+    const u32x4 zz = {z0, z0, z0, z0};
+    if (tt < 16) *(u32x4*)(smem + (tt >> 3) * HALO + ZROW * ROWB + ((tt & 7) << 4)) = zz;
     if (M16 && ITSD_P4_ZR8) {
       const int r = (tt >> 3) & 15;
-      *(u32x4*)(smem + (tt >> 7) * HALO + (ZROW + (r & 7) + (r >> 3) * 64) * ROWB + ((tt & 7) << 4)) = u32x4{0u, 0u, 0u, 0u};
+      *(u32x4*)(smem + (tt >> 7) * HALO + (ZROW + (r & 7) + (r >> 3) * 64) * ROWB + ((tt & 7) << 4)) = zz;
     } else if (M16 && tt >= 16 && tt < 32) {
-      *(u32x4*)(smem + ((tt >> 3) & 1) * HALO + (ZROW + 64) * ROWB + ((tt & 7) << 4)) = u32x4{0u, 0u, 0u, 0u};
+      *(u32x4*)(smem + ((tt >> 3) & 1) * HALO + (ZROW + 64) * ROWB + ((tt & 7) << 4)) = zz;
     }
   }
   emit(smem);
@@ -2271,6 +2278,36 @@
     drain(ntiles - 1);
   }
   P4_STAMP_OUT();
+}
+
+template <int W, int AB = 0>
+__global__ __launch_bounds__(512, 1) void conv3x3_gn_p4_kernel(ConvArgs a) {
+  conv3x3_gn_p4_body<W, AB, const ConvArgs>(a, 0);
+}
+
+struct P4ChainArgs {
+  ConvArgs op[kP4ChainMax];
+  int nops;
+};
+template <int W>
+__global__ __launch_bounds__(512, 1) void conv3x3_gn_p4_chain_kernel(P4ChainArgs c) {
+  (void)c;
+  typedef const __attribute__((address_space(4))) ConvArgs CA;
+  typedef const __attribute__((address_space(4))) char CB;
+  CB* const kp = (CB*)__builtin_amdgcn_kernarg_segment_ptr();
+  CA* const tab = (CA*)(kp + offsetof(P4ChainArgs, op));
+  const int nops = *(const __attribute__((address_space(4))) int*)(kp + offsetof(P4ChainArgs, nops));
+  for (int op = 0; op < nops; ++op) {
+    if (op) {
+      asm volatile("s_waitcnt vmcnt(0) lgkmcnt(0)" ::: "memory");
+      __builtin_amdgcn_fence(__ATOMIC_RELEASE, "workgroup");
+      __builtin_amdgcn_s_barrier();
+      __builtin_amdgcn_fence(__ATOMIC_ACQUIRE, "workgroup");
+    }
+    int tz;
+    asm volatile("v_mov_b32 %0, 0" : "=v"(tz));
+    conv3x3_gn_p4_body<W, 0, CA&>(tab[op], tz);
+  }
 }
 
 template <int W> struct Gp5Cfg {
@@ -3723,6 +3760,28 @@
 template hipError_t launch_conv<float>(const ConvArgs&, const ConvPlan&, hipStream_t);
 template hipError_t launch_conv<bf16_t>(const ConvArgs&, const ConvPlan&, hipStream_t);
 
+static_assert(sizeof(P4ChainArgs) <= 4096, "the op table is the kernel's argument block");
+hipError_t launch_p4_chain(const ConvArgs* ops, int nops, int G, hipStream_t s) {
+  if (nops < 2 || nops > kP4ChainMax || G < 1) return hipErrorInvalidValue;
+  const ConvArgs& a0 = ops[0];
+  if (a0.Wout != 32 && a0.Wout != 16) return hipErrorInvalidValue;
+  const long long NT = (long long)(a0.M / GNW_BN) * (a0.Cout / CONV_BM);
+  const long long tpi = (long long)(a0.Hout * a0.Wout / GNW_BN) * (a0.Cout / CONV_BM);
+  if (a0.M % GNW_BN || a0.Cout % CONV_BM || NT % G || (NT / G) % tpi) return hipErrorInvalidValue;
+  P4ChainArgs c{};
+  for (int i = 0; i < nops; ++i) {
+    const ConvArgs& a = ops[i];
+    if (a.Wout != a0.Wout || a.Hout != a0.Hout || a.M != a0.M || a.Cout != a0.Cout || a.xcd != a0.xcd || !a.gn_fold ||
+        !a.wfrag || a.subpix || a.vt_out)
+      return hipErrorInvalidValue;
+    c.op[i] = a;
+  }
+  c.nops = nops;
+  if (a0.Wout == 32) ITSD_LAUNCH(conv3x3_gn_p4_chain_kernel<32>, dim3(G), dim3(512), 0, s, c);
+  else ITSD_LAUNCH(conv3x3_gn_p4_chain_kernel<16>, dim3(G), dim3(512), 0, s, c);
+  return hipGetLastError();
+}
+
 }
 
 #ifdef ITSD_STAMPS
diff --git a/inference-time-scaling-for-diffusion-models-beyond-scaling-denoising-steps_amd/runtime.py b/inference-time-scaling-for-diffusion-models-beyond-scaling-denoising-steps_amd/runtime.py
--- a/inference-time-scaling-for-diffusion-models-beyond-scaling-denoising-steps_amd/runtime.py
+++ b/inference-time-scaling-for-diffusion-models-beyond-scaling-denoising-steps_amd/runtime.py
@@ -106,6 +106,8 @@
     "itsd_unet_read": [ctypes.c_void_p, ctypes.c_int, ctypes.c_int, ctypes.c_int, ctypes.c_void_p, ctypes.c_int64,
                        ctypes.c_void_p],
     "itsd_unet_poison": [ctypes.c_void_p, ctypes.c_void_p],
+    "itsd_p4_chain_plan": [ctypes.POINTER(UNetDesc), ctypes.c_int, ctypes.c_int, ctypes.c_int,
+                           ctypes.POINTER(ctypes.c_int32), ctypes.c_int, ctypes.POINTER(ctypes.c_int32)],
     "itsd_kernel_name": [ctypes.c_int],
     "itsd_last_error": [],
     "itsd_version": [],
```

Result: no change. 65.00 candidate-images/sec (median of 6 runs) (+0.8%).
